# modelstreaming/ams

Hardware: AMD Instinct MI355X
Metric: frames/sec student infer (DeeplabV3+MobileNetV2, 512x1024) + distill-steps/sec (higher is better)
Workload: dtype f32 (2xfp16 split products)

## Files before the change

ams_amd/csrc/api.hip:

```cpp
#include "engine.hpp"
#include "head_common.hpp"

using namespace ams;

extern "C" {

const char* ams_last_error(void) { return ams::last_error(); }
int ams_abi_version(void) { return AMS_ABI_VERSION; }

int ams_device_info(char* name_out, size_t name_cap, int32_t* n_cu, int64_t* hbm_bytes) {
    int dev = 0;
    AMS_CHECK_HIP(hipGetDevice(&dev));
    hipDeviceProp_t p;
    AMS_CHECK_HIP(hipGetDeviceProperties(&p, dev));
    if (name_out && name_cap) { snprintf(name_out, name_cap, "%s (%s)", p.name, p.gcnArchName); }
    if (n_cu) *n_cu = p.multiProcessorCount;
    if (hbm_bytes) *hbm_bytes = (int64_t)p.totalGlobalMem;
    return AMS_OK;
}

int ams_student_arena_bytes(const ams_student_config* cfg, const ams_layer_desc* layers, size_t* bytes_out) {
    AMS_REQUIRE(bytes_out, "arena_bytes: null output");
    ams_student tmp;
    int rc = student_build(&tmp, cfg, layers);
// ... 639 lines not shown
                                int32_t* status_dev, int64_t* scratch_dev, size_t scratch_elems, void* stream) {
    AMS_REQUIRE(base_params_dev && payload_dev && payload_bytes_dev && status_dev && scratch_dev, "encode_delta_q8: null pointer");
    AMS_REQUIRE(advance_base == 0 || advance_base == 1, "encode_delta_q8: advance_base %d (0 or 1)", advance_base);
    bool has_stats = false;
    const int64_t shape = delta_table_shape(vars_host, n_vars, "encode_delta_q8", &has_stats);
    if (shape < 0) return AMS_E_INVALID;
    AMS_REQUIRE(base_stats_dev || !has_stats, "encode_delta_q8: null statistics base, and the table has variables in AMS_REGION_STATS");
    const size_t table = q8_encode_table_words(n_vars);
    const size_t need = table + 1 + (size_t)delta_segments(shape);
    AMS_REQUIRE(scratch_elems >= need, "encode_delta_q8: scratch too small (need %zu int64)", need);
    AMS_REQUIRE(payload_cap >= shape + 4 * (int64_t)n_vars, "encode_delta_q8: room for %lld bytes, the mask and scale sections alone have %lld",
                (long long)payload_cap, (long long)(shape + 4 * (int64_t)n_vars));
    AMS_REQUIRE(s, "encode_delta_q8: null handle");
    const int64_t mask_bytes = delta_mask_bytes(s, vars_host, n_vars, "encode_delta_q8");
    if (mask_bytes < 0) return AMS_E_INVALID;
    hipStream_t st = (hipStream_t)stream;
    if (s->ev_encode) AMS_CHECK_HIP(hipEventSynchronize(s->ev_encode));
    else RUN(create_sync_event(&s->ev_encode));
    s->encode_table.assign(table, 0);
    memcpy(s->encode_table.data(), vars_host, n_vars * sizeof(ams_delta_var));
    int64_t first = 0;
    for (int32_t i = 0; i < n_vars; ++i) { s->encode_table[4 * (size_t)n_vars + i] = first; first += vars_host[i].count; }
    s->encode_table[5 * (size_t)n_vars] = first;
    AMS_CHECK_HIP(hipMemcpyAsync(scratch_dev, s->encode_table.data(), table * sizeof(int64_t), hipMemcpyHostToDevice, st));
    AMS_CHECK_HIP(hipEventRecord(s->ev_encode, st));
    return launch_encode_delta_q8(mask_dev, scratch_dev, n_vars, mask_bytes, s->params, s->stats, base_params_dev, base_stats_dev, advance_base,
                                  scratch_dev + table, payload_dev, payload_cap, payload_bytes_dev, status_dev, st);
}

size_t ams_student_apply_delta_q8_scratch(const ams_delta_var* vars_host, int32_t n_vars) {
    return ams_student_apply_delta_scratch(vars_host, n_vars);
}

int ams_student_apply_delta_q8(ams_student* s, const uint8_t* payload_dev, int64_t payload_bytes, const ams_delta_var* vars_host, int32_t n_vars,
                               int64_t* n_applied_dev, int32_t* status_dev, int64_t* scratch_dev, size_t scratch_elems, void* stream) {
    AMS_REQUIRE(n_applied_dev && status_dev && scratch_dev, "apply_delta_q8: null pointer");
    AMS_REQUIRE(payload_bytes >= 0 && (payload_dev || payload_bytes == 0), "apply_delta_q8: %lld payload bytes at %p", (long long)payload_bytes,
                (const void*)payload_dev);
    bool has_stats = false;
    const int64_t shape = delta_table_shape(vars_host, n_vars, "apply_delta_q8", &has_stats);
    if (shape < 0) return AMS_E_INVALID;
    const size_t need = 4 * (size_t)n_vars + (size_t)delta_segments(shape);
    AMS_REQUIRE(scratch_elems >= need, "apply_delta_q8: scratch too small (need %zu int64)", need);
    AMS_REQUIRE(s, "apply_delta_q8: null handle");
    const int64_t mask_bytes = delta_mask_bytes(s, vars_host, n_vars, "apply_delta_q8");
    if (mask_bytes < 0) return AMS_E_INVALID;
    hipStream_t st = (hipStream_t)stream;
    if (s->ev_delta) AMS_CHECK_HIP(hipEventSynchronize(s->ev_delta));
    else RUN(create_sync_event(&s->ev_delta));
    s->delta_vars.assign(vars_host, vars_host + n_vars);
    ams_delta_var* vars_dev = reinterpret_cast<ams_delta_var*>(scratch_dev);
    AMS_CHECK_HIP(hipMemcpyAsync(vars_dev, s->delta_vars.data(), n_vars * sizeof(ams_delta_var), hipMemcpyHostToDevice, st));
    AMS_CHECK_HIP(hipEventRecord(s->ev_delta, st));
    return launch_apply_delta_q8(payload_dev, payload_bytes, vars_dev, n_vars, mask_bytes, s->params, (int64_t)s->cfg.n_trainable, s->stats,
                                 (int64_t)s->cfg.n_stats, scratch_dev + 4 * n_vars, n_applied_dev, status_dev, st);
}

int ams_k_stem_conv(const void* frames, int32_t frames_dtype, int32_t B, int32_t H, int32_t W, const float* w, int32_t cout,
                    const float* scale, const float* shift, int32_t act, float pixel_scale, float* y, void* stream) {
    return launch_stem(frames, frames_dtype, B, H, W, w, cout, scale, shift, act, pixel_scale, y, (hipStream_t)stream);
}

int ams_k_depthwise3x3(const float* x, int32_t B, int32_t H, int32_t W, int32_t C, const float* w, int32_t stride, int32_t rate,
                       const float* scale, const float* shift, int32_t act, float* y, void* stream) {
    return launch_depthwise(x, B, H, W, C, w, stride, rate, scale, shift, act, y, (hipStream_t)stream);
}

int ams_k_pointwise(const float* x, int64_t M, int32_t K, const float* w, int32_t N, int32_t trans_w, const float* img_bias,
                    int64_t rows_per_img, const float* scale, const float* shift, int32_t act, const float* res, float* y,
                    void* stream) {
    PwArgs a = pw_args(x, M, K, K, w, N, y, N);
    if (trans_w) { a.w_sk = 1; a.w_sn = K; }
    a.img_bias = img_bias; a.rows_per_img = rows_per_img > 0 ? rows_per_img : 1;
    a.scale = scale; a.shift = shift; a.act = act; a.res = res; a.ldr = N;
    if (scale && !shift) { set_error("pointwise: scale without shift"); return AMS_E_INVALID; }
    return launch_pointwise(a, (hipStream_t)stream);
}

int ams_k_pointwise_split(const float* x, int64_t M, int32_t K, const float* w, int32_t N, const float* scale, const float* shift,
                          int32_t act, const float* res, float* y, uint16_t* panels, size_t panel_elems, void* stream) {
    const int Kp = (K + 31) / 32 * 32;
    AMS_REQUIRE(panels && panel_elems >= (size_t)2 * N * Kp, "pointwise_split: panel scratch too small (need %zu)", (size_t)2 * N * Kp);
    hipStream_t st = (hipStream_t)stream;
    uint16_t* hi = panels;
    uint16_t* lo = panels + (size_t)N * Kp;
    RUN(launch_split_weights(w, N, 1, K, N, Kp, hi, lo, st));
    PwArgs a = pw_args(x, M, K, K, w, N, y, N);
    a.scale = scale; a.shift = shift; a.act = act; a.res = res; a.ldr = N;
    if (scale && !shift) { set_error("pointwise_split: scale without shift"); return AMS_E_INVALID; }
    return launch_pointwise_split(a, hi, lo, Kp, st);
}

int ams_k_pointwise_split3(const float* x, int64_t M, int32_t K, const float* w, int32_t N, const float* scale, const float* shift,
                           int32_t act, const float* res, float* y, uint16_t* panels, size_t panel_elems, void* stream) {
    const int Kp = (K + 31) / 32 * 32;
    const size_t plane = (size_t)N * Kp;
    AMS_REQUIRE(panels && panel_elems >= 3 * plane, "pointwise_split3: panel scratch too small (need %zu)", 3 * plane);
    hipStream_t st = (hipStream_t)stream;
    RUN(launch_split_weights3(w, N, 1, K, N, Kp, panels, panels + plane, panels + 2 * plane, st));
    PwArgs a = pw_args(x, M, K, K, w, N, y, N);
    a.scale = scale; a.shift = shift; a.act = act; a.res = res; a.ldr = N;
    if (scale && !shift) { set_error("pointwise_split3: scale without shift"); return AMS_E_INVALID; }
    return launch_pointwise_split3(a, panels, panels + plane, panels + 2 * plane, Kp, st);
}

int ams_k_pack_h2i(const float* x, int64_t M, int32_t Cn, float* out, void* stream) { return launch_pack_h2i(x, M, Cn, out, (hipStream_t)stream); }

int ams_k_pointwise_split_f16(const float* x, int64_t M, int32_t K, const float* w, int32_t N, const float* scale, const float* shift, int32_t act,
                              const float* res, float* y, uint16_t* panels, size_t panel_elems, float* x_h2i, uint16_t* y_parts, void* stream) {
    const int Kp = (K + 31) / 32 * 32;
    const size_t plane = (size_t)N * Kp;
    AMS_REQUIRE(panels && panel_elems >= 2 * plane, "pointwise_split_f16: panel scratch too small (need %zu)", 2 * plane);
    hipStream_t st = (hipStream_t)stream;
    RUN(launch_split_weights_f16(w, N, 1, K, N, Kp, panels, panels + plane, st));
    PwArgs a = pw_args(x, M, K, K, w, N, y, N);
    a.scale = scale; a.shift = shift; a.act = act; a.res = res; a.ldr = N;
    if (scale && !shift) { set_error("pointwise_split_f16: scale without shift"); return AMS_E_INVALID; }
    if (x_h2i) {
        if (x_h2i != x) RUN(launch_pack_h2i(x, M, K, x_h2i, st));
        a.x = x_h2i; a.x_fmt = 1;
    }
    if (y_parts) {
        AMS_REQUIRE(pointwise_split_writes_parts(a), "pointwise_split_f16: this shape has no vector epilogue to write parts from");
        a.ysplit = y_parts; a.ysplit_plane = M * (int64_t)N; a.ysplit_np = 2; a.ysplit_fmt = 1;
    }
    AMS_REQUIRE(pointwise_f16_applies(a), "pointwise_split_f16: unsupported shape M=%lld K=%d", (long long)M, K);
    return launch_pointwise_split_f16(a, panels, (int64_t)plane, Kp, st);
}

int ams_ingest_resize_u8(const uint8_t* src, int32_t Hs, int32_t Ws, int32_t Cn, int32_t mode, int32_t swap_rb, uint8_t* dst, int32_t H,
                         int32_t W, void* stream) {
    return launch_resize_u8(src, Hs, Ws, Cn, mode, swap_rb, dst, H, W, (hipStream_t)stream);
}

static void set_panels(ConvLayer* l, const uint16_t* panels, int64_t plane, int np, int Kp) { l->panels = panels; l->plane = plane; l->np = np; l->Kp = Kp; }

int ams_k_dw_project(const float* e, int32_t B, int32_t H, int32_t W, int32_t Cc, const float* w_dw, int32_t rate, const float* scale_d,
                     const float* shift_d, const float* w_proj, int32_t N, const float* scale_p, const float* shift_p,
                     const float* res, float* y, uint16_t* panels, size_t panel_elems, void* stream) {
    hipStream_t st = (hipStream_t)stream;
    const int64_t plane = (int64_t)N * Cc;
    BlockCall c;
    c.x = e; c.B = B; c.H = H; c.W = W; c.Cexp = Cc; c.rate = rate; c.Cout = N; c.residual = res != nullptr; c.res = res; c.y = y;
    c.dw = ConvLayer{w_dw, scale_d, shift_d, AMS_ACT_RELU6};
    c.project = ConvLayer{w_proj, scale_p, shift_p, AMS_ACT_NONE, panels, plane, 2, Cc};
    const EntryScratch sc{panels, panel_elems, (size_t)(2 * plane)};
    RUN(block_call_check("dw_project", BK_DW_PROJECT, c, &sc));
    RUN(launch_split_weights(w_proj, N, 1, Cc, N, Cc, panels, panels + plane, st));
    return launch_dw_project(c, st);
}

static int block_fused_entry(const char* who, bool f16, const float* x, int32_t B, int32_t H, int32_t W, int32_t Cin, const float* w_exp,
                             const float* scale_e, const float* shift_e, int32_t Cexp, const float* w_dw, int32_t stride, const float* scale_d,
                             const float* shift_d, const float* w_proj, int32_t Cout, const float* scale_p, const float* shift_p, int32_t residual,
                             float* y, uint16_t* panels, size_t panel_elems, void* stream) {
    hipStream_t st = (hipStream_t)stream;
    const int kp_p = (Cexp + 31) / 32 * 32;
    const int64_t pe = (int64_t)Cexp * 32, pp = (int64_t)Cout * kp_p;
    BlockCall c;
    c.x = x; c.B = B; c.H = H; c.W = W; c.Cin = Cin; c.Cexp = Cexp; c.stride = stride; c.Cout = Cout; c.residual = residual != 0; c.y = y;
    c.expand = ConvLayer{w_exp, scale_e, shift_e, AMS_ACT_RELU6};
    c.dw = ConvLayer{w_dw, scale_d, shift_d, AMS_ACT_RELU6};
    c.project = ConvLayer{w_proj, scale_p, shift_p, AMS_ACT_NONE};
    uint16_t* hp = panels ? panels + 2 * pe : nullptr;
    if (f16) { set_panels(&c.expand, panels, pe, AMS_NP_F16, 32); set_panels(&c.project, hp, pp, AMS_NP_F16, kp_p); }
    else if (panels) set_panels(&c.expand, panels, pe, 3, 32);
    const EntryScratch sc{panels, panel_elems, (size_t)(f16 ? 2 * pe + 2 * pp : panels ? 3 * pe : 0)};
    RUN(block_call_check(who, BK_WHOLE, c, &sc));
    if (f16) {
        RUN(launch_split_weights_f16(w_exp, Cexp, 1, Cin, Cexp, 32, panels, panels + pe, st));
        RUN(launch_split_weights_f16(w_proj, Cout, 1, Cexp, Cout, kp_p, hp, hp + pp, st));
    } else if (panels)
        RUN(launch_split_weights3(w_exp, Cexp, 1, Cin, Cexp, 32, panels, panels + pe, panels + 2 * pe, st));
    return launch_block_fused(c, st);
}

int ams_k_block_fused(const float* x, int32_t B, int32_t H, int32_t W, int32_t Cin, const float* w_exp, const float* scale_e, const float* shift_e,
                      int32_t Cexp, const float* w_dw, int32_t stride, const float* scale_d, const float* shift_d, const float* w_proj, int32_t Cout,
                      const float* scale_p, const float* shift_p, int32_t residual, float* y, uint16_t* panels, size_t panel_elems, void* stream) {
    return block_fused_entry("block_fused", false, x, B, H, W, Cin, w_exp, scale_e, shift_e, Cexp, w_dw, stride, scale_d, shift_d, w_proj, Cout, scale_p,
                             shift_p, residual, y, panels, panel_elems, stream);
}

int ams_k_block_fused_f16(const float* x, int32_t B, int32_t H, int32_t W, int32_t Cin, const float* w_exp, const float* scale_e, const float* shift_e,
                          int32_t Cexp, const float* w_dw, int32_t stride, const float* scale_d, const float* shift_d, const float* w_proj, int32_t Cout,
                          const float* scale_p, const float* shift_p, int32_t residual, float* y, uint16_t* panels, size_t panel_elems, void* stream) {
    return block_fused_entry("block_fused_f16", true, x, B, H, W, Cin, w_exp, scale_e, shift_e, Cexp, w_dw, stride, scale_d, shift_d, w_proj, Cout, scale_p,
                             shift_p, residual, y, panels, panel_elems, stream);
}

static_assert(sizeof(ams_first_block_plan) == sizeof(FirstBlockPlan) && sizeof(FirstBlockPlan) == 15 * sizeof(int32_t), "ams_first_block_plan is FirstBlockPlan, field by field");
static size_t first_block_scratch(int form) { return form == 1 ? 3 * 32 * 32 : (form == 2 ? 2 * 32 * 32 + 2 * 16 * 32 : 0); }
static BlockCall first_block_call(const void* frames, int dtype, int B, int H, int W, float pixel_scale, const float* w_stem, const float* scale_s,
                                  const float* shift_s, const float* w_dw, const float* scale_d, const float* shift_d, const float* w_proj,
                                  const float* scale_p, const float* shift_p, float* y) {
    BlockCall c;
    c.frames = frames; c.dtype = dtype; c.pixel_scale = pixel_scale; c.B = B; c.H = H; c.W = W; c.Cin = 3; c.Cexp = 32; c.Cout = 16; c.y = y;
    c.expand = ConvLayer{w_stem, scale_s, shift_s, AMS_ACT_RELU6};
    c.dw = ConvLayer{w_dw, scale_d, shift_d, AMS_ACT_RELU6};
    c.project = ConvLayer{w_proj, scale_p, shift_p, AMS_ACT_NONE};
    return c;
}

size_t ams_k_first_block_scratch(int32_t form) { return first_block_scratch(form); }

int ams_k_first_block_plan(int32_t frames_dtype, int32_t B, int32_t H, int32_t W, int32_t form, const int32_t* occupancy, ams_first_block_plan* plan_out) {
    BlockCall c;
    c.dtype = frames_dtype; c.B = B; c.H = H; c.W = W;
    const EntryScratch sc{nullptr, 0, 0, form, 3};
    RUN(block_call_check("first_block_plan", BK_FIRST_PLAN, c, &sc));
    AMS_REQUIRE(!occupancy || (occupancy[0] > 0 && occupancy[1] > 0 && occupancy[2] > 0), "first_block_plan: occupancy figures must be positive");
    AMS_REQUIRE(plan_out, "first_block_plan: null pointer");
    FirstBlockPlan p;
    RUN(first_block_plan(frames_dtype, B, H, W, form == 2, occupancy, &p));
    memcpy(plan_out, &p, sizeof(p));
    return AMS_OK;
}

int ams_k_first_block(const void* frames, int32_t frames_dtype, int32_t B, int32_t H, int32_t W, float pixel_scale, const float* w_stem,
                      const float* scale_s, const float* shift_s, const float* w_dw, const float* scale_d, const float* shift_d, const float* w_proj,
                      const float* scale_p, const float* shift_p, float* y, int32_t form, uint16_t* panels, size_t panel_elems,
                      ams_first_block_plan* plan_out, void* stream) {
    hipStream_t st = (hipStream_t)stream;
    const int64_t ps = 32 * 32, pj = 16 * 32;
    BlockCall c = first_block_call(frames, frames_dtype, B, H, W, pixel_scale, w_stem, scale_s, shift_s, w_dw, scale_d, shift_d, w_proj, scale_p, shift_p, y);
    uint16_t* hj = panels ? panels + 2 * ps : nullptr;
    if (form == 1) set_panels(&c.expand, panels, ps, 3, 32);
    else if (form == 2) { set_panels(&c.expand, panels, ps, AMS_NP_F16, 32); set_panels(&c.project, hj, pj, AMS_NP_F16, 32); }
    const EntryScratch sc{panels, panel_elems, first_block_scratch(form), form, 3};
    RUN(block_call_check("first_block", BK_FIRST, c, &sc));
    if (form == 1)
        RUN(launch_split_weights3(w_stem, 32, 1, 27, 32, 32, panels, panels + ps, panels + 2 * ps, st));
    else if (form == 2) {
        RUN(launch_split_weights_f16(w_stem, 32, 1, 27, 32, 32, panels, panels + ps, st));
        RUN(launch_split_weights_f16(w_proj, 16, 1, 32, 16, 32, hj, hj + pj, st));
    }
    FirstBlockPlan p;
    RUN(launch_first_block(c, st, &p));
    if (plan_out) memcpy(plan_out, &p, sizeof(p));
    return AMS_OK;
}

int ams_k_first_block_tiles(const void* frames, int32_t frames_dtype, int32_t B, int32_t H, int32_t W, float pixel_scale, const float* w_stem,
                            const float* scale_s, const float* shift_s, const float* w_dw, const float* scale_d, const float* shift_d,
                            const float* w_proj, const float* scale_p, const float* shift_p, float* y, void* stream) {
    return launch_first_block_tiles(first_block_call(frames, frames_dtype, B, H, W, pixel_scale, w_stem, scale_s, shift_s, w_dw, scale_d, shift_d, w_proj,
                                                     scale_p, shift_p, y), (hipStream_t)stream);
}

int ams_k_expand_dw(const float* x, int32_t B, int32_t H, int32_t W, int32_t Cin, const float* w_exp, const float* scale_e,
                    const float* shift_e, int32_t Cexp, const float* w_dw, int32_t stride, int32_t rate, const float* scale_d,
                    const float* shift_d, float* y, void* stream) {
    BlockCall c;
    c.x = x; c.B = B; c.H = H; c.W = W; c.Cin = Cin; c.Cexp = Cexp; c.stride = stride; c.rate = rate; c.y = y;
    c.expand = ConvLayer{w_exp, scale_e, shift_e, AMS_ACT_RELU6};
    c.dw = ConvLayer{w_dw, scale_d, shift_d, AMS_ACT_RELU6};
    return launch_expand_dw(c, (hipStream_t)stream);
}

static int expand_dw_stream_entry(const char* who, bool f16, const float* x, int32_t B, int32_t H, int32_t W, int32_t Cin, const float* w_exp,
                                  const float* scale_e, const float* shift_e, int32_t Cexp, const float* w_dw, int32_t rate, const float* scale_d,
                                  const float* shift_d, float* y, uint16_t* panels, size_t panel_elems, int32_t parts, int32_t presplit, int32_t y_h2i,
                                  void* stream) {
    hipStream_t st = (hipStream_t)stream;
    const bool f32 = !f16 && Cin <= 32;
    const int ns = f16 ? 2 : 3;
    const size_t plane = (size_t)Cexp * Cin, xplane = (size_t)B * H * W * Cin;
    BlockCall c;
    c.x = x; c.B = B; c.H = H; c.W = W; c.Cin = Cin; c.Cexp = Cexp; c.rate = rate; c.y = y; c.y_fmt = y_h2i ? 1 : 0;
    c.expand = ConvLayer{w_exp, scale_e, shift_e, AMS_ACT_RELU6};
    c.dw = ConvLayer{w_dw, scale_d, shift_d, AMS_ACT_RELU6};
    if (f32 && rate < 0) { c.stride = -rate; c.rate = 1; }
    const EntryScratch sc{panels, panel_elems, f32 ? 0 : ns * plane + (presplit ? ns * xplane : 0), 0, 1, f16 ? Cin >= 64 : (parts == 2 || parts == 3)};
    uint16_t* xq = panels && presplit ? panels + ns * plane : nullptr;
    if (!f32) {
        set_panels(&c.expand, panels, (int64_t)plane, f16 ? AMS_NP_F16 : parts, Cin);
        c.x_parts = xq; c.x_plane = (int64_t)xplane;
    }
    const bool wreg = !f32 && presplit == 2;
    RUN(block_call_check(who, wreg ? BK_WREG : BK_STREAM, c, &sc));
    AMS_REQUIRE(x, "%s: null pointer", who);
    if (!f32) {
        const int M = (int)((int64_t)B * H * W);
        if (f16) RUN(launch_split_weights_f16(w_exp, Cexp, 1, Cin, Cexp, Cin, panels, panels + plane, st));
        else RUN(launch_split_weights3(w_exp, Cexp, 1, Cin, Cexp, Cin, panels, panels + plane, panels + 2 * plane, st));
        if (xq && f16) RUN(launch_split_weights_f16(x, 1, Cin, Cin, M, Cin, xq, xq + xplane, st));
        else if (xq) RUN(launch_split_weights3(x, 1, Cin, Cin, M, Cin, xq, xq + xplane, xq + 2 * xplane, st));
    }
    return wreg ? launch_expand_dw_wreg(c, st) : launch_expand_dw_stream(c, st);
}

int ams_k_expand_dw_stream(const float* x, int32_t B, int32_t H, int32_t W, int32_t Cin, const float* w_exp, const float* scale_e,
                           const float* shift_e, int32_t Cexp, const float* w_dw, int32_t rate, const float* scale_d, const float* shift_d,
                           float* y, uint16_t* panels, size_t panel_elems, int32_t parts, int32_t presplit, void* stream) {
    return expand_dw_stream_entry("expand_dw_stream", false, x, B, H, W, Cin, w_exp, scale_e, shift_e, Cexp, w_dw, rate, scale_d, shift_d, y, panels, panel_elems,
                                  parts, presplit, 0, stream);
}

int ams_k_expand_dw_stream_f16(const float* x, int32_t B, int32_t H, int32_t W, int32_t Cin, const float* w_exp, const float* scale_e,
                               const float* shift_e, int32_t Cexp, const float* w_dw, int32_t rate, const float* scale_d, const float* shift_d,
                               float* y, uint16_t* panels, size_t panel_elems, int32_t presplit, int32_t y_h2i, void* stream) {
    return expand_dw_stream_entry("expand_dw_stream_f16", true, x, B, H, W, Cin, w_exp, scale_e, shift_e, Cexp, w_dw, rate, scale_d, shift_d, y, panels,
                                  panel_elems, 2, presplit, y_h2i, stream);
}

int ams_k_global_mean(const float* x, int32_t B, int64_t HW, int32_t C, float* y, float* scratch, size_t scratch_floats,
                      void* stream) {
    AMS_REQUIRE(scratch && scratch_floats >= image_colsum_scratch(B, C), "global_mean: scratch too small (need %zu floats)",
                image_colsum_scratch(B, C));
    return launch_global_mean(x, B, HW, C, y, scratch, (hipStream_t)stream);
}
size_t ams_k_global_mean_scratch(int32_t B, int32_t C) { return image_colsum_scratch(B, C); }

int ams_k_upsample_argmax(const float* logits, int32_t B, int32_t h, int32_t w, int32_t NC, const int32_t* class_idx_host, int32_t K,
                          int32_t H, int32_t W, const uint8_t* teacher, int32_t* labels_out, int64_t* conf_mat, double* loss,
                          void* stream) {
    const HeadCall c{logits, NC, B, h, w, class_idx_host, K, H, W, teacher, NC};
    return launch_upsample_argmax(c, labels_out, conf_mat, loss, (hipStream_t)stream);
}

int ams_k_upsample_confidence(const float* logits, int32_t B, int32_t h, int32_t w, int32_t NC, const int32_t* class_idx_host, int32_t K,
                              int32_t H, int32_t W, const uint8_t* teacher, uint8_t* conf_u8, float* conf_f32, int64_t* stats, void* stream) {
    const HeadCall c{logits, NC, B, h, w, class_idx_host, K, H, W, teacher, NC};
    return launch_upsample_confidence(c, conf_u8, conf_f32, stats, (hipStream_t)stream);
}
size_t ams_confidence_stats_len(void) { return (size_t)confidence_stats_len(); }

int ams_k_upsample_soft_metric_layout(const float* logits, int32_t B, int32_t h, int32_t w, int32_t ld, int32_t NC, const int32_t* class_idx_host,
                                      int32_t K, int32_t H, int32_t W, const uint8_t* teacher, const float* teacher_logits, int32_t th, int32_t tw,
                                      int32_t layout, int64_t* stats, float* p_f32, float* ce_f32, void* stream) {
    const HeadCall c{logits, ld, B, h, w, class_idx_host, K, H, W, teacher, NC};
    return launch_upsample_soft_metric(c, LossObjective{teacher_logits, th, tw, layout}, stats, p_f32, ce_f32, (hipStream_t)stream);
}

int ams_k_upsample_soft_metric(const float* logits, int32_t B, int32_t h, int32_t w, int32_t NC, const int32_t* class_idx_host, int32_t K,
                               int32_t H, int32_t W, const uint8_t* teacher, const float* teacher_logits, int32_t th, int32_t tw, int64_t* stats,
                               float* p_f32, float* ce_f32, void* stream) {
    return ams_k_upsample_soft_metric_layout(logits, B, h, w, NC, NC, class_idx_host, K, H, W, teacher, teacher_logits, th, tw, AMS_TLOGITS_FULL, stats, p_f32,
                                             ce_f32, stream);
}
size_t ams_soft_metric_stats_len(int32_t K) { return K >= 1 && K <= 32 ? (size_t)soft_metric_stats_len(K) : 0; }

int ams_k_ce_grad(const float* logits, int32_t B, int32_t h, int32_t w, int32_t NC, const int32_t* class_idx_host, int32_t K, int32_t H,
                  int32_t W, const uint8_t* teacher, const double* loss_and_count_dev, float* dlogits, void* stream) {
    const HeadCall c{logits, NC, B, h, w, class_idx_host, K, H, W, teacher, NC};
    return launch_ce_grad(c, loss_and_count_dev, dlogits, NC, (hipStream_t)stream);
}

size_t ams_k_ce_loss_grad_scratch(int32_t B, int32_t h, int32_t w, int32_t K) { return ce_loss_grad_scratch(B, h, w, K); }

static int ce_loss_grad_entry(const char* who, const HeadCall& c, const LossObjective& o, bool needs_teacher_logits, double* loss_dev, float* dlogits,
                              float* scratch, size_t scratch_floats, void* stream) {
    RUN(kd_params_check(who, o.temperature, o.alpha));
    RUN(loss_weights_check(who, o.class_weights, c.K, c.K, o.conf_gamma));
    AMS_REQUIRE(o.teacher_logits || !needs_teacher_logits, "%s: null teacher logits (alpha %g, conf_gamma %g)", who, (double)o.alpha, (double)o.conf_gamma);
    AMS_REQUIRE(c.cls, "%s: null class table", who);
    AMS_REQUIRE(c.K >= 1 && c.K <= 32, "%s: K=%d out of range (1..32)", who, c.K);
    AMS_REQUIRE(tlogits_layout_ok(o.layout), "%s: unknown teacher-logit layout %d", who, o.layout);
    AMS_REQUIRE(c.ld >= c.NC && c.ld <= 256, "%s: row stride %d must hold %d classes", who, c.ld, c.NC);
    AMS_REQUIRE(ce_loss_grad_supported(c.w, c.W), "%s: %d output columns on %d source columns is outside the one-pass kernel", who, c.W, c.w);
    AMS_REQUIRE(scratch && scratch_floats >= ce_loss_grad_scratch(c.B, c.h, c.w, c.K), "%s: scratch too small (need %zu floats)", who,
                ce_loss_grad_scratch(c.B, c.h, c.w, c.K));
    hipStream_t st = (hipStream_t)stream;
    RUN(launch_ce_loss_grad(c, o, loss_dev, scratch, st));
    return launch_ce_combine(c, loss_dev, scratch, dlogits, c.ld, st);
}

int ams_k_ce_loss_grad(const float* logits, int32_t B, int32_t h, int32_t w, int32_t NC, const int32_t* class_idx_host, int32_t K, int32_t H,
                       int32_t W, const uint8_t* teacher, double* loss_dev, float* dlogits, float* scratch, size_t scratch_floats, void* stream) {
    const HeadCall c{logits, NC, B, h, w, class_idx_host, K, H, W, teacher, NC};
    return ce_loss_grad_entry("ce_loss_grad", c, LossObjective{}, false, loss_dev, dlogits, scratch, scratch_floats, stream);
}

int ams_k_ce_loss_grad_soft(const float* logits, int32_t B, int32_t h, int32_t w, int32_t NC, const int32_t* class_idx_host, int32_t K, int32_t H,
                            int32_t W, const uint8_t* teacher, const float* teacher_logits, int32_t th, int32_t tw, double* loss_dev, float* dlogits,
                            float* scratch, size_t scratch_floats, void* stream) {
    const HeadCall c{logits, NC, B, h, w, class_idx_host, K, H, W, teacher, NC};
    const LossObjective o{teacher_logits, th, tw, AMS_TLOGITS_FULL};
    return ce_loss_grad_entry("ce_loss_grad_soft", c, o, true, loss_dev, dlogits, scratch, scratch_floats, stream);
}

int ams_k_ce_loss_grad_soft_layout(const float* logits, int32_t B, int32_t h, int32_t w, int32_t ld, int32_t NC, const int32_t* class_idx_host,
                                   int32_t K, int32_t H, int32_t W, const uint8_t* teacher, const float* teacher_logits, int32_t th, int32_t tw, int32_t layout,
                                   double* loss_dev, float* dlogits, float* scratch, size_t scratch_floats, void* stream) {
    const HeadCall c{logits, ld, B, h, w, class_idx_host, K, H, W, teacher, NC};
    const LossObjective o{teacher_logits, th, tw, layout};
    return ce_loss_grad_entry("ce_loss_grad_soft_layout", c, o, true, loss_dev, dlogits, scratch, scratch_floats, stream);
}

int ams_k_ce_loss_grad_kd(const float* logits, int32_t B, int32_t h, int32_t w, int32_t ld, int32_t NC, const int32_t* class_idx_host, int32_t K,
                          int32_t H, int32_t W, const uint8_t* teacher, const float* teacher_logits, int32_t th, int32_t tw, int32_t layout,
                          double* loss_dev, float* dlogits, float* scratch, size_t scratch_floats, void* stream, float temperature, float alpha) {
    const HeadCall c{logits, ld, B, h, w, class_idx_host, K, H, W, teacher, NC};
    const LossObjective o{teacher_logits, th, tw, layout, temperature, alpha};
    return ce_loss_grad_entry("ce_loss_grad_kd", c, o, true, loss_dev, dlogits, scratch, scratch_floats, stream);
}

int ams_k_ce_loss_grad_weighted(const float* logits, int32_t B, int32_t h, int32_t w, int32_t ld, int32_t NC, const int32_t* class_idx_host, int32_t K,
                                int32_t H, int32_t W, const uint8_t* teacher, const float* teacher_logits, int32_t th, int32_t tw, int32_t layout,
                                double* loss_dev, float* dlogits, float* scratch, size_t scratch_floats, void* stream, float temperature, float alpha,
                                const float* class_weights_host, float conf_gamma) {
    const HeadCall c{logits, ld, B, h, w, class_idx_host, K, H, W, teacher, NC};
    const LossObjective o{teacher_logits, th, tw, layout, temperature, alpha, class_weights_host, conf_gamma};
    return ce_loss_grad_entry("ce_loss_grad_weighted", c, o, conf_gamma != 0.f || alpha != 0.f, loss_dev, dlogits, scratch, scratch_floats, stream);
}

size_t ams_k_loss_mining_scratch(int32_t B, int32_t H, int32_t W) { return loss_mining_scratch(B, H, W); }

int ams_k_ce_loss_grad_mined(const float* logits, int32_t B, int32_t h, int32_t w, int32_t ld, int32_t NC, const int32_t* class_idx_host, int32_t K,
                             int32_t H, int32_t W, const uint8_t* teacher, const float* teacher_logits, int32_t th, int32_t tw, int32_t layout,
                             double* loss_dev, float* dlogits, float* scratch, size_t scratch_floats, void* stream, float temperature, float alpha,
                             const float* class_weights_host, float conf_gamma, float top_k, uint8_t* labels_out_dev, float* key_out_dev,
                             ams_mining_result* result_dev, void* mining_scratch_dev, size_t mining_scratch_bytes) {
    const char* who = "ce_loss_grad_mined";
    HeadCall c{logits, ld, B, h, w, class_idx_host, K, H, W, teacher, NC};
    const LossObjective o{teacher_logits, th, tw, layout, temperature, alpha, class_weights_host, conf_gamma};
    RUN(kd_params_check(who, o.temperature, o.alpha));
    RUN(loss_weights_check(who, o.class_weights, c.K, c.K, o.conf_gamma));
    AMS_REQUIRE(o.teacher_logits || (conf_gamma == 0.f && alpha == 0.f), "%s: null teacher logits (alpha %g, conf_gamma %g)", who, (double)o.alpha, (double)o.conf_gamma);
    AMS_REQUIRE(c.cls, "%s: null class table", who);
    AMS_REQUIRE(c.K >= 1 && c.K <= 32, "%s: K=%d out of range (1..32)", who, c.K);
    AMS_REQUIRE(tlogits_layout_ok(o.layout), "%s: unknown teacher-logit layout %d", who, o.layout);
    AMS_REQUIRE(c.ld >= c.NC && c.ld <= 256, "%s: row stride %d must hold %d classes", who, c.ld, c.NC);
    AMS_REQUIRE(ce_loss_grad_supported(c.w, c.W), "%s: %d output columns on %d source columns is outside the one-pass kernel", who, c.W, c.w);
    AMS_REQUIRE(scratch && scratch_floats >= ce_loss_grad_scratch(c.B, c.h, c.w, c.K), "%s: scratch too small (need %zu floats)", who,
                ce_loss_grad_scratch(c.B, c.h, c.w, c.K));
    RUN(mining_top_k_check(who, top_k));
    hipStream_t st = (hipStream_t)stream;
    if (top_k < 1.f) {
        AMS_REQUIRE(B >= 1 && H >= 1 && W >= 1, "%s: no pixels: B=%d, %d x %d", who, B, H, W);
        AMS_REQUIRE(mining_scratch_dev && ((uintptr_t)mining_scratch_dev & 15) == 0 && mining_scratch_bytes >= loss_mining_scratch(B, H, W),
                    "%s: mining scratch NULL, misaligned or too small (need %zu bytes, 16-byte aligned)", who, loss_mining_scratch(B, H, W));
        AMS_REQUIRE(labels_out_dev && result_dev, "%s: null output (mined labels, result)", who);
        AMS_REQUIRE(((uintptr_t)result_dev & 7) == 0 && ((uintptr_t)key_out_dev & 3) == 0, "%s: misaligned output", who);
        MiningBuffers m = loss_mining_buffers(mining_scratch_dev, B, H, W);
        m.labels = labels_out_dev;
        m.result = result_dev;
        if (key_out_dev) m.keys = key_out_dev;
        AMS_REQUIRE(loss_dev && dlogits, "%s: null pointer", who);
        RUN(launch_loss_mining(c, o, top_k, m, st));
        c.teacher = labels_out_dev;
    } else {
        AMS_REQUIRE(labels_out_dev, "%s: null output (mined labels)", who);
        AMS_REQUIRE(c.logits && c.teacher && loss_dev && dlogits && B >= 1 && H >= 1 && W >= 1, "%s: null pointer", who);
        AMS_CHECK_HIP(hipMemcpyAsync(labels_out_dev, teacher, (size_t)B * H * W, hipMemcpyDeviceToDevice, st));
    }
    RUN(launch_ce_loss_grad(c, o, loss_dev, scratch, st));
    return launch_ce_combine(c, loss_dev, scratch, dlogits, c.ld, st);
}

size_t ams_k_pointwise_wgrad_scratch(int64_t M, int32_t K, int32_t N) { return pointwise_wgrad_scratch(M, K, N); }

int ams_k_pointwise_wgrad_split(const float* x, const float* dy, int64_t M, int32_t K, int32_t N, float* dw, float* scratch,
                                size_t scratch_floats, void* stream) {
    if (!pointwise_wgrad_x6_applies(M, K, N, K, N)) { set_error("pointwise_wgrad_split: shape M=%lld K=%d N=%d not supported", (long long)M, K, N); return AMS_E_INVALID; }
    WgArgs a;
    a.x = x; a.ldx = K; a.K = K; a.dy = dy; a.ldy = N; a.N = N; a.M = M; a.dw = dw; a.scratch = scratch; a.scratch_floats = scratch_floats; a.allow_split = 1;
    return launch_pointwise_wgrad(a, (hipStream_t)stream);
}

int ams_k_pointwise_wgrad(const float* x, const float* dy, int64_t M, int32_t K, int32_t N, float* dw, float* scratch,
                          size_t scratch_floats, void* stream) {
    WgArgs a;
    a.x = x; a.ldx = K; a.K = K; a.dy = dy; a.ldy = N; a.N = N; a.M = M; a.dw = dw; a.scratch = scratch; a.scratch_floats = scratch_floats; a.allow_split = 0;
    return launch_pointwise_wgrad(a, (hipStream_t)stream);
}

int ams_k_depthwise3x3_dgrad(const float* dy, int32_t B, int32_t H, int32_t W, int32_t C, const float* w, int32_t stride, int32_t rate,
                             float* dx, void* stream) {
    return launch_depthwise_dgrad(dy, B, H, W, C, w, stride, rate, dx, (hipStream_t)stream);
}

int ams_k_depthwise3x3_wgrad(const float* x, const float* dy, int32_t B, int32_t H, int32_t W, int32_t C, int32_t stride, int32_t rate,
                             float* dw, float* scratch, size_t scratch_floats, void* stream) {
    return launch_depthwise_wgrad(x, dy, B, H, W, C, stride, rate, dw, scratch, scratch_floats, (hipStream_t)stream);
}

int ams_k_pointwise_red(const float* x, int64_t M, int32_t K, const float* w, int32_t N, int32_t trans_w, int32_t split, int32_t mode,
                        const float* center, const float* z, const float* scale, const float* shift, const float* mean, const float* rstd,
                        int32_t act, const float* res, float* y, float* part, size_t part_floats, int32_t* rows_out, uint16_t* panels,
                        size_t panel_elems, void* stream) {
    AMS_REQUIRE(x && w && y && part && rows_out && (mode == 1 || mode == 2), "pointwise_red: bad arguments");
    AMS_REQUIRE(mode == 1 || (z && scale && shift && mean && rstd), "pointwise_red: mode 2 needs z, scale, shift, mean, rstd");
    hipStream_t st = (hipStream_t)stream;
    PwArgs a = pw_args(x, M, K, K, w, N, y, N);
    if (trans_w) { a.w_sk = 1; a.w_sn = K; }
    a.res = res; a.ldr = N;
    a.red_mode = mode; a.red_center = center; a.red_z = z; a.red_scale = scale; a.red_shift = shift; a.red_mean = mean; a.red_rstd = rstd;
    a.red_act = act; a.red_part = part; a.red_part_floats = part_floats;
    int rows = 0;
    a.red_rows_out = &rows;
    int rc;
    if (split == 2) {
        const int Kp = (K + 31) / 32 * 32;
        const size_t plane = (size_t)N * Kp;
        AMS_REQUIRE(panels && panel_elems >= 2 * plane && pointwise_f16_applies(a), "pointwise_red: fp16 form needs mode 1, K %% 8 == 0 and %zu panel elements", 2 * plane);
        RUN(launch_split_weights_f16(w, a.w_sk, a.w_sn, K, N, Kp, panels, panels + plane, st));
        rc = launch_pointwise_split_f16(a, panels, (int64_t)plane, Kp, st);
    } else if (split) {
        const int Kp = (K + 31) / 32 * 32;
        const size_t plane = (size_t)N * Kp;
        AMS_REQUIRE(panels && panel_elems >= 3 * plane && K % 8 == 0, "pointwise_red: panel scratch too small (need %zu) or K %% 8", 3 * plane);
        RUN(launch_split_weights3(w, a.w_sk, a.w_sn, K, N, Kp, panels, panels + plane, panels + 2 * plane, st));
        rc = launch_pointwise_split3(a, panels, panels + plane, panels + 2 * plane, Kp, st);
    } else {
        rc = launch_pointwise(a, st);
    }
    *rows_out = rows;
    return rc;
}

int ams_k_pointwise_xform(const float* x, int64_t M, int32_t K, const float* w, int32_t N, int32_t trans_w, int32_t split, int32_t x_mode,
                          int32_t x_act, const float* v0, const float* v1, const float* v2, const float* x2, float* y, float* x_tmp,
                          uint16_t* panels, size_t panel_elems, void* stream) {
    AMS_REQUIRE(x && w && y && v0 && v1 && (x_mode == 1 || (x_mode == 2 && v2 && x2)), "pointwise_xform: bad arguments");
    hipStream_t st = (hipStream_t)stream;
    PwArgs a = pw_args(x, M, K, K, w, N, y, N);
    if (trans_w) { a.w_sk = 1; a.w_sn = K; }
    a.x_mode = x_mode; a.x_act = x_act; a.x_v0 = v0; a.x_v1 = v1; a.x_v2 = v2; a.x2 = x2; a.x_tmp = x_tmp;
    if (split == 2) {
        const int Kp = (K + 31) / 32 * 32;
        const size_t plane = (size_t)N * Kp;
        AMS_REQUIRE(panels && panel_elems >= 2 * plane && pointwise_f16_applies(a), "pointwise_xform: fp16 form needs x_mode 1, K %% 8 == 0, K <= 1024 and %zu panel elements", 2 * plane);
        RUN(launch_split_weights_f16(w, a.w_sk, a.w_sn, K, N, Kp, panels, panels + plane, st));
        return launch_pointwise_split_f16(a, panels, (int64_t)plane, Kp, st);
    }
    if (split) {
        const int Kp = (K + 31) / 32 * 32;
        const size_t plane = (size_t)N * Kp;
        AMS_REQUIRE(panels && panel_elems >= 3 * plane && K % 8 == 0, "pointwise_xform: panel scratch too small (need %zu) or K %% 8", 3 * plane);
        RUN(launch_split_weights3(w, a.w_sk, a.w_sn, K, N, Kp, panels, panels + plane, panels + 2 * plane, st));
        return launch_pointwise_split3(a, panels, panels + plane, panels + 2 * plane, Kp, st);
    }
    return launch_pointwise(a, st);
}

int ams_k_pointwise_wgrad_xform(const float* x, const float* dy, int64_t M, int32_t K, int32_t N, int32_t split, int32_t x_mode, int32_t x_act,
                                const float* v0, const float* v1, int32_t dy_mode, const float* d0, const float* d1, const float* d2,
                                const float* dy2, float* dw, float* scratch, size_t scratch_floats, void* stream) {
    AMS_REQUIRE(x && dy && dw && scratch, "pointwise_wgrad_xform: null pointer");
    if (split && !pointwise_wgrad_x6_applies(M, K, N, K, N)) { set_error("pointwise_wgrad_xform: shape M=%lld K=%d N=%d outside the split kernel", (long long)M, K, N); return AMS_E_INVALID; }
    WgArgs a;
    a.x = x; a.ldx = K; a.K = K; a.dy = dy; a.ldy = N; a.N = N; a.M = M; a.dw = dw; a.scratch = scratch; a.scratch_floats = scratch_floats;
    a.allow_split = split != 0;
    a.x_mode = x_mode; a.x_act = x_act; a.x_v0 = v0; a.x_v1 = v1;
    a.dy_mode = dy_mode; a.dy_v0 = d0; a.dy_v1 = d1; a.dy_v2 = d2; a.dy2 = dy2;
    return launch_pointwise_wgrad(a, (hipStream_t)stream);
}

size_t ams_k_depthwise3x3_fwd_bn_scratch(int32_t B, int32_t H, int32_t W, int32_t C, int32_t rate) { return depthwise_fwd_bn_scratch(B, H, W, C, rate); }
int ams_k_depthwise3x3_fwd_bn(const float* ze, int32_t B, int32_t H, int32_t W, int32_t C, const float* w, int32_t rate, const float* scale,
                              const float* shift, int32_t act, const float* center, float* zd, float* scratch, size_t scratch_floats,
                              int32_t* rows_out, void* stream) {
    AMS_REQUIRE(ze && w && scale && shift && zd && scratch && rows_out, "depthwise3x3_fwd_bn: null pointer");
    AMS_REQUIRE(scratch_floats >= depthwise_fwd_bn_scratch(B, H, W, C, rate), "depthwise3x3_fwd_bn: scratch too small");
    int rows = 0;
    int rc = launch_depthwise_fwd_bn(ze, B, H, W, C, w, rate, scale, shift, act, center, zd, scratch, &rows, (hipStream_t)stream);
    *rows_out = rows;
    return rc;
}
size_t ams_k_depthwise3x3_dgrad_bn_scratch(int32_t B, int32_t H, int32_t W, int32_t C) { return depthwise_dgrad_bn_scratch(B, H, W, C); }
int ams_k_depthwise3x3_dgrad_bn(const float* dz, int32_t B, int32_t H, int32_t W, int32_t C, const float* w, int32_t rate, const float* z_prev,
                                const float* scale, const float* shift, int32_t act, const float* mean, const float* rstd, float* out,
                                float* scratch, size_t scratch_floats, int32_t* rows_out, void* stream) {
    AMS_REQUIRE(dz && w && z_prev && scale && shift && mean && rstd && out && scratch && rows_out, "depthwise3x3_dgrad_bn: null pointer");
    AMS_REQUIRE(rate == 1 || rate == 2, "depthwise3x3_dgrad_bn: rate %d", rate);
    AMS_REQUIRE(scratch_floats >= depthwise_dgrad_bn_scratch(B, H, W, C), "depthwise3x3_dgrad_bn: scratch too small");
    int rows = 0;
    int rc = launch_depthwise_dgrad_bn(dz, B, H, W, C, w, rate, z_prev, scale, shift, act, mean, rstd, out, scratch, &rows, (hipStream_t)stream);
    *rows_out = rows;
    return rc;
}

size_t ams_k_depthwise3x3_fwd_bn_tiles_scratch(int32_t B, int32_t H, int32_t W, int32_t C, int32_t rate) { return depthwise_fwd_bn2_scratch(B, H, W, C, rate); }
int ams_k_depthwise3x3_fwd_bn_tiles(const float* ze, int32_t B, int32_t H, int32_t W, int32_t C, const float* w, int32_t rate, const float* scale,
                                    const float* shift, int32_t act, const float* center, float* zd, float* scratch, size_t scratch_floats,
                                    int32_t* rows_out, void* stream) {
    AMS_REQUIRE(ze && w && scale && shift && zd && scratch && rows_out, "depthwise3x3_fwd_bn_tiles: null pointer");
    AMS_REQUIRE(scratch_floats >= depthwise_fwd_bn2_scratch(B, H, W, C, rate), "depthwise3x3_fwd_bn_tiles: scratch too small");
    int rows = 0;
    int rc = launch_depthwise_fwd_bn2(ze, B, H, W, C, w, rate, scale, shift, act, center, zd, scratch, &rows, (hipStream_t)stream);
    *rows_out = rows;
    return rc;
}

size_t ams_k_depthwise3x3_dgrad_bn_apply_scratch(int32_t B, int32_t H, int32_t W, int32_t C, int32_t rate) { return depthwise_dgrad_bn2_scratch(B, H, W, C, rate); }
int ams_k_depthwise3x3_dgrad_bn_apply(const float* dy, const float* zd, const float* cA, const float* cB, const float* cC, int32_t B, int32_t H, int32_t W,
                                      int32_t C, const float* w, int32_t rate, const float* z_prev, const float* scale, const float* shift, int32_t act,
                                      const float* mean, const float* rstd, float* out, float* scratch, size_t scratch_floats, int32_t* rows_out,
                                      void* stream) {
    AMS_REQUIRE(dy && zd && cA && cB && cC && w && z_prev && scale && shift && mean && rstd && out && scratch && rows_out, "depthwise3x3_dgrad_bn_apply: null pointer");
    AMS_REQUIRE(rate == 1 || rate == 2, "depthwise3x3_dgrad_bn_apply: rate %d", rate);
    AMS_REQUIRE(scratch_floats >= depthwise_dgrad_bn2_scratch(B, H, W, C, rate), "depthwise3x3_dgrad_bn_apply: scratch too small");
    int rows = 0;
    int rc = launch_depthwise_dgrad_bn2(dy, zd, cA, cB, cC, B, H, W, C, w, rate, z_prev, scale, shift, act, mean, rstd, out, scratch, &rows, (hipStream_t)stream);
    *rows_out = rows;
    return rc;
}

size_t ams_k_xx_gram_scratch(int64_t M, int32_t Cin) { return xx_stats_scratch_doubles(M, Cin); }
int ams_k_xx_gram(const float* x, int64_t M, int32_t Cin, double* scratch, size_t scratch_doubles, double* xx64, float* xx32, void* stream) {
    AMS_REQUIRE(scratch_doubles >= xx_stats_scratch_doubles(M, Cin), "xx_gram: scratch too small");
    return launch_xx_gram(x, M, Cin, scratch, xx64, xx32, (hipStream_t)stream);
}
int ams_k_expand_stats(const double* xx64, int32_t Cin, const float* w_exp, int32_t Cexp, double n, const float* center, const float* gamma,
                       const float* beta, float eps, float one_minus_decay, float* moving_mean, float* moving_var, float* scale, float* shift,
// ... 58 lines not shown
```

ams_amd/csrc/k_xdw_stream.hip:

```cpp
#include "pw_common.hpp"
#include "split_bf16.hpp"
#include "block_call.hpp"

namespace ams {

#ifdef AMS_XDW_PK
#define AMS_DW_FMA4(A_, V_, W_) fma4_pk(A_, V_, W_)
#else
#define AMS_DW_FMA4(A_, V_, W_) do { A_.x = fmaf(V_.x, W_.x, A_.x); A_.y = fmaf(V_.y, W_.y, A_.y); A_.z = fmaf(V_.z, W_.z, A_.z); A_.w = fmaf(V_.w, W_.w, A_.w); } while (0)
#endif

constexpr int xds_pitch(int nc) { return nc == 32 ? 48 : nc == 64 ? 80 : nc == 96 ? 112 : nc + 4; }

struct XdsArgs {
    const float* x;
    const unsigned short* xs;
    int64_t xs_plane;
    int B, H, W, Cin;
    const unsigned short* wp;
    int64_t plane;
    const float* wf;
    const float* sc_e; const float* sh_e;
    int act_e;
    int Cexp;
    const float* w_dw;
    const float* sc_d; const float* sh_d;
    int act_d;
    float* y;
    int rate;
    int stride;
    int Ho, Wo, cy0, cx0;
    int SH, SW;
    int Wp;
    int T;
    int ring;
    int nsy, nsx;
    int chunks;
    int items;
    int groups;
    int y_fmt;
    int timed;
};

__device__ unsigned long long g_xds_cycles[1024][8];

template <int KS, int NT, int NP, int NWE, int NWD, bool PRE, bool F32, int S = 1, bool H16 = false>
__global__ __launch_bounds__(64 * (NWE + NWD)) void xdw_stream_kernel(XdsArgs a, unsigned nblocks) {
    static_assert(!H16 || (NP == 2 && !F32 && S == 1), "the fp16 form: two parts, stride 1");
    constexpr int NC = 16 * NT;
    constexpr int CG = NC / 4;
    constexpr int STEP = 16 * NWE;
    constexpr int PX = STEP * CG / (64 * NWD);
    static_assert(PX * 64 * NWD == STEP * CG && PX >= 1, "D-step mapping");
    static_assert(!(F32 && PRE), "the exact-f32 form splits nothing");
    constexpr int PITCH = xds_pitch(NC);
    constexpr int MIRROR = 4;
    constexpr int Kp = F32 ? KS * 16 : KS * 32;
    constexpr int WPF = NC + 4;
    constexpr int W_BYTES = F32 ? Kp * WPF * 4 : NP * Kp * NC * 2;
    extern __shared__ __attribute__((aligned(16))) unsigned char smem[];
    u32x4* sW = reinterpret_cast<u32x4*>(smem);
    float* sWf = reinterpret_cast<float*>(smem);
    float* sAff = reinterpret_cast<float*>(smem + W_BYTES);
    float* ring = sAff + 2 * NC;

    const unsigned lb = xcd_remap(blockIdx.x, nblocks);
    const int chunk = lb % a.chunks;
    const int group = lb / a.chunks;
    const int n0 = chunk * NC;
    const int tid = threadIdx.x, lane = tid & 63;
    const int wave = __builtin_amdgcn_readfirstlane(tid >> 6);
    const int Wp = a.Wp, rate = a.rate, R = a.ring;

    if constexpr (F32) {
        for (int e = tid; e < Kp * NC; e += 64 * (NWE + NWD)) {
            const int k = e / NC, n = e - k * NC;
            const int nn = n0 + n < a.Cexp ? n0 + n : a.Cexp - 1;
            sWf[k * WPF + n] = k < a.Cin ? a.wf[(int64_t)k * a.Cexp + nn] : 0.f;
        }
    } else {
        constexpr int UPR = Kp / 8;
        constexpr int NPIECE = NP * NC * UPR;
        for (int e = tid; e < NPIECE; e += 64 * (NWE + NWD)) {
            const int part = e / (NC * UPR), r = e - part * (NC * UPR), n = r / UPR, u = r - n * UPR;
            const int nn = n0 + n < a.Cexp ? n0 + n : a.Cexp - 1;
            const u32x4 v = *reinterpret_cast<const u32x4*>(a.wp + part * a.plane + (int64_t)nn * Kp + u * 8);
            sW[((part * KS + (u >> 2)) * 4 + (u & 3)) * NC + n] = v;
        }
    }
    if (tid < NC) {
        const int nn = n0 + tid < a.Cexp ? n0 + tid : a.Cexp - 1;
        sAff[tid] = a.sc_e[nn]; sAff[NC + tid] = a.sh_e[nn];
    }
    __syncthreads();
    const int qS = STEP / Wp, rS = STEP - qS * Wp;
    unsigned long long tc[2] = {0, 0}, tl_ = a.timed ? __builtin_amdgcn_s_memtime() : 0, nstep = 0;
    auto lap = [&](int slot) {
        if (a.timed) {
            const unsigned long long now = __builtin_amdgcn_s_memtime();
            tc[slot] += now - tl_;
            tl_ = now;
        }
    };
    auto flush = [&](int base) {
        if (a.timed && lane == 0) {
            unsigned long long* row = g_xds_cycles[(blockIdx.x * 8 + wave) & 1023];
            atomicAdd(&row[base], tc[0]);
            atomicAdd(&row[base + 1], tc[1]);
            atomicAdd(&row[base ? 7 : 6], nstep);
        }
    };

    if (wave < NWE) {
        const int l15 = lane & 15, q = lane >> 4;
        const int ring_lane = (16 * wave + l15) * PITCH + 4 * q;
        int sbase = 0;
        for (int item = group; item < a.items; item += a.groups) {
            int u1 = item;
            const int segx = u1 % a.nsx; u1 /= a.nsx;
            const int segy = u1 % a.nsy; u1 /= a.nsy;
            const int sub = u1 % (rate * rate);
            const int b = u1 / (rate * rate);
            const int sy = sub / rate, sx = sub - sy * rate;
            const int Hs = (a.H - sy + rate - 1) / rate, Ws = (a.W - sx + rate - 1) / rate;
            const int i0 = segy * a.SH, j0 = segx * a.SW;
            const bool live = i0 < Hs && j0 < Ws;
            const int64_t frame0 = (int64_t)b * a.H * a.W * a.Cin + (F32 ? 0 : 8 * q);
            int e_row, e_col;
            { const int e0 = 16 * wave + l15; e_row = e0 / Wp; e_col = e0 - e_row * Wp; }
            float4 raw[(PRE || F32) ? 1 : KS][2];
            u32x4 rawp[PRE ? KS : 1][NP];
            float4 rawf[F32 ? KS : 1];
            bool in_next = false;
            auto next_pixel = [&]() -> int64_t {
                const int i = i0 - 1 + e_row, j = j0 - 1 + e_col;
                in_next = (i >= 0) & (i < Hs) & (j >= 0) & (j < Ws) & (e_row < a.SH + 2) & live;
                const int ic = i < 0 ? 0 : (i > Hs - 1 ? Hs - 1 : i), jc = j < 0 ? 0 : (j > Ws - 1 ? Ws - 1 : j);
                return frame0 + ((int64_t)(sy + rate * ic) * a.W + (sx + rate * jc)) * a.Cin;
            };
            auto load_stage = [&](int64_t off, int s) {
                if constexpr (F32) {
                    int ko = 16 * s + 4 * q;
                    if (ko > a.Cin - 4) ko = a.Cin - 4;
                    rawf[s] = ld4(a.x + off + ko);
                } else if constexpr (PRE) {
#pragma unroll
                    for (int pp = 0; pp < NP; ++pp) rawp[s][pp] = *reinterpret_cast<const u32x4*>(a.xs + pp * a.xs_plane + off + 32 * s);
                } else {
                    raw[s][0] = ld4(a.x + off + 32 * s);
                    raw[s][1] = ld4(a.x + off + 32 * s + 4);
                }
            };
            {
                const int64_t p = next_pixel();
#pragma unroll
                for (int s = 0; s < KS; ++s) load_stage(p, s);
            }
            for (int t = 0; t < a.T; ++t) {
                const bool inside = in_next;
                f32x4 acc[NT], accx[H16 ? NT : 1];
#pragma unroll
                for (int tt = 0; tt < NT; ++tt) acc[tt] = (f32x4){0.f, 0.f, 0.f, 0.f};
#pragma unroll
                for (int tt = 0; tt < (H16 ? NT : 1); ++tt) accx[tt] = (f32x4){0.f, 0.f, 0.f, 0.f};
                e_row += qS; e_col += rS;
                if (e_col >= Wp) { e_col -= Wp; ++e_row; }
                const int64_t pn = next_pixel();
                if constexpr (F32) {
#pragma unroll
                    for (int s = 0; s < KS; ++s) {
                        const float4 av[1] = {rawf[s]};
                        load_stage(pn, s);
                        f32x4(&acc2)[1][NT] = *reinterpret_cast<f32x4(*)[1][NT]>(&acc);
                        pw_chunk<1, NT, WPF>(acc2, av, sWf + (16 * s + 4 * q) * WPF + l15);
                    }
                } else {
                bf16x8 x0, x1, x2;
    #pragma unroll
                    for (int s = 0; s < KS; ++s) {
                        if constexpr (PRE) {
                            x0 = __builtin_bit_cast(bf16x8, rawp[s][0]);
                            if (NP >= 2) x1 = __builtin_bit_cast(bf16x8, rawp[s][NP >= 2 ? 1 : 0]);
                            if (NP == 3) x2 = __builtin_bit_cast(bf16x8, rawp[s][NP - 1]);
                        } else if constexpr (H16) {
                            f16x8 h, l;
                            split8_f16(raw[s][0], raw[s][1], h, l);
                            x0 = __builtin_bit_cast(bf16x8, h); x1 = __builtin_bit_cast(bf16x8, l);
                        } else {
                            if (NP == 3) split8(raw[s][0], raw[s][1], x0, x1, x2);
                            else if (NP == 2) split8(raw[s][0], raw[s][1], x0, x1);
                            else split8(raw[s][0], raw[s][1], x0);
                        }
                        load_stage(pn, s);
                        const u32x4* bw = sW + (s * 4 + q) * NC + l15;
                        bf16x8 q0[NT], q1[NT], q2[NT];
    #pragma unroll
                        for (int tt = 0; tt < NT; ++tt) {
                            q0[tt] = *reinterpret_cast<const bf16x8*>(bw + 16 * tt);
                            if (NP >= 2) q1[tt] = *reinterpret_cast<const bf16x8*>(bw + KS * 4 * NC + 16 * tt);
                            if (NP == 3) q2[tt] = *reinterpret_cast<const bf16x8*>(bw + 2 * KS * 4 * NC + 16 * tt);
                        }
                        if constexpr (H16) {
    #pragma unroll
                            for (int tt = 0; tt < NT; ++tt) accx[tt] = __builtin_amdgcn_mfma_f32_16x16x32_f16(__builtin_bit_cast(f16x8, q1[tt]), __builtin_bit_cast(f16x8, x0), accx[tt], 0, 0, 0);
    #pragma unroll
                            for (int tt = 0; tt < NT; ++tt) accx[tt] = __builtin_amdgcn_mfma_f32_16x16x32_f16(__builtin_bit_cast(f16x8, q0[tt]), __builtin_bit_cast(f16x8, x1), accx[tt], 0, 0, 0);
    #pragma unroll
                            for (int tt = 0; tt < NT; ++tt) acc[tt] = __builtin_amdgcn_mfma_f32_16x16x32_f16(__builtin_bit_cast(f16x8, q0[tt]), __builtin_bit_cast(f16x8, x0), acc[tt], 0, 0, 0);
                        } else {
                        if (NP == 3) {
    #pragma unroll
                            for (int tt = 0; tt < NT; ++tt) acc[tt] = __builtin_amdgcn_mfma_f32_16x16x32_bf16(q2[tt], x0, acc[tt], 0, 0, 0);
    #pragma unroll
                            for (int tt = 0; tt < NT; ++tt) acc[tt] = __builtin_amdgcn_mfma_f32_16x16x32_bf16(q0[tt], x2, acc[tt], 0, 0, 0);
    #pragma unroll
                            for (int tt = 0; tt < NT; ++tt) acc[tt] = __builtin_amdgcn_mfma_f32_16x16x32_bf16(q1[tt], x1, acc[tt], 0, 0, 0);
                        }
                        if (NP >= 2) {
    #pragma unroll
                            for (int tt = 0; tt < NT; ++tt) acc[tt] = __builtin_amdgcn_mfma_f32_16x16x32_bf16(q1[tt], x0, acc[tt], 0, 0, 0);
    #pragma unroll
                            for (int tt = 0; tt < NT; ++tt) acc[tt] = __builtin_amdgcn_mfma_f32_16x16x32_bf16(q0[tt], x1, acc[tt], 0, 0, 0);
                        }
    #pragma unroll
                        for (int tt = 0; tt < NT; ++tt) acc[tt] = __builtin_amdgcn_mfma_f32_16x16x32_bf16(q0[tt], x0, acc[tt], 0, 0, 0);
                        }
                    }
                }
                {
                    float* dst = ring + sbase * PITCH + ring_lane;
                    const bool mirror = sbase == 0 && 16 * wave + l15 < MIRROR;
#pragma unroll
                    for (int tt = 0; tt < NT; ++tt) {
                        const float4 sc = ld4(sAff + 16 * tt + 4 * q), sh = ld4(sAff + NC + 16 * tt + 4 * q);
                        float4 v;
                        const float lo = inside ? (a.act_e == AMS_ACT_NONE ? -__builtin_huge_valf() : 0.f) : 0.f;
                        const float hi = inside ? (a.act_e == AMS_ACT_RELU6 ? 6.f : __builtin_huge_valf()) : 0.f;
                        if constexpr (H16) acc[tt] = combine_f16(acc[tt], accx[H16 ? tt : 0]);
                        const float4 bn = muladd4_pk(make_float4(acc[tt][0], acc[tt][1], acc[tt][2], acc[tt][3]), sc, sh);
                        v.x = __builtin_amdgcn_fmed3f(bn.x, lo, hi); v.y = __builtin_amdgcn_fmed3f(bn.y, lo, hi);
                        v.z = __builtin_amdgcn_fmed3f(bn.z, lo, hi); v.w = __builtin_amdgcn_fmed3f(bn.w, lo, hi);
                        st4(dst + 16 * tt, v);
                        if (mirror) st4(dst + R * PITCH + 16 * tt, v);
                    }
                }
                sbase += STEP;
                if (sbase == R) sbase = 0;
                lap(0);
                __syncthreads();
                lap(1);
                ++nstep;
            }
            __syncthreads();
        }
        flush(0);
    } else {
        const int dt = tid - 64 * NWE;
        const int cg = dt % CG, pt = dt / CG;
        const bool chan_ok = n0 + 4 * cg < a.Cexp;
        const int nch = chan_ok ? n0 + 4 * cg : 0;
        float4 wv[9];
#pragma unroll
        for (int k = 0; k < 9; ++k) wv[k] = ld4(a.w_dw + (int64_t)k * a.Cexp + nch);
        const float4 dsc = ld4(a.sc_d + nch), dsh = ld4(a.sh_d + nch);
        const bool odd_cg = (cg & 1) != 0;
        const unsigned ych = a.y_fmt ? (unsigned)(nch >> 3) * 32u + (odd_cg ? 16u : 0u) : (unsigned)nch * 4u;
        int cb = (2 * R - 2 * Wp - 2 + pt * PX) % R;
        for (int item = group; item < a.items; item += a.groups) {
            int u1 = item;
            const int segx = u1 % a.nsx; u1 /= a.nsx;
            const int segy = u1 % a.nsy; u1 /= a.nsy;
            const int sub = u1 % (rate * rate);
            const int b = u1 / (rate * rate);
            const int sy = sub / rate, sx = sub - sy * rate;
            const int Hs = (a.H - sy + rate - 1) / rate, Ws = (a.W - sx + rate - 1) / rate;
            const int i0 = segy * a.SH, j0 = segx * a.SW;
            const bool live = i0 < Hs && j0 < Ws && chan_ok;
            const int64_t oframe = S == 2 ? (int64_t)a.Ho * a.Wo * a.Cexp : (int64_t)a.H * a.W * a.Cexp;
            const __amdgpu_buffer_rsrc_t yrsrc = __builtin_amdgcn_make_buffer_rsrc(a.y + b * oframe, 0, (int)(oframe * 4), 0x00020000);
            const int rmax = live ? (a.SH < Hs - i0 ? a.SH : Hs - i0) : 0, cmax = a.SW < Ws - j0 ? a.SW : Ws - j0;
            const int colpitch = rate * a.Cexp * 4, rowpitch = rate * a.W * a.Cexp * 4;
            const int off0 = ((sy + rate * (i0 - 1)) * a.W + sx + rate * (j0 - 1)) * a.Cexp * 4 + (int)ych;
            int d_row, d_col;
            { const int c0 = Wp - 1 + pt * PX; d_row = c0 / Wp; d_col = c0 - d_row * Wp; d_row -= 2; }
            __syncthreads();
            for (int t = 0; t < a.T; ++t) {
                if constexpr (S == 2) {
#pragma unroll
                    for (int h = 0; h < PX; h += 2) {
                        int row = d_row, col = d_col + h;
#pragma unroll
                        for (int w = 0; w < (PX + 1) / 2; ++w)
                            if (col >= Wp) { col -= Wp; ++row; }
                        const int u = (j0 + col - 1 - a.cx0) & 1;
                        col += u;
                        if (col >= Wp) { col -= Wp; ++row; }
                        const int i = i0 + row - 1, j = j0 + col - 1;
                        const bool ok = ((unsigned)(row - 1) < (unsigned)rmax) & ((unsigned)(col - 1) < (unsigned)cmax) &
                                        ((((i - a.cy0) | (j - a.cx0)) & 1) == 0);
                        if (__builtin_amdgcn_ballot_w64(ok) != 0) {
                            float4 v[3][3];
#pragma unroll
                            for (int di = 0; di < 3; ++di) {
                                unsigned slot = (unsigned)(cb + di * Wp + h + u);
                                slot = slot < (unsigned)R ? slot : slot - (unsigned)R;
                                const float* rp = ring + __umul24(slot, PITCH) + 4 * cg;
#pragma unroll
                                for (int jj = 0; jj < 3; ++jj) v[di][jj] = ld4(rp + jj * PITCH);
                            }
                            float4 acc4 = make_float4(0.f, 0.f, 0.f, 0.f);
#pragma unroll
                            for (int ii = 0; ii < 3; ++ii)
#pragma unroll
                                for (int jj = 0; jj < 3; ++jj) {
                                    const float4 vv = v[ii][jj];
                                    const float4 w4 = wv[ii * 3 + jj];
                                    AMS_DW_FMA4(acc4, vv, w4);
                                }
                            float4 o;
                            o.x = apply_act(acc4.x * dsc.x + dsh.x, a.act_d); o.y = apply_act(acc4.y * dsc.y + dsh.y, a.act_d);
                            o.z = apply_act(acc4.z * dsc.z + dsh.z, a.act_d); o.w = apply_act(acc4.w * dsc.w + dsh.w, a.act_d);
                            const int oy = (i - a.cy0) >> 1, ox = (j - a.cx0) >> 1;
                            const unsigned off = ok ? (unsigned)((oy * a.Wo + ox) * a.Cexp * 4) + ych : 0xfffffff0u;
                            const u32x4 d = {__float_as_uint(o.x), __float_as_uint(o.y), __float_as_uint(o.z), __float_as_uint(o.w)};
                            __builtin_amdgcn_raw_buffer_store_b128(d, yrsrc, off, 0, 0);
                        }
                    }
                } else
#pragma unroll
                for (int h = 0; h < PX; h += 2) {
                    constexpr int PH = PX >= 2 ? 2 : 1;
                    float4 v[3][PH + 2];
#pragma unroll
                    for (int di = 0; di < 3; ++di) {
                        unsigned slot = (unsigned)(cb + di * Wp + h);
                        slot = slot < (unsigned)R ? slot : slot - (unsigned)R;
                        const float* rp = ring + __umul24(slot, PITCH) + 4 * cg;
#pragma unroll
                        for (int jj = 0; jj < PH + 2; ++jj) v[di][jj] = ld4(rp + jj * PITCH);
                    }
#pragma unroll
                    for (int u = 0; u < PH; ++u) {
                        float4 acc4 = make_float4(0.f, 0.f, 0.f, 0.f);
#pragma unroll
                        for (int i = 0; i < 3; ++i)
#pragma unroll
                            for (int j = 0; j < 3; ++j) {
                                const float4 vv = v[i][u + j];
                                const float4 w4 = wv[i * 3 + j];
                                AMS_DW_FMA4(acc4, vv, w4);
                            }
                        float4 o;
                        o.x = apply_act(acc4.x * dsc.x + dsh.x, a.act_d); o.y = apply_act(acc4.y * dsc.y + dsh.y, a.act_d);
                        o.z = apply_act(acc4.z * dsc.z + dsh.z, a.act_d); o.w = apply_act(acc4.w * dsc.w + dsh.w, a.act_d);
                        int row = d_row, col = d_col + h + u;
#pragma unroll
                        for (int w = 0; w < (PX + 1) / 2; ++w)
                            if (col >= Wp) { col -= Wp; ++row; }
                        const bool ok = ((unsigned)(row - 1) < (unsigned)rmax) & ((unsigned)(col - 1) < (unsigned)cmax);
                        const unsigned off = ok ? (unsigned)(row * rowpitch + col * colpitch + off0) : 0xfffffff0u;
                        if (H16 && a.y_fmt) {
                            unsigned h[2], l[2];
                            split4_f16(o, h, l);
                            const unsigned r0 = (unsigned)__builtin_amdgcn_update_dpp(0, (int)(odd_cg ? h[0] : l[0]), 0xB1, 0xF, 0xF, false);
                            const unsigned r1 = (unsigned)__builtin_amdgcn_update_dpp(0, (int)(odd_cg ? h[1] : l[1]), 0xB1, 0xF, 0xF, false);
                            const u32x4 d = {odd_cg ? r0 : h[0], odd_cg ? r1 : h[1], odd_cg ? l[0] : r0, odd_cg ? l[1] : r1};
                            __builtin_amdgcn_raw_buffer_store_b128(d, yrsrc, off, 0, 0);
                        } else {
                        const u32x4 d = {__float_as_uint(o.x), __float_as_uint(o.y), __float_as_uint(o.z), __float_as_uint(o.w)};
                        __builtin_amdgcn_raw_buffer_store_b128(d, yrsrc, off, 0, 0);
                        }
                    }
                }
                d_row += qS; d_col += rS;
                if (d_col >= Wp) { d_col -= Wp; ++d_row; }
                cb += STEP;
                if (cb >= R) cb -= R;
                lap(0);
                __syncthreads();
                lap(1);
                ++nstep;
            }
        }
        flush(2);
    }
}

int xds_phase_cycles(unsigned long long* h) {
    static unsigned long long rows[1024][8], z[1024][8];
    if (hipMemcpyFromSymbol(rows, HIP_SYMBOL(g_xds_cycles), sizeof(rows)) != hipSuccess) return AMS_E_HIP;
    if (hipMemcpyToSymbol(HIP_SYMBOL(g_xds_cycles), z, sizeof(z)) != hipSuccess) return AMS_E_HIP;
    for (int i = 0; i < 8; ++i) h[i] = 0;
    for (int r = 0; r < 1024; ++r)
        for (int i = 0; i < 8; ++i) h[i] += rows[r][i];
    return AMS_OK;
}

struct XdsPlan { int nt, nwe, nwd, SH, SW, nsy, nsx, ring, groups; size_t lds; };

static size_t xds_lds(int Kp, int nt, int np, int ring) {
    const int NC = 16 * nt;
    const size_t w = np == 0 ? (size_t)Kp * (NC + 4) * 4 : (size_t)np * Kp * NC * 2;
    return w + 2 * NC * 4 + (size_t)(ring + 4) * xds_pitch(NC) * 4;
}
static int xds_ring(int SW, int step) { return (2 * (SW + 2) + 2 + 2 * step + step - 1) / step * step; }

static bool xds_plan_try(int B, int H, int W, int Cin, int Cexp, int rate, int np, int nt, int nwe, int nwd, int nsy_force, int nsx_force,
                         int groups_force, XdsPlan* p) {
    const int Kp = np == 0 ? (Cin + 15) / 16 * 16 : Cin;
    const int Hs = (H + rate - 1) / rate, Ws = (W + rate - 1) / rate;
    const int step = 16 * nwe;
    const size_t budget = 160 * 1024 - 512;
    int nsx = nsx_force > 0 ? nsx_force : 1;
    int SW, ring;
    for (;; ++nsx) {
        SW = (Ws + nsx - 1) / nsx;
        ring = xds_ring(SW, step);
        if (xds_lds(Kp, nt, np, ring) <= budget / 2 || SW <= 24 || nsx_force > 0) break;
    }
    for (; xds_lds(Kp, nt, np, ring) > budget && SW > 1; ++nsx) {
        SW = (Ws + nsx) / (nsx + 1);
        ring = xds_ring(SW, step);
    }
    if (xds_lds(Kp, nt, np, ring) > budget || SW < 1) return false;
    nsx = (Ws + SW - 1) / SW;
    const int chunks = (Cexp + 16 * nt - 1) / (16 * nt);
    int nsy = 1;
    if (nsy_force > 0) nsy = nsy_force;
    else
        while ((int64_t)B * rate * rate * chunks * nsx * nsy < 768 && (Hs + nsy - 1) / nsy > 8) ++nsy;
    p->nt = nt; p->nwe = nwe; p->nwd = nwd; p->nsx = nsx; p->SW = SW; p->nsy = nsy; p->SH = (Hs + nsy - 1) / nsy; p->ring = ring;
    p->lds = xds_lds(Kp, nt, np, ring);
    const int64_t items = (int64_t)B * rate * rate * nsx * nsy;
    int64_t groups = groups_force > 0 ? groups_force : (2048 + chunks - 1) / chunks;
    if (groups > items) groups = items;
    if (groups < 1) groups = 1;
    p->groups = (int)groups;
    return true;
}

static bool xds_plan(int B, int H, int W, int Cin, int Cexp, int rate, int np, XdsPlan* p) {
    int nt = Cin >= 128 ? 4 : 2, nsy_force = 0, nsx_force = 0, nwe = 4, nwd = 4, groups_force = 0;
    if (knobs().xds_set) { const int* f = knobs().xds; nt = f[0]; nsy_force = f[1]; nsx_force = f[2]; nwe = f[3]; nwd = f[4]; groups_force = f[5]; }
    if (nt != 2 && nt != 4) nt = Cin >= 128 ? 4 : 2;
    if (np == 0) { nwe = 4; nwd = 4; }
    if (!((nwe == 4 && (nwd == 2 || nwd == 4)) || (nwe == 8 && nwd == 4))) { nwe = 4; nwd = 4; }
    if (xds_plan_try(B, H, W, Cin, Cexp, rate, np, nt, nwe, nwd, nsy_force, nsx_force, groups_force, p)) return true;
    if (xds_plan_try(B, H, W, Cin, Cexp, rate, np, 2, nwe, nwd, nsy_force, nsx_force, groups_force, p)) return true;
    return xds_plan_try(B, H, W, Cin, Cexp, rate, np, 2, 4, 4, nsy_force, 0, groups_force, p);
}

bool expand_dw_stream_supported(int Cin, int Cexp, int stride, int rate) {
    if (rate != 1 && rate != 2) return false;
    if (stride == 2) { if (rate != 1 || Cin > 32) return false; }
    else if (stride != 1) return false;
    if (Cin != 16 && Cin != 24 && Cin != 32 && Cin != 64 && Cin != 96 && Cin != 160) return false;
    return Cexp % 16 == 0 && Cexp >= 32;
}

template <int KS, int NT, int NP, int NWE, int NWD, bool PRE, bool F32 = false, int S = 1, bool H16 = false>
static int launch_xds_p(XdsArgs a, const XdsPlan& p, hipStream_t st) {
    RUN_RC(func_allow_lds((const void*)xdw_stream_kernel<KS, NT, NP, NWE, NWD, PRE, F32, S, H16>, p.lds));
    const int64_t nblocks = (int64_t)a.groups * a.chunks;
    AMS_REQUIRE(nblocks > 0 && nblocks < 0x7fffffffLL, "expand_dw_stream: bad grid");
    static const std::string nm = "xdw_stream_kernel<" + std::to_string(KS) + ", " + std::to_string(NT) + ", " + std::to_string(NP) + ", " +
                                  std::to_string(NWE) + ", " + std::to_string(NWD) + (PRE ? ", true" : ", false") + (F32 ? ", true, " : ", false, ") + std::to_string(S) +
                                  (H16 ? ", true>" : ", false>");
    note_kernel(nm.c_str());
    hipLaunchKernelGGL((xdw_stream_kernel<KS, NT, NP, NWE, NWD, PRE, F32, S, H16>), dim3((unsigned)nblocks), dim3(64 * (NWE + NWD)), p.lds, st, a, (unsigned)nblocks);
    AMS_CHECK_LAUNCH();
    return AMS_OK;
}

template <int KS, int NT, int NP, int NWE, int NWD>
static int launch_xds_k(const XdsArgs& a, const XdsPlan& p, hipStream_t st) {
    return a.xs ? launch_xds_p<KS, NT, NP, NWE, NWD, true>(a, p, st) : launch_xds_p<KS, NT, NP, NWE, NWD, false>(a, p, st);
}

template <int KS, int NT, int NP>
static int launch_xds_w(const XdsArgs& a, const XdsPlan& p, hipStream_t st) {
    if (p.nwe == 8) return launch_xds_k<KS, NT, NP, 8, 4>(a, p, st);
    if (p.nwd == 4) return launch_xds_k<KS, NT, NP, 4, 4>(a, p, st);
    return launch_xds_k<KS, NT, NP, 4, 2>(a, p, st);
}

template <int KC>
static int launch_xds_f32(const XdsArgs& a, const XdsPlan& p, hipStream_t st) {
    if (a.stride == 2) return p.nt == 4 ? launch_xds_p<KC, 4, 3, 4, 4, false, true, 2>(a, p, st) : launch_xds_p<KC, 2, 3, 4, 4, false, true, 2>(a, p, st);
    if (p.nt == 4) return launch_xds_p<KC, 4, 3, 4, 4, false, true>(a, p, st);
    return launch_xds_p<KC, 2, 3, 4, 4, false, true>(a, p, st);
}

template <int KS>
static int launch_xds_h16(const XdsArgs& a, const XdsPlan& p, hipStream_t st) {
    if (p.nt == 4) return a.xs ? launch_xds_p<KS, 4, 2, 4, 4, true, false, 1, true>(a, p, st) : launch_xds_p<KS, 4, 2, 4, 4, false, false, 1, true>(a, p, st);
    return a.xs ? launch_xds_p<KS, 2, 2, 4, 4, true, false, 1, true>(a, p, st) : launch_xds_p<KS, 2, 2, 4, 4, false, false, 1, true>(a, p, st);
}

template <int KS>
static int launch_xds_ks(const XdsArgs& a, const XdsPlan& p, int np, hipStream_t st) {
    if (p.nt == 4) return np == 3 ? launch_xds_w<KS, 4, 3>(a, p, st) : np == 1 ? launch_xds_w<KS, 4, 1>(a, p, st) : launch_xds_w<KS, 4, 2>(a, p, st);
    return np == 3 ? launch_xds_w<KS, 2, 3>(a, p, st) : np == 1 ? launch_xds_w<KS, 2, 1>(a, p, st) : launch_xds_w<KS, 2, 2>(a, p, st);
}

int launch_expand_dw_stream(const BlockCall& c, hipStream_t st) {
    RUN_RC(block_call_check("expand_dw_stream", BK_STREAM, c));
    const int B = c.B, H = c.H, W = c.W, Cin = c.Cin, Cexp = c.Cexp, stride = c.stride, rate = c.rate;
    const bool f32 = Cin <= 32;
    const bool h16 = !f32 && c.expand.np == AMS_NP_F16;
    const int np = f32 ? 0 : h16 ? 2 : c.expand.np;
    AMS_REQUIRE((int64_t)H * W * Cexp * 4 < 0x7fffffffLL, "expand_dw_stream: a frame of the output exceeds 2 GiB");
    XdsPlan p;
    AMS_REQUIRE(xds_plan(B, H, W, Cin, Cexp, rate, np, &p), "expand_dw_stream: no segment geometry fits LDS (W=%d rate=%d)", W, rate);
    XdsArgs a;
    memset(&a, 0, sizeof(a));
    a.x = c.x; a.xs = f32 ? nullptr : c.x_parts; a.xs_plane = c.x_plane; a.wf = c.expand.w; a.B = B; a.H = H; a.W = W; a.Cin = Cin; a.wp = c.expand.panels; a.plane = c.expand.plane;
    a.sc_e = c.expand.scale; a.sh_e = c.expand.shift; a.act_e = c.expand.act;
    a.Cexp = Cexp; a.w_dw = c.dw.w; a.sc_d = c.dw.scale; a.sh_d = c.dw.shift; a.act_d = c.dw.act; a.y = c.y; a.rate = rate;
    a.stride = stride;
    if (stride == 2) {
        int pt, pl;
        same_pad(H, 3, 2, 1, &a.Ho, &pt);
        same_pad(W, 3, 2, 1, &a.Wo, &pl);
        a.cy0 = 1 - pt; a.cx0 = 1 - pl;
    }
    const int step = 16 * p.nwe;
    a.SH = p.SH; a.SW = p.SW; a.Wp = p.SW + 2; a.T = ((p.SH + 2) * a.Wp + step - 1) / step; a.ring = p.ring;
    a.nsy = p.nsy; a.nsx = p.nsx; a.chunks = (Cexp + 16 * p.nt - 1) / (16 * p.nt);
    a.items = B * rate * rate * p.nsy * p.nsx; a.groups = p.groups;
    a.y_fmt = c.y_fmt;
    a.timed = knobs().xwr_timed;
    if (h16) {
        AMS_REQUIRE(p.nwe == 4 && p.nwd == 4, "expand_dw_stream: the fp16 form runs with 4 + 4 waves");
        switch (Cin / 32) {
            case 2: return launch_xds_h16<2>(a, p, st);
            case 3: return launch_xds_h16<3>(a, p, st);
            default: return launch_xds_h16<5>(a, p, st);
        }
    }
    if (f32) return Cin <= 16 ? launch_xds_f32<1>(a, p, st) : launch_xds_f32<2>(a, p, st);
    switch (Cin / 32) {
        case 2: return launch_xds_ks<2>(a, p, np, st);
        case 3: return launch_xds_ks<3>(a, p, np, st);
        default: return launch_xds_ks<5>(a, p, np, st);
    }
}

}
```

ams_amd/csrc/k_xdw_wreg.hip:

```cpp
#include "pw_common.hpp"
#include "split_bf16.hpp"
#include "block_call.hpp"

namespace ams {

#ifdef AMS_XDW_PK
#define AMS_DW_FMA4(A_, V_, W_) fma4_pk(A_, V_, W_)
#else
#define AMS_DW_FMA4(A_, V_, W_) do { A_.x = fmaf(V_.x, W_.x, A_.x); A_.y = fmaf(V_.y, W_.y, A_.y); A_.z = fmaf(V_.z, W_.z, A_.z); A_.w = fmaf(V_.w, W_.w, A_.w); } while (0)
#endif

struct XwrArgs {
    const unsigned short* xs;
    int64_t xs_plane;
    int B, H, W, Cin;
    const unsigned short* wp;
    int64_t plane;
    const float* sc_e; const float* sh_e;
    int act_e;
    int Cexp;
    const float* w_dw;
    const float* sc_d; const float* sh_d;
    int act_d;
    float* y;
    int rate;
    int SH, SW, Wp, T, ring;
    int nsy, nsx;
    int cgroups;
    int items, groups;
    int y_fmt;
};

__device__ unsigned long long g_xwr_cycles[1024][8];

template <int KS, int NP, int NWE, int NWD, int NRG, bool H16 = false, int ABL = 0>
__global__ __launch_bounds__(64 * (NWE + NWD)) void xdw_wreg_kernel(XwrArgs a, unsigned nblocks) {
    static_assert(!H16 || NP == 2, "the fp16 form has two parts");
    constexpr int STEP = 16 * NRG;
    constexpr int NCB = 32 * NWE;
    constexpr int CG = NCB / 4;
    constexpr int NDT = 64 * NWD;
    constexpr int PX = STEP * CG / NDT;
    static_assert(PX * NDT == STEP * CG && NDT % CG == 0 && (PX == 1 || PX % 2 == 0), "D-step mapping");
    constexpr int PH = PX >= 2 ? 2 : 1;
    constexpr int PITCH = NCB + 4;
    constexpr int MIRROR = 4;
    constexpr int Kp = KS * 32;
    constexpr int PPP = NP * KS * 4;
    constexpr int AUNITS = NRG * PPP * 16;
    constexpr int TPP = 4 * NWE / NRG;
    constexpr int LPT = (PPP + TPP - 1) / TPP;
    extern __shared__ __attribute__((aligned(16))) unsigned char smem[];
    u32x4* sA = reinterpret_cast<u32x4*>(smem);
    float* ring = reinterpret_cast<float*>(smem + 2 * AUNITS * 16);

    const unsigned lb = xcd_remap(blockIdx.x, nblocks);
    const int cgi = lb % a.cgroups;
    const int group = lb / a.cgroups;
    const int tid = threadIdx.x, lane = tid & 63;
    const int wave = __builtin_amdgcn_readfirstlane(tid >> 6);
    const int Wp = a.Wp, rate = a.rate, R = a.ring;
    const int qS = STEP / Wp, rS = STEP - qS * Wp;
    constexpr bool TIMED = (ABL & 32) != 0;
    unsigned long long tc[4] = {0, 0, 0, 0}, tl_ = TIMED ? __builtin_amdgcn_s_memtime() : 0, nstep = 0;
    auto lap = [&](int slot) {
        if constexpr (TIMED) {
            const unsigned long long now = __builtin_amdgcn_s_memtime();
            tc[slot] += now - tl_;
            tl_ = now;
        }
    };
    auto flush = [&](int base) {
        if (TIMED && lane == 0) {
            unsigned long long* row = g_xwr_cycles[(blockIdx.x * 8 + wave) & 1023];
            atomicAdd(&row[base], tc[0]);
            atomicAdd(&row[base + 1], tc[1]);
            atomicAdd(&row[base ? 7 : 6], nstep);
            if (base) { atomicAdd(&row[4], tc[2]); atomicAdd(&row[5], tc[3]); }
        }
    };

    if (wave < NWE) {
        const int l15 = lane & 15, q = lane >> 4;
        const int n0 = cgi * NCB + 32 * wave;
        const bool active = n0 < a.Cexp;
        const int n0c = active ? n0 : 0;
        bf16x8 wq[NP][KS][2];
#pragma unroll
        for (int pp = 0; pp < NP; ++pp)
#pragma unroll
            for (int s = 0; s < KS; ++s)
#pragma unroll
                for (int tt = 0; tt < 2; ++tt)
                    wq[pp][s][tt] = *reinterpret_cast<const bf16x8*>(a.wp + pp * a.plane + (int64_t)(n0c + 16 * tt + l15) * Kp + 32 * s + 8 * q);
        float4 esc[2], esh[2];
#pragma unroll
        for (int tt = 0; tt < 2; ++tt) { esc[tt] = ld4(a.sc_e + n0c + 16 * tt + 4 * q); esh[tt] = ld4(a.sh_e + n0c + 16 * tt + 4 * q); }
        const int ring_lane = l15 * PITCH + 32 * wave + 4 * q;
        const float lo_e = a.act_e == AMS_ACT_NONE ? -__builtin_huge_valf() : 0.f, hi_e = a.act_e == AMS_ACT_RELU6 ? 6.f : __builtin_huge_valf();
        const int lrg = NRG == 2 ? (q & 1) : 0;
        const int lj = NRG == 2 ? wave * 2 + (q >> 1) : wave * 4 + q;
        int64_t psrc[LPT];
        int pdst[LPT];
#pragma unroll
        for (int k = 0; k < LPT; ++k) {
            int j = lj + k * TPP;
            if (j > PPP - 1) j = PPP - 1;
            const int part = j / (KS * 4), u = j - part * (KS * 4);
            psrc[k] = part * a.xs_plane + 8 * u;
            pdst[k] = (lrg * PPP + j) * 16 + l15;
        }
        int sbase = 0;
        int par = 0;
        for (int item = group; item < a.items; item += a.groups) {
            int u1 = item;
            const int segx = u1 % a.nsx; u1 /= a.nsx;
            const int segy = u1 % a.nsy; u1 /= a.nsy;
            const int sub = u1 % (rate * rate);
            const int b = u1 / (rate * rate);
            const int sy = sub / rate, sx = sub - sy * rate;
            const int Hs = (a.H - sy + rate - 1) / rate, Ws = (a.W - sx + rate - 1) / rate;
            const int i0 = segy * a.SH, j0 = segx * a.SW;
            const bool live = i0 < Hs && j0 < Ws;
            const unsigned short* xf = a.xs + (int64_t)b * a.H * a.W * a.Cin;
            int e_row[NRG], e_col[NRG];
#pragma unroll
            for (int rg = 0; rg < NRG; ++rg) { const int e0 = l15 + 16 * rg; e_row[rg] = e0 / Wp; e_col[rg] = e0 - e_row[rg] * Wp; }
            bool in_cur[NRG];
            auto inside_of = [&](int rg) {
                const int i = i0 - 1 + e_row[rg], j = j0 - 1 + e_col[rg];
                return (bool)((i >= 0) & (i < Hs) & (j >= 0) & (j < Ws) & (e_row[rg] < a.SH + 2) & live);
            };
            auto loader_pixel = [&]() -> const unsigned short* {
                const int er = NRG == 2 ? (lrg ? e_row[NRG - 1] : e_row[0]) : e_row[0], ec = NRG == 2 ? (lrg ? e_col[NRG - 1] : e_col[0]) : e_col[0];
                const int i = i0 - 1 + er, j = j0 - 1 + ec;
                const int ic = i < 0 ? 0 : (i > Hs - 1 ? Hs - 1 : i), jc = j < 0 ? 0 : (j > Ws - 1 ? Ws - 1 : j);
                return xf + ((int64_t)(sy + rate * ic) * a.W + (sx + rate * jc)) * a.Cin;
            };
            u32x4 piece[LPT];
            auto load_pieces = [&](const unsigned short* px) {
#pragma unroll
                for (int k = 0; k < LPT; ++k) piece[k] = *reinterpret_cast<const u32x4*>(px + psrc[k]);
            };
            auto store_pieces = [&](int buf) {
#pragma unroll
                for (int k = 0; k < LPT; ++k) sA[buf * AUNITS + pdst[k]] = piece[k];
            };
            load_pieces(loader_pixel());
            store_pieces(par);
            __syncthreads();
            for (int t = 0; t < a.T; ++t) {
#pragma unroll
                for (int rg = 0; rg < NRG; ++rg) {
                    in_cur[rg] = inside_of(rg);
                    e_row[rg] += qS; e_col[rg] += rS;
                    if (e_col[rg] >= Wp) { e_col[rg] -= Wp; ++e_row[rg]; }
                }
                if constexpr (!(ABL & 1)) load_pieces(loader_pixel());
                f32x4 acc[NRG][2], accx[H16 ? NRG : 1][2];
                auto zero_acc = [&]() {
#pragma unroll
                    for (int rg = 0; rg < NRG; ++rg) { acc[rg][0] = (f32x4){0.f, 0.f, 0.f, 0.f}; acc[rg][1] = (f32x4){0.f, 0.f, 0.f, 0.f}; }
#pragma unroll
                    for (int rg = 0; rg < (H16 ? NRG : 1); ++rg) { accx[rg][0] = (f32x4){0.f, 0.f, 0.f, 0.f}; accx[rg][1] = (f32x4){0.f, 0.f, 0.f, 0.f}; }
                };
                if constexpr ((ABL & 2) != 0) zero_acc();
                else if (active) {
                    zero_acc();
                    const u32x4* ap = sA + par * AUNITS + q * 16 + l15;
                    constexpr bool XA2 = NWD <= 4;
                    bf16x8 xa[XA2 ? 2 : 1][NP][NRG];
                    auto load_x = [&](int s, bf16x8 (&dst)[NP][NRG]) {
#pragma unroll
                        for (int rg = 0; rg < NRG; ++rg)
#pragma unroll
                            for (int pp = 0; pp < NP; ++pp) dst[pp][rg] = __builtin_bit_cast(bf16x8, ap[((rg * NP + pp) * KS + s) * 64]);
                    };
                    if constexpr (XA2) load_x(0, xa[0]);
#pragma unroll
                    for (int s = 0; s < KS; ++s) {
                        if constexpr (XA2) { if (s + 1 < KS) load_x(s + 1, xa[(s + 1) & 1]); }
                        else load_x(s, xa[0]);
                        constexpr int XS = XA2 ? 1 : 0;
                        bf16x8 x0[NRG], x1[NRG], x2[NRG];
#pragma unroll
                        for (int rg = 0; rg < NRG; ++rg) {
                            x0[rg] = xa[s & XS][0][rg];
                            if (NP >= 2) x1[rg] = xa[s & XS][NP >= 2 ? 1 : 0][rg];
                            if (NP == 3) x2[rg] = xa[s & XS][NP - 1][rg];
                        }
#define AMS_XWR_TERM(WP, XB)                                                                                         \
    _Pragma("unroll") for (int rg = 0; rg < NRG; ++rg)                                                               \
        _Pragma("unroll") for (int tt = 0; tt < 2; ++tt)                                                             \
            acc[rg][tt] = __builtin_amdgcn_mfma_f32_16x16x32_bf16(wq[WP][s][tt], XB[rg], acc[rg][tt], 0, 0, 0);
#define AMS_XWR_TERM_H(ACC, WP, XB)                                                                                   \
    _Pragma("unroll") for (int rg = 0; rg < NRG; ++rg)                                                               \
        _Pragma("unroll") for (int tt = 0; tt < 2; ++tt)                                                             \
            ACC[H16 ? rg : 0][tt] = __builtin_amdgcn_mfma_f32_16x16x32_f16(__builtin_bit_cast(f16x8, wq[WP][s][tt]), __builtin_bit_cast(f16x8, XB[rg]), ACC[H16 ? rg : 0][tt], 0, 0, 0);
                        if constexpr (H16) {
                            AMS_XWR_TERM_H(accx, 1, x0)
                            AMS_XWR_TERM_H(accx, 0, x1)
                            AMS_XWR_TERM_H(acc, 0, x0)
                        } else {
                        if (NP == 3) {
                            AMS_XWR_TERM(NP - 1, x0)
                            AMS_XWR_TERM(0, x2)
                            AMS_XWR_TERM(1, x1)
                        }
                        if (NP >= 2) {
                            AMS_XWR_TERM(NP >= 2 ? 1 : 0, x0)
                            AMS_XWR_TERM(0, x1)
                        }
                        AMS_XWR_TERM(0, x0)
                        }
#undef AMS_XWR_TERM
#undef AMS_XWR_TERM_H
                    }
                }
                if (active || (ABL & 2) != 0)
#pragma unroll
                for (int rg = 0; rg < NRG; ++rg) {
                    const float lo = in_cur[rg] ? lo_e : 0.f, hi = in_cur[rg] ? hi_e : 0.f;
                    float* dst = ring + (sbase + 16 * rg) * PITCH + ring_lane;
                    const bool mirror = sbase == 0 && rg == 0 && l15 < MIRROR;
#pragma unroll
                    for (int tt = 0; tt < 2; ++tt) {
                        float4 v;
                        if constexpr (H16) acc[rg][tt] = combine_f16(acc[rg][tt], accx[H16 ? rg : 0][tt]);
                        const float4 bn = muladd4_pk(make_float4(acc[rg][tt][0], acc[rg][tt][1], acc[rg][tt][2], acc[rg][tt][3]), esc[tt], esh[tt]);
                        v.x = __builtin_amdgcn_fmed3f(bn.x, lo, hi);
                        v.y = __builtin_amdgcn_fmed3f(bn.y, lo, hi);
                        v.z = __builtin_amdgcn_fmed3f(bn.z, lo, hi);
                        v.w = __builtin_amdgcn_fmed3f(bn.w, lo, hi);
                        if constexpr (!(ABL & 16)) {
                        st4(dst + 16 * tt, v);
                        if (mirror) st4(dst + R * PITCH + 16 * tt, v);
                        }
                    }
                }
                store_pieces(par ^ 1);
                par ^= 1;
                sbase += STEP;
                if (sbase == R) sbase = 0;
                lap(0);
                __syncthreads();
                lap(1);
                if constexpr (TIMED) ++nstep;
            }
            __syncthreads();
            par = 0;
        }
        flush(0);
    } else {
        const int dt = tid - 64 * NWE;
        const int cg = dt % CG, pt = dt / CG;
        const int nch = cgi * NCB + 4 * cg;
        const bool chan_ok = nch < a.Cexp;
        const int nchc = chan_ok ? nch : 0;
        float4 wv[9];
#pragma unroll
        for (int k = 0; k < 9; ++k) wv[k] = ld4(a.w_dw + (int64_t)k * a.Cexp + nchc);
        const float4 dsc = ld4(a.sc_d + nchc), dsh = ld4(a.sh_d + nchc);
        const bool odd_cg = (cg & 1) != 0;
        const unsigned ych = a.y_fmt ? (unsigned)(nchc >> 3) * 32u + (odd_cg ? 16u : 0u) : (unsigned)nchc * 4u;
        int cb = (2 * R - 2 * Wp - 2 + pt * PX) % R;
        for (int item = group; item < a.items; item += a.groups) {
            int u1 = item;
            const int segx = u1 % a.nsx; u1 /= a.nsx;
            const int segy = u1 % a.nsy; u1 /= a.nsy;
            const int sub = u1 % (rate * rate);
            const int b = u1 / (rate * rate);
            const int sy = sub / rate, sx = sub - sy * rate;
            const int Hs = (a.H - sy + rate - 1) / rate, Ws = (a.W - sx + rate - 1) / rate;
            const int i0 = segy * a.SH, j0 = segx * a.SW;
            const bool live = i0 < Hs && j0 < Ws && chan_ok;
            const __amdgpu_buffer_rsrc_t yrsrc = __builtin_amdgcn_make_buffer_rsrc(a.y + (int64_t)b * a.H * a.W * a.Cexp, 0,
                                                                                   (int)((int64_t)a.H * a.W * a.Cexp * 4), 0x00020000);
            const int rmax = live ? (a.SH < Hs - i0 ? a.SH : Hs - i0) : 0, cmax = a.SW < Ws - j0 ? a.SW : Ws - j0;
            const int colpitch = rate * a.Cexp * 4, rowpitch = rate * a.W * a.Cexp * 4;
            const int off0 = ((sy + rate * (i0 - 1)) * a.W + sx + rate * (j0 - 1)) * a.Cexp * 4 + (int)ych;
            int d_row, d_col;
            { const int c0 = Wp - 1 + pt * PX; d_row = c0 / Wp; d_col = c0 - d_row * Wp; d_row -= 2; }
            const int wrapdelta = rowpitch - Wp * colpitch;
            const int stepdelta = qS * rowpitch + rS * colpitch;
            int d_off = d_row * rowpitch + d_col * colpitch + off0;
            __syncthreads();
            __syncthreads();
            constexpr int NH = (PX + 1) / 2;
            float4 vt[NH][3][PH + 2];
            auto load_row = [&](int di) {
#pragma unroll
                for (int hh = 0; hh < NH; ++hh) {
                    unsigned slot = (unsigned)(cb + di * Wp + 2 * hh);
                    slot = slot < (unsigned)R ? slot : slot - (unsigned)R;
                    slot = slot < (unsigned)R ? slot : slot - (unsigned)R;
                    const float* rp = ring + __umul24(slot, PITCH) + 4 * cg;
#pragma unroll
                    for (int jj = 0; jj < PH + 2; ++jj) vt[hh][di][jj] = (ABL & 4) ? wv[di] : ld4(rp + jj * PITCH);
                }
            };
            auto epilogue = [&](const float4 (&accs)[NH][PH], int row, int col, int off_c) {
#pragma unroll
                for (int hh = 0; hh < NH; ++hh) {
#pragma unroll
                    for (int u = 0; u < PH; ++u) {
                        const float4 a4 = accs[hh][u];
                        float4 o;
                        o.x = apply_act(a4.x * dsc.x + dsh.x, a.act_d); o.y = apply_act(a4.y * dsc.y + dsh.y, a.act_d);
                        o.z = apply_act(a4.z * dsc.z + dsh.z, a.act_d); o.w = apply_act(a4.w * dsc.w + dsh.w, a.act_d);
                        const bool ok = ((unsigned)(row - 1) < (unsigned)rmax) & ((unsigned)(col - 1) < (unsigned)cmax);
                        const unsigned off = (ok && !(ABL & 8)) ? (unsigned)off_c : 0xfffffff0u;
                        ++col; off_c += colpitch;
                        if (col >= Wp) { col -= Wp; ++row; off_c += wrapdelta; }
                        if (H16 && a.y_fmt) {
                            unsigned h2[2], l2[2];
                            split4_f16_mix(o, h2, l2);
                            const unsigned r0 = (unsigned)__builtin_amdgcn_update_dpp(0, (int)(odd_cg ? h2[0] : l2[0]), 0xB1, 0xF, 0xF, false);
                            const unsigned r1 = (unsigned)__builtin_amdgcn_update_dpp(0, (int)(odd_cg ? h2[1] : l2[1]), 0xB1, 0xF, 0xF, false);
                            const u32x4 d = {odd_cg ? r0 : h2[0], odd_cg ? r1 : h2[1], odd_cg ? l2[0] : r0, odd_cg ? l2[1] : r1};
                            __builtin_amdgcn_raw_buffer_store_b128(d, yrsrc, off, 0, 2);
                        } else {
                        const u32x4 d = {__float_as_uint(o.x), __float_as_uint(o.y), __float_as_uint(o.z), __float_as_uint(o.w)};
                        __builtin_amdgcn_raw_buffer_store_b128(d, yrsrc, off, 0, 0);
                        }
                    }
                }
            };
            for (int t = 0; t < a.T; ++t) {
                load_row(0);
                load_row(1);
                load_row(2);
                if constexpr (TIMED) { asm volatile("s_waitcnt lgkmcnt(0)" ::: "memory"); lap(2); }
                float4 acc4[NH][PH];
#pragma unroll
                for (int hh = 0; hh < NH; ++hh)
#pragma unroll
                    for (int u = 0; u < PH; ++u) acc4[hh][u] = make_float4(0.f, 0.f, 0.f, 0.f);
#pragma unroll
                for (int i = 0; i < ((ABL & 4) ? 1 : 3); ++i) {
#pragma unroll
                    for (int hh = 0; hh < NH; ++hh)
#pragma unroll
                        for (int u = 0; u < PH; ++u)
#pragma unroll
                            for (int j = 0; j < ((ABL & 4) ? 1 : 3); ++j) {
                                const float4 vv = vt[hh][i][u + j];
                                const float4 w4 = wv[i * 3 + j];
                                AMS_DW_FMA4(acc4[hh][u], vv, w4);
                            }
                }
                const int row0 = d_row, col0 = d_col, off0c = d_off;
                d_row += qS; d_col += rS; d_off += stepdelta;
                if (d_col >= Wp) { d_col -= Wp; ++d_row; d_off += wrapdelta; }
                cb += STEP;
                if (cb >= R) cb -= R;
                if constexpr (TIMED) {
#pragma unroll
                    for (int hh = 0; hh < NH; ++hh)
#pragma unroll
                        for (int u = 0; u < PH; ++u) asm volatile("" : "+v"(acc4[hh][u].x), "+v"(acc4[hh][u].y), "+v"(acc4[hh][u].z), "+v"(acc4[hh][u].w));
                    lap(3);
                }
                epilogue(acc4, row0, col0, off0c);
                lap(0);
                __syncthreads();
                lap(1);
                if constexpr (TIMED) ++nstep;
            }
        }
        flush(2);
    }
}

int xwr_phase_cycles(unsigned long long* h) {
    static unsigned long long rows[1024][8], z[1024][8];
    if (hipMemcpyFromSymbol(rows, HIP_SYMBOL(g_xwr_cycles), sizeof(rows)) != hipSuccess) return AMS_E_HIP;
    if (hipMemcpyToSymbol(HIP_SYMBOL(g_xwr_cycles), z, sizeof(z)) != hipSuccess) return AMS_E_HIP;
    for (int i = 0; i < 8; ++i) h[i] = 0;
    for (int r = 0; r < 1024; ++r)
        for (int i = 0; i < 8; ++i) h[i] += rows[r][i];
    return AMS_OK;
}

static size_t xwr_lds(int Kp, int np, int nwe, int nrg, int ring) {
    return (size_t)2 * nrg * np * (Kp / 8) * 16 * 16 + (size_t)(ring + 4) * (32 * nwe + 4) * 4;
}

template <int KS, int NP, int NWE, int NWD, int NRG, bool H16 = false, int ABL = 0>
static int launch_xwr_k(const XwrArgs& a, size_t lds, hipStream_t st) {
#ifdef AMS_MEASURE
    if constexpr (ABL == 0 && KS == 5 && NP == 2 && NWE == 4 && NWD == 4 && NRG == 2 && H16) {
        switch (knobs().xwr_abl) {
            case 1: return launch_xwr_k<KS, NP, NWE, NWD, NRG, H16, 1>(a, lds, st);
            case 2: return launch_xwr_k<KS, NP, NWE, NWD, NRG, H16, 2>(a, lds, st);
            case 3: return launch_xwr_k<KS, NP, NWE, NWD, NRG, H16, 3>(a, lds, st);
            case 4: return launch_xwr_k<KS, NP, NWE, NWD, NRG, H16, 4>(a, lds, st);
            case 8: return launch_xwr_k<KS, NP, NWE, NWD, NRG, H16, 8>(a, lds, st);
            case 12: return launch_xwr_k<KS, NP, NWE, NWD, NRG, H16, 12>(a, lds, st);
            case 16: return launch_xwr_k<KS, NP, NWE, NWD, NRG, H16, 16>(a, lds, st);
            case 19: return launch_xwr_k<KS, NP, NWE, NWD, NRG, H16, 19>(a, lds, st);
            case 28: return launch_xwr_k<KS, NP, NWE, NWD, NRG, H16, 28>(a, lds, st);
            case 31: return launch_xwr_k<KS, NP, NWE, NWD, NRG, H16, 31>(a, lds, st);
            default: break;
        }
        if (knobs().xwr_timed) return launch_xwr_k<KS, NP, NWE, NWD, NRG, H16, 32>(a, lds, st);
    }
#endif
    RUN_RC(func_allow_lds((const void*)xdw_wreg_kernel<KS, NP, NWE, NWD, NRG, H16, ABL>, lds));
    const int64_t nblocks = (int64_t)a.groups * a.cgroups;
    AMS_REQUIRE(nblocks > 0 && nblocks < 0x7fffffffLL, "expand_dw_wreg: bad grid");
    static const std::string nm = "xdw_wreg_kernel<" + std::to_string(KS) + ", " + std::to_string(NP) + ", " + std::to_string(NWE) + ", " +
                                  std::to_string(NWD) + ", " + std::to_string(NRG) + (H16 ? ", true, " : ", false, ") + std::to_string(ABL) + ">";
    note_kernel(nm.c_str());
    hipLaunchKernelGGL((xdw_wreg_kernel<KS, NP, NWE, NWD, NRG, H16, ABL>), dim3((unsigned)nblocks), dim3(64 * (NWE + NWD)), lds, st, a, (unsigned)nblocks);
    AMS_CHECK_LAUNCH();
    return AMS_OK;
}

template <int KS, int NP, bool H16 = false>
static int launch_xwr_w(const XwrArgs& a, int nwe, int nrg, size_t lds, hipStream_t st) {
    if (nwe == 8) return launch_xwr_k<KS, NP, 8, 4, 1, H16>(a, lds, st);
    if (nrg == 2) return launch_xwr_k<KS, NP, 4, 4, 2, H16>(a, lds, st);
    return launch_xwr_k<KS, NP, 4, 4, 1, H16>(a, lds, st);
}

int launch_expand_dw_wreg(const BlockCall& c, hipStream_t st) {
    RUN_RC(block_call_check("expand_dw_wreg", BK_WREG, c));
    const int B = c.B, H = c.H, W = c.W, Cin = c.Cin, Cexp = c.Cexp, rate = c.rate;
    const bool h16 = c.expand.np == AMS_NP_F16;
    const int np = h16 ? 2 : c.expand.np;
    AMS_REQUIRE((int64_t)H * W * Cexp * 4 < 0x7fffffffLL, "expand_dw_wreg: a frame of the output exceeds 2 GiB");
    int nwe = 4, nsy_force = 0, nsx_force = 0, groups_force = 0, nrg = 2;
    if (knobs().xwr_set) { const int* f = knobs().xwr; nwe = f[0]; nsy_force = f[1]; nsx_force = f[2]; groups_force = f[3]; nrg = f[4]; }
    if (nwe != 4 && nwe != 8) nwe = 4;
    if (nrg != 1 && nrg != 2) nrg = 2;
    if (nwe == 8) nrg = 1;
    const int step = 16 * nrg;
    const int Hs = (H + rate - 1) / rate, Ws = (W + rate - 1) / rate;
    const size_t budget = 160 * 1024 - 512;
    int nsx = nsx_force > 0 ? nsx_force : 1, SW, ring;
    for (;; ++nsx) {
        SW = (Ws + nsx - 1) / nsx;
        ring = (2 * (SW + 2) + 2 + 2 * step + step - 1) / step * step;
        if (xwr_lds(Cin, np, nwe, nrg, ring) <= budget || SW <= 1) break;
    }
    AMS_REQUIRE(xwr_lds(Cin, np, nwe, nrg, ring) <= budget, "expand_dw_wreg: no segment geometry fits LDS (W=%d rate=%d)", W, rate);
    nsx = (Ws + SW - 1) / SW;
    const int cgroups = (Cexp + 32 * nwe - 1) / (32 * nwe);
    int nsy = 1;
    if (nsy_force > 0) nsy = nsy_force;
    else
        while ((int64_t)B * rate * rate * cgroups * nsx * nsy < 512 && (Hs + nsy - 1) / nsy > 8) ++nsy;
    XwrArgs a;
    memset(&a, 0, sizeof(a));
    a.xs = c.x_parts; a.xs_plane = c.x_plane; a.B = B; a.H = H; a.W = W; a.Cin = Cin; a.wp = c.expand.panels; a.plane = c.expand.plane; a.sc_e = c.expand.scale;
    a.sh_e = c.expand.shift; a.act_e = c.expand.act; a.Cexp = Cexp; a.w_dw = c.dw.w; a.sc_d = c.dw.scale; a.sh_d = c.dw.shift; a.act_d = c.dw.act; a.y = c.y; a.rate = rate;
    a.SH = (Hs + nsy - 1) / nsy; a.SW = SW; a.Wp = SW + 2; a.T = ((a.SH + 2) * a.Wp + step - 1) / step; a.ring = ring;
    a.nsy = nsy; a.nsx = nsx; a.cgroups = cgroups;
    a.items = B * rate * rate * nsy * nsx;
    a.y_fmt = c.y_fmt;
    int64_t groups = groups_force > 0 ? groups_force : (512 + cgroups - 1) / cgroups;
    if (groups > a.items) groups = a.items;
    a.groups = (int)groups;
    const size_t lds = xwr_lds(Cin, np, nwe, nrg, ring);
    if (h16) {
        switch (Cin / 32) {
            case 2: return launch_xwr_w<2, 2, true>(a, nwe, nrg, lds, st);
            case 3: return launch_xwr_w<3, 2, true>(a, nwe, nrg, lds, st);
            default: return launch_xwr_w<5, 2, true>(a, nwe, nrg, lds, st);
        }
    }
    switch (Cin / 32) {
        case 2: return np == 3 ? launch_xwr_w<2, 3>(a, nwe, nrg, lds, st) : np == 1 ? launch_xwr_w<2, 1>(a, nwe, nrg, lds, st) : launch_xwr_w<2, 2>(a, nwe, nrg, lds, st);
        case 3: return np == 3 ? launch_xwr_w<3, 3>(a, nwe, nrg, lds, st) : np == 1 ? launch_xwr_w<3, 1>(a, nwe, nrg, lds, st) : launch_xwr_w<3, 2>(a, nwe, nrg, lds, st);
        default: return np == 3 ? launch_xwr_w<5, 3>(a, nwe, nrg, lds, st) : np == 1 ? launch_xwr_w<5, 1>(a, nwe, nrg, lds, st) : launch_xwr_w<5, 2>(a, nwe, nrg, lds, st);
    }
}

}
```

ams_amd/csrc/kernels.hpp:

```cpp
#pragma once
#include <vector>

#include "common.hpp"

struct ams_comm;

namespace ams {

struct ConvLayer;
struct BlockCall;

int func_allow_lds(const void* fn, size_t lds);
int func_blocks_per_cu(const void* fn, int threads, size_t lds, int* per_cu);
int device_cus(int* cus);
bool launch_table_needs_attr(int device, const void* fn, size_t lds);
struct Knobs {
    int blk_th = 0, blk_tw = 0;
    int fb_walk = -1;
    int fb_abl = 0;
    int xwr_timed = 0;
    int blk_timed = 0;
    int blk_hp = -1;
    char pw_force = 0; int pw_rm = 0, pw_nt = 0;
    int pw_percu = 0;
    bool pwx_no_tail = false;
    int pwx_rm = 0, pwx_nt = 0;
    int xwr_abl = 0;
    int pwh_abl = 0;
    bool pwh_set = false; int pwh_nw = 4, pwh_d = 2;
    bool xds_set = false; int xds[6] = {0, 0, 0, 0, 0, 0};
    bool xwr_set = false; int xwr[5] = {0, 0, 0, 0, 0};
    bool wg6_eight_waves = false;
    int wg6_split_cap = 0;
    int event_flags = -1;
    unsigned side_cu_mask = 0;
};
const Knobs& knobs();
int blk_phase_cycles(unsigned long long* h);
int xwr_phase_cycles(unsigned long long* h);
int xds_phase_cycles(unsigned long long* h);
int create_side_stream(hipStream_t* out);
int create_sync_event(hipEvent_t* out);

int comm_allreduce(ams_comm* c, void* p, size_t n, int dtype, hipStream_t st);

struct PwArgs {
    const float* x;
    int64_t M;
    int K;
    int Kw;
    int ldx;
    const float* w;
    int64_t w_sk, w_sn;
    int N;
    const float* img_bias;
    int64_t rows_per_img;
    const float* scale;
    const float* shift;
    int act;
    const float* res;
    int ldr;
    float* y;
    int ldy;
    uint16_t* ysplit;
    int64_t ysplit_plane;
    int ysplit_np;
    int ysplit_fmt;
    int y_skip_f32;
    int x_fmt;
    int red_mode;
    const float* red_center;
    const float* red_z; const float* red_scale; const float* red_shift; const float* red_mean; const float* red_rstd;
    int red_act;
    float* red_part;
    size_t red_part_floats;
    int* red_rows_out;
    const float* red_res; int red_ldr;
    int x_mode; int x_act;
    const float* x_v0; const float* x_v1; const float* x_v2; const float* x2;
    float* x_tmp;
};
static inline PwArgs pw_args(const float* x, int64_t M, int K, int ldx, const float* w, int N, float* y, int ldy) {
    PwArgs a;
    memset(&a, 0, sizeof(a));
    a.x = x; a.M = M; a.K = K; a.Kw = K; a.ldx = ldx; a.w = w; a.w_sk = N; a.w_sn = 1; a.N = N;
    a.rows_per_img = 1; a.act = AMS_ACT_NONE; a.y = y; a.ldy = ldy;
    return a;
}
int launch_pointwise(const PwArgs& a, hipStream_t st);
int pointwise_materialize_x(const PwArgs& a, PwArgs* b, hipStream_t st);
bool pointwise_stream_applies(const PwArgs& a);
bool pointwise_transforms_on_load(const PwArgs& a);
bool pointwise_split3_transforms_on_load(const PwArgs& a);

int launch_split_weights(const float* w, int64_t sk, int64_t sn, int K, int N, int Kp, uint16_t* hi, uint16_t* lo, hipStream_t st);
int launch_pointwise_split(const PwArgs& a, const uint16_t* whi, const uint16_t* wlo, int Kp, hipStream_t st);
int launch_split_weights3(const float* w, int64_t sk, int64_t sn, int K, int N, int Kp, uint16_t* hi, uint16_t* mid, uint16_t* lo,
                          hipStream_t st);
int launch_pointwise_split3(const PwArgs& a, const uint16_t* whi, const uint16_t* wmid, const uint16_t* wlo, int Kp, hipStream_t st);
struct SplitJob { const float* w; int64_t sk, sn; int K, N, Kp; uint16_t* p0; int64_t plane; int64_t first_block; int f16; };
int launch_split_batch(const SplitJob* jobs_dev, int njobs, int64_t total_blocks, hipStream_t st, int write_f16);
int launch_pointwise_split1(const PwArgs& a, const uint16_t* whi, int Kp, hipStream_t st);
int launch_split_weights_f16(const float* w, int64_t sk, int64_t sn, int K, int N, int Kp, uint16_t* hi, uint16_t* lo, hipStream_t st);
bool pointwise_f16_applies(const PwArgs& a);
int launch_pointwise_split_f16(const PwArgs& a, const uint16_t* whi, int64_t plane, int Kp, hipStream_t st);
int launch_pack_h2i(const float* x, int64_t M, int C, float* out, hipStream_t st);
bool pointwise_split_writes_parts(const PwArgs& a);
bool head_chain_supported(int KA, int NA, int KB, int NB, int KC, int NC);
int launch_head_chain(const float* x, int64_t M, int KA, const ConvLayer& A, const ConvLayer& B, const ConvLayer& C, const float* img_bias,
                      int64_t rows_per_img, int NC, float* y, hipStream_t st);

struct WgArgs {
    const float* x;  int ldx;  int K;
    const float* dy; int ldy;  int N;
    int64_t M;
    float* dw;
    float* scratch; size_t scratch_floats;
    int allow_split;
    int x_mode = 0, x_act = 0; const float* x_v0 = nullptr; const float* x_v1 = nullptr;
    int dy_mode = 0; const float* dy_v0 = nullptr; const float* dy_v1 = nullptr; const float* dy_v2 = nullptr; const float* dy2 = nullptr;
};
bool dw_project_supported(int C, int N, int stride, int rate);
int launch_dw_project(const BlockCall& c, hipStream_t st);
bool pointwise_wgrad_x6_applies(int64_t M, int K, int N, int ldx, int ldy);
int wgrad_x6_splits(int64_t M, int K, int N);
int launch_pointwise_wgrad_x6(const WgArgs& a, int splits, hipStream_t st);
size_t pointwise_wgrad_scratch(int64_t M, int K, int N);
int launch_pointwise_wgrad(const WgArgs& a, hipStream_t st);

struct FirstBlockPlan {
    int Ho, Wo, pt, pl;
    int tiles_y, tiles_x;
    int ity0, itx0, niy, nix;
    int interior_tiles, interior_grid;
    int border_tiles, border_grid;
    int border_walks;
};
int first_block_plan(int dtype, int B, int H, int W, bool h16, const int* occupancy, FirstBlockPlan* plan);
int launch_first_block(const BlockCall& c, hipStream_t st, FirstBlockPlan* plan_out = nullptr);

int launch_resize_u8(const uint8_t* src, int Hs, int Ws, int C, int mode, int swap_rb, uint8_t* dst, int H, int W, hipStream_t st);

int launch_stem(const void* frames, int dtype, int B, int H, int W, const float* w, int cout, const float* scale,
                const float* shift, int act, float pixel_scale, float* y, hipStream_t st);
int launch_stem_im2col(const void* frames, int dtype, int B, int H, int W, float pixel_scale, float* out, hipStream_t st);
int launch_depthwise(const float* x, int B, int H, int W, int C, const float* w, int stride, int rate,
                     const float* scale, const float* shift, int act, float* y, hipStream_t st);
int launch_depthwise_dgrad(const float* dy, int B, int H, int W, int C, const float* w, int stride, int rate,
                           float* dx, hipStream_t st);
size_t depthwise_fwd_bn_scratch(int B, int H, int W, int C, int rate);
int launch_depthwise_fwd_bn(const float* ze, int B, int H, int W, int C, const float* w, int rate, const float* scale, const float* shift, int act,
                            const float* center, float* zd, float* scratch, int* rows_out, hipStream_t st);
size_t depthwise_dgrad_bn_scratch(int B, int H, int W, int C);
int launch_depthwise_dgrad_bn(const float* dy, int B, int H, int W, int C, const float* w, int rate, const float* z, const float* scale,
                              const float* shift, int act, const float* mean, const float* rstd, float* out, float* scratch, int* rows_out,
                              hipStream_t st);
size_t depthwise_dgrad_bn2_scratch(int B, int H, int W, int C, int rate);
int launch_depthwise_dgrad_bn2(const float* dy, const float* zd, const float* cA, const float* cB, const float* cC, int B, int H, int W, int C,
                               const float* w, int rate, const float* ze, const float* scale, const float* shift, int act, const float* mean,
                               const float* rstd, float* out, float* scratch, int* rows_out, hipStream_t st);
size_t depthwise_fwd_bn2_scratch(int B, int H, int W, int C, int rate);
int launch_depthwise_fwd_bn2(const float* ze, int B, int H, int W, int C, const float* w, int rate, const float* scale, const float* shift, int act,
                             const float* center, float* zd, float* scratch, int* rows_out, hipStream_t st);
size_t depthwise_wgrad_scratch(int B, int H, int W, int C, int stride, int rate);
int launch_depthwise_wgrad(const float* x, const float* dy, int B, int H, int W, int C, int stride, int rate,
                           float* dw, float* scratch, size_t scratch_floats, hipStream_t st);

bool expand_dw_supported(int Cin, int Cexp, int stride, int rate);
size_t expand_dw_stats_scratch(int B, int H, int W, int Cexp, int stride);
int launch_expand_dw(const BlockCall& c, hipStream_t st, const float* stats_center = nullptr, float* stats_part = nullptr, int* stats_rows = nullptr);

bool xdw_train_supported(int Cin, int Cexp, int stride, int rate);
size_t xdw_train_scratch(int B, int H, int W, int Cin, int Cexp);
int xdw_train_blocks(int B, int H, int W, int Cexp);
int launch_xdw_fwd_stats(const float* x, int B, int H, int W, int Cin, const float* w_exp, int Cexp, const float* center, float* scratch,
                         int* rows_out, int64_t* stride_out, hipStream_t st);
int launch_xdw_bwd_reduce(const float* x, int B, int H, int W, int Cin, const float* w_exp, int Cexp, const float* sc_e, const float* sh_e,
                          const float* mean_e, const float* rstd_e, int act_e, const float* w_dw, int stride, const float* dz_d, float* scratch,
                          int* rows_out, int64_t* stride_out, hipStream_t st);
size_t xdw_stem_scratch(int B, int fH, int fW);
int launch_xdw_bwd_reduce_stem(const void* frames, int dtype, int B, int fH, int fW, float pixel_scale, const float* w_stem, const float* sc_e,
                               const float* sh_e, const float* mean_e, const float* rstd_e, int act_e, const float* w_dw, const float* dz_d,
                               float* scratch, int* rows_out, int64_t* stride_out, hipStream_t st);
int launch_xdw_bwd_dx(const float* x, int B, int H, int W, int Cin, const float* w_exp, int Cexp, const float* sc_e, const float* sh_e,
                      int act_e, const float* w_dw, int stride, const float* dz_d, const float* cA, const float* cB, const float* cC,
                      const float* res, float* dx, hipStream_t st, const float* red_z = nullptr, const float* red_mean = nullptr,
                      const float* red_rstd = nullptr, float* red_part = nullptr, int* red_rows_out = nullptr);
int launch_xdw_dwe(const float* G1, const float* xx_g0, int Cin, int Cexp, const float* w_exp, const float* cA, const float* cB, const float* cC,
                   float* dw, hipStream_t st);

int xx_stats_blocks(int64_t M);
size_t xx_stats_scratch_doubles(int64_t M, int Cin);
int launch_xx_gram(const float* x, int64_t M, int Cin, double* scratch, double* xx64, float* xx32, hipStream_t st);
int launch_expand_stats(const double* xx64, int Cin, const float* w_exp, int Cexp, double n, const float* center, const float* gamma,
                        const float* beta, float eps, float one_minus_decay, float* moving_mean, float* moving_var, float* scale, float* shift,
                        float* save_mean, float* save_rstd, double* sums, hipStream_t st);

bool block_fused_supported(int Cin, int Cexp, int Cout, int stride, int rate, bool residual);
int launch_block_fused(const BlockCall& c, hipStream_t st);
int launch_first_block_tiles(const BlockCall& c, hipStream_t st);
int launch_block_pack(const float* sc_e, const float* sh_e, const float* sc_d, const float* sh_d, const float* w_dw, int Cexp, float* out, hipStream_t st);

constexpr int AMS_NP_F16 = 4;
bool expand_dw_stream_supported(int Cin, int Cexp, int stride, int rate);
int launch_expand_dw_stream(const BlockCall& c, hipStream_t st);

int launch_expand_dw_wreg(const BlockCall& c, hipStream_t st);


size_t image_colsum_scratch(int B, int C);
int launch_global_mean(const float* x, int B, int64_t HW, int C, float* y, float* scratch, hipStream_t st);
int launch_image_colsum(const float* x, int B, int64_t HW, int C, int ldx, float* out, float* scratch, hipStream_t st);

size_t colstats_scratch(int64_t M, int C);
int launch_colstats(const float* z, int64_t M, int C, const float* center, double* sums , float* scratch,
                    hipStream_t st);
int launch_colstats_f64(const float* z, int64_t M, int C, const float* center, double* sums , hipStream_t st);
int launch_bn_finalize(const double* sums, double n, int C, const float* center, const float* gamma, const float* beta,
                       float eps, float one_minus_decay, float* moving_mean, float* moving_var, float* scale,
                       float* shift, float* save_mean, float* save_rstd, hipStream_t st);
int launch_bn_fold(const float* gamma, const float* beta, const float* mean, const float* var, float eps, int C,
                   float* scale, float* shift, hipStream_t st);
int launch_bn_act(const float* z, int64_t M, int C, const float* scale, const float* shift, int act, const float* res,
                  float* a, hipStream_t st);
int launch_bn_bwd_reduce(const float* da, const float* z, int64_t M, int C, const float* scale, const float* shift,
                         int act, const float* mean, const float* rstd, double* sums, float* scratch, hipStream_t st);
int launch_bn_bwd_coef(const double* sums, double n, int C, const float* gamma, const float* mean, const float* rstd,
                       float* coefA, float* coefB, float* coefC, float* dgamma, float* dbeta, hipStream_t st);
int launch_bn_param_grads(const double* sums, int C, float* dgamma, float* dbeta, hipStream_t st);
int launch_colstats_bn(const float* z, int64_t M, int C, const float* center, double* sums, float* scratch, double n,
                       const float* gamma, const float* beta, float eps, float one_minus_decay, float* moving_mean,
                       float* moving_var, float* scale, float* shift, float* save_mean, float* save_rstd, hipStream_t st);
int launch_bn_bwd_reduce_coef(const float* da, const float* z, int64_t M, int C, const float* scale, const float* shift, int act,
                              const float* mean, const float* rstd, double* sums, float* scratch, double n, const float* gamma,
                              float* coefA, float* coefB, float* coefC, float* dgamma, float* dbeta, hipStream_t st);
int launch_bn_bwd_apply(const float* da, const float* z, int64_t M, int C, const float* scale, const float* shift, int act,
                        const float* coefA, const float* coefB, const float* coefC, float* dz, hipStream_t st);
int launch_colsum(const float* x, int64_t M, int C, int ldx, float* out, float* scratch, hipStream_t st);
int launch_adam(float* p, const float* g, float* m, float* v, const uint8_t* mask, int64_t n, float lr_t, float b1,
                float b2, float eps, hipStream_t st);
struct ReduceJobs {
    static constexpr int kMax = 32;
    int n = 0;
    const float* part[kMax]; float* out[kMax]; int splits[kMax]; int64_t count[kMax]; int64_t stride[kMax]; int first_block[kMax];
    bool add(const float* p, int splits_, int64_t count_, float* o, int64_t stride_) {
        if (n >= kMax) return false;
        part[n] = p; splits[n] = splits_; count[n] = count_; out[n] = o; stride[n] = stride_ > 0 ? stride_ : count_; ++n;
        return true;
    }
};
int launch_reduce_batch(ReduceJobs& jobs, hipStream_t st);
int launch_reduce_splits(const float* part, int splits, int64_t n, float* out, hipStream_t st, int64_t stride = 0);
int launch_bn_fwd_finalize_partials(const float* part, int rows, int64_t row_stride, int C, double* sums, double n, const float* center,
                                    const float* gamma, const float* beta, float eps, float one_minus_decay, float* moving_mean,
                                    float* moving_var, float* scale, float* shift, float* save_mean, float* save_rstd, hipStream_t st);
int launch_bn_bwd_finalize_partials(const float* part, int rows, int64_t row_stride, int C, double* sums, double n, const float* gamma,
                                    const float* mean, const float* rstd, float* coefA, float* coefB, float* coefC, float* dgamma,
                                    float* dbeta, hipStream_t st);
int launch_partials_to_sums(const float* part, int rows, int64_t row_stride, int C, double* sums, hipStream_t st);
int launch_fill(float* p, int64_t n, float v, hipStream_t st);
int launch_round_bf16(float* p, int64_t n, hipStream_t st);
int launch_copy(float* dst, const float* src, int64_t n, hipStream_t st);
size_t pack_fp16_scratch(int64_t n);
int launch_pack_fp16(const float* p, const uint8_t* mask, int64_t n, uint16_t* out, int64_t* n_out, int64_t* counts, hipStream_t st);
int64_t delta_segments(int64_t mask_bytes);
int launch_apply_delta(const uint8_t* payload, int64_t payload_bytes, const ams_delta_var* vars_dev, int n_vars, int64_t mask_bytes,
                       float* params, int64_t n_params, float* stats, int64_t n_stats, int64_t* counts, int64_t* n_applied, int32_t* status,
                       hipStream_t st);
int launch_delta_count(const uint8_t* payload, int64_t readable, int nseg, int64_t* counts, hipStream_t st);
size_t q8_encode_table_words(int n_vars);
int launch_encode_delta_q8(const uint8_t* mask, int64_t* table_dev, int n_vars, int64_t mask_bytes, const float* params, const float* stats,
                           float* base_params, float* base_stats, int advance_base, int64_t* work, uint8_t* payload, int64_t cap,
                           int64_t* payload_bytes, int32_t* status, hipStream_t st);
int launch_apply_delta_q8(const uint8_t* payload, int64_t payload_bytes, const ams_delta_var* vars_dev, int n_vars, int64_t mask_bytes,
                          float* params, int64_t n_params, float* stats, int64_t n_stats, int64_t* counts, int64_t* n_applied, int32_t* status,
                          hipStream_t st);
size_t select_scratch();
int launch_select_changed(const float* after, const float* before, int64_t n, int64_t k, ams_select_result* result, int64_t* scratch,
                          hipStream_t st);
int launch_select_apply(float* params, const float* before, int64_t n, float cut, uint8_t* mask, int64_t* n_kept, hipStream_t st);
int64_t encode_segments(int64_t mask_bytes);
int launch_encode_delta(const uint8_t* mask, const int64_t* table_dev, int n_vars, int64_t mask_bytes, const float* params, const float* stats,
                        int64_t* work, uint8_t* payload, int64_t cap, int64_t* payload_bytes, hipStream_t st);

struct HeadCall;
struct LossObjective;
int launch_upsample_argmax(const HeadCall& c, int32_t* labels, int64_t* conf, double* loss, hipStream_t st, int per_frame = 0,
                           int labels_u8 = 0 );
int launch_ce_grad(const HeadCall& c, const double* loss_and_count, float* dlogits, int ldd, hipStream_t st, float empty_val = 0.f);
bool ce_loss_grad_supported(int w, int W);
size_t ce_loss_grad_scratch(int B, int h, int w, int K);
int launch_ce_loss_grad(const HeadCall& c, const LossObjective& o, double* loss, float* scratch, hipStream_t st);
int launch_ce_combine(const HeadCall& c, const double* loss_and_count, const float* scratch, float* dlogits, int ldd, hipStream_t st,
                      float empty_val = 0.f);
struct WeightRange { const float* w; int64_t n; };
int weights_beyond(const std::vector<WeightRange>& jobs, float limit, float low, int* flags_dev , int* over_host,
                   hipStream_t st);
int launch_l2_regularizer(const float* p, float* g, const uint8_t* mask, int64_t n, int n_vars, float coef, double* part_scratch ,
                          double* loss, hipStream_t st);
int launch_cross_confusion(const uint8_t* a, const uint8_t* b, int64_t n, const int32_t* lut ,
                           int K, int64_t* conf, hipStream_t st);

int confidence_stats_len();
int launch_upsample_confidence(const HeadCall& c, uint8_t* conf_u8, float* conf_f32, int64_t* stats, hipStream_t st);

int soft_metric_stats_len(int K);
int launch_upsample_soft_metric(const HeadCall& c, const LossObjective& o, int64_t* stats, float* p_f32, float* ce_f32, hipStream_t st);

struct MiningBuffers { float* keys = nullptr; uint8_t* labels = nullptr; uint32_t* hist = nullptr; ams_mining_result* result = nullptr; };
size_t loss_mining_scratch(int B, int H, int W);
MiningBuffers loss_mining_buffers(void* scratch, int B, int H, int W);
int mining_top_k_check(const char* who, float top_k);
int launch_mining_keys(const HeadCall& c, const LossObjective& o, float top_k, const MiningBuffers& m, hipStream_t st);
int launch_mining_select(int64_t n, float top_k, const MiningBuffers& m, hipStream_t st);
int launch_mining_relabel(const uint8_t* labels, int64_t n, const MiningBuffers& m, hipStream_t st);
int launch_loss_mining(const HeadCall& c, const LossObjective& o, float top_k, const MiningBuffers& m, hipStream_t st);

int launch_replay_gather(const uint8_t* frame_slots, int64_t frame_stride, const uint8_t* label_slots, int64_t label_stride, int capacity, int Hs,
                         int Ws, const ams_replay_sample* samples_dev, const ams_replay_sample* samples_host, int B, int H, int W,
                         uint8_t* frames_out, uint8_t* labels_out, hipStream_t st);
int launch_replay_gather_rows(const float* slots, int64_t slot_stride, int capacity, int th, int tw, int C, const ams_replay_sample* samples_dev,
                              const ams_replay_sample* samples_host, int B, float* out, hipStream_t st);
int launch_replay_gather_logits(const float* slots, int64_t slot_stride, int capacity, int Hs, int Ws, int C, const ams_replay_sample* samples_dev,
                                const ams_replay_sample* samples_host, int B, int H, int W, float* out, hipStream_t st);
int launch_replay_gather_logits_lowres(const float* slots, int64_t slot_stride, int capacity, int lh, int lw, int C, int Hs, int Ws,
                                       const ams_replay_sample* samples_dev, const ams_replay_sample* samples_host, int B, int H, int W, float* out,
                                       hipStream_t st);
int launch_replay_pack_logits(const float* in, int th, int tw, int NC, const int32_t* idx_host, int K, float* out, hipStream_t st);
int launch_teacher_labels_from_logits(const float* logits, int64_t slot_stride, int n, int lh, int lw, int NC, int Hs, int Ws, uint8_t* out,
                                      int64_t out_stride, hipStream_t st);
int launch_cross_confusion_pairs(const uint8_t* label_slots, int64_t label_stride, int capacity, int64_t n, const int32_t* pairs_dev,
                                 const int32_t* pairs_host, int n_pairs, const int32_t* lut , int K, int64_t* conf,
                                 hipStream_t st);

int launch_render_views(const uint8_t* frames, const void* student, int student_dtype, const uint8_t* teacher, int B, int H, int W, int K,
                        const uint8_t* tables, const ams_render_out* out, hipStream_t st);

}
```

ams_amd/hip.py:

```python
from __future__ import annotations

import ctypes as C
import os
from pathlib import Path

_HERE = Path(__file__).resolve().parent
LIB_PATH = _HERE / "libams_hip.so"

ABI_VERSION = 6

ROLE_STEM, ROLE_EXPAND, ROLE_DEPTHWISE, ROLE_PROJECT, ROLE_POOL_CONV, ROLE_ASPP, ROLE_CONCAT_PROJ, ROLE_LOGITS = range(8)
ACT_NONE, ACT_RELU, ACT_RELU6 = 0, 1, 2
DT_F32, DT_U8, DT_I32, DT_F64 = 0, 1, 3, 4
MODE_FROZEN, MODE_LIVE = 0, 1
OPT_MATMUL = 1
RESIZE_NEAREST, RESIZE_LINEAR = 0, 1
OPT_FUSE_EXPAND_DW = 2
OPT_FUSE_DW_PROJECT = 3
OPT_FUSE_FIRST_BLOCK = 4
OPT_FUSE_EXPAND_DW_STREAM = 5
OPT_FUSE_BLOCK = 6
OPT_LATE_SUBBATCH = 7
OPT_BLOCK_X6 = 8
OPT_DUAL_STREAM = 10
OPT_TRAIN_RECOMPUTE = 11
OPT_FUSE_DGRAD_BN = 16
OPT_FUSE_GEMM_RED = 17
OPT_EMULATE_BF16_STORAGE = 15
OPT_DUAL_AUTOTUNE = 12
OPT_DUAL_PARTS = 13
OPT_NAN_GRADS = 18
OPT_TRAIN_FWD_F16 = 24
OPT_SOFT_TEACHER = 25
OPT_FUSE_HEAD = 26
TLOGITS_FULL, TLOGITS_SELECTED = 0, 1
TLOGITS_LAYOUTS = {"full": TLOGITS_FULL, "selected": TLOGITS_SELECTED}
OPT_OVERLAP_WGRAD = 19
OPT_OVERLAP_HEAD = 20
OPT_STREAM_MIN_ROWS = 21
OPT_FUSE_OPERAND_BN = 22
OPT_WGRAD_FORK_EVERY = 23
MATMUL_F32, MATMUL_SPLIT_BF16, MATMUL_SPLIT_BF16_X6, MATMUL_BF16, MATMUL_SPLIT_F16 = 0, 1, 2, 3, 4
MATMUL_DEFAULT = MATMUL_SPLIT_F16
(REGION_PARAMS, REGION_STATS, REGION_GRADS, REGION_ADAM_M, REGION_ADAM_V, REGION_FROZEN, REGION_BN_SYNC,
 REGION_LOGITS) = range(8)


class LayerDesc(C.Structure):
    _fields_ = [("role", C.c_int32), ("cin", C.c_int32), ("cout", C.c_int32), ("stride", C.c_int32),
                ("rate", C.c_int32), ("act", C.c_int32), ("residual_from", C.c_int32), ("bn_eps", C.c_float),
                ("w_off", C.c_int64), ("gamma_off", C.c_int64), ("beta_off", C.c_int64), ("mean_off", C.c_int64),
                ("var_off", C.c_int64)]


class StudentConfig(C.Structure):
    _fields_ = [("abi_version", C.c_int32), ("height", C.c_int32), ("width", C.c_int32), ("max_batch", C.c_int32),
                ("num_classes", C.c_int32), ("n_selected", C.c_int32), ("class_indices", C.c_int32 * 32),
                ("n_layers", C.c_int32), ("trainable", C.c_int32), ("act_dtype", C.c_int32),
                ("n_trainable", C.c_int64), ("n_stats", C.c_int64), ("bn_decay", C.c_float),
                ("bn_eps_frozen", C.c_float), ("pixel_scale", C.c_float)]


class DeltaVar(C.Structure):
    _fields_ = [("region", C.c_int32), ("reserved", C.c_int32), ("offset", C.c_int64), ("count", C.c_int64), ("mask_offset", C.c_int64)]


class RenderOut(C.Structure):
    _fields_ = [("colour_student", C.c_void_p), ("overlay_student", C.c_void_p), ("colour_teacher", C.c_void_p), ("overlay_teacher", C.c_void_p),
                ("ignore_mask", C.c_void_p), ("cross_mask", C.c_void_p)]


class FirstBlockPlan(C.Structure):
    _fields_ = [(n, C.c_int32) for n in ("out_h", "out_w", "pad_top", "pad_left", "tiles_y", "tiles_x", "ity0", "itx0", "niy", "nix",
                                         "interior_tiles", "interior_grid", "border_tiles", "border_grid", "border_walks")]


class MiningResult(C.Structure):
    _fields_ = [("threshold", C.c_float), ("valid", C.c_int64), ("rank", C.c_int64), ("kept", C.c_int64)]


MINING_KEYS_OFFSET = 24832

RENDER_VIEWS = tuple(f[0] for f in RenderOut._fields_)
RENDER_TABLE_BYTES = 1120
CONFIDENCE_BINS = 32

DELTA_OK, DELTA_BAD_SIZE, DELTA_BAD_PADDING, DELTA_BAD_SCALE, DELTA_Q8_NONFINITE = 0, 1, 2, 3, 4
DELTA_MAX_VARS = 1024

ALLREDUCE_CB = C.CFUNCTYPE(C.c_int, C.c_void_p, C.c_size_t, C.c_size_t, C.c_int32)

_vp, _i32, _i64, _f32, _sz = C.c_void_p, C.c_int32, C.c_int64, C.c_float, C.c_size_t

SIGNATURES = {
    "ams_last_error": (C.c_char_p, []),
    "ams_abi_version": (C.c_int, []),
    "ams_device_info": (C.c_int, [C.c_char_p, _sz, C.POINTER(_i32), C.POINTER(_i64)]),
    "ams_student_arena_bytes": (C.c_int, [C.POINTER(StudentConfig), C.POINTER(LayerDesc), C.POINTER(_sz)]),
    "ams_student_create": (C.c_int, [C.POINTER(StudentConfig), C.POINTER(LayerDesc), _vp, _sz, C.POINTER(_vp)]),
    "ams_student_destroy": (None, [_vp]),
    "ams_student_region": (C.c_int, [_vp, _i32, C.POINTER(_sz), C.POINTER(_sz)]),
    "ams_student_lowres_size": (C.c_int, [_vp, C.POINTER(_i32), C.POINTER(_i32)]),
    "ams_student_layer_tensor": (C.c_int, [_vp, _i32, _i32, C.POINTER(C.c_size_t), C.POINTER(C.c_size_t)]),
    "ams_student_freeze": (C.c_int, [_vp, _vp]),
    "ams_student_predict": (C.c_int, [_vp, _vp, _i32, _i32, _i32, _vp, _vp]),
    "ams_student_predict_with_metric": (C.c_int, [_vp, _vp, _i32, _i32, _i32, _vp, _vp, _vp, _vp, _vp]),
    "ams_student_predict_frames": (C.c_int, [_vp, _vp, _i32, _i32, _i32, _vp, _vp, _vp, _vp, _vp]),
    "ams_student_predict_frames_u8": (C.c_int, [_vp, _vp, _i32, _i32, _i32, _vp, _vp, _vp, _vp, _vp]),
    "ams_student_confidence": (C.c_int, [_vp, _i32, _vp, _vp, _vp, _vp, _vp]),
    "ams_student_soft_metric": (C.c_int, [_vp, _i32, _vp, _vp, _i32, _i32, _vp, _vp, _vp, _vp]),
    "ams_cross_confusion": (C.c_int, [_vp, _vp, _i64, _vp, _vp]),
    "ams_cross_confusion_pairs": (C.c_int, [_vp, _vp, _i64, _i32, _i64, _vp, _vp, _i32, _vp, _vp]),
    "ams_student_soft_metric_layout": (C.c_int, [_vp, _i32, _vp, _vp, _i32, _i32, _vp, _vp, _vp, _vp, _i32]),
    "ams_replay_pack_logits": (C.c_int, [_vp, _i32, _i32, _i32, C.POINTER(_i32), _i32, _i32, _vp, _vp]),
    "ams_replay_gather": (C.c_int, [_vp, _i64, _vp, _i64, _i32, _i32, _i32, _vp, _vp, _i32, _i32, _i32, _vp, _vp, _vp]),
    "ams_replay_gather_f32": (C.c_int, [_vp, _i64, _i32, _i32, _i32, _i32, _vp, _vp, _i32, _vp, _vp]),
    "ams_replay_gather_logits": (C.c_int, [_vp, _i64, _i32, _i32, _i32, _i32, _vp, _vp, _i32, _i32, _i32, _vp, _vp]),
    "ams_replay_gather_logits_lowres": (C.c_int, [_vp, _i64, _i32, _i32, _i32, _i32, _i32, _i32, _vp, _vp, _i32, _i32, _i32, _vp, _vp]),
    "ams_teacher_labels_from_logits": (C.c_int, [_vp, _i64, _i32, _i32, _i32, _i32, _i32, _i32, _vp, _i64, _vp]),
    "ams_render_table_bytes": (_sz, []),
    "ams_render_views": (C.c_int, [_vp, _vp, _i32, _vp, _i32, _i32, _i32, _i32, _vp, C.POINTER(RenderOut), _vp]),
    "ams_student_train_step": (C.c_int, [_vp, _vp, _i32, _vp, _i32, _f32, _vp, _vp, _vp]),
    "ams_student_train_step_dp": (C.c_int, [_vp, _vp, _i32, _vp, _i32, _i32, _f32, _vp, _vp, ALLREDUCE_CB, _vp, _vp]),
    "ams_comm_unique_id": (C.c_int, [_vp, _sz]),
    "ams_comm_create": (C.c_int, [_vp, _sz, _i32, _i32, C.POINTER(_vp)]),
    "ams_comm_destroy": (None, [_vp]),
    "ams_comm_stats": (C.c_int, [_vp, C.POINTER(_i32), C.POINTER(_i32), C.POINTER(_i64), C.POINTER(_i64)]),
    "ams_comm_set_timing": (C.c_int, [_vp, _i32]),
    "ams_comm_timing_read": (C.c_int, [_vp, C.POINTER(C.c_double), C.POINTER(C.c_double), C.POINTER(_i64)]),
    "ams_comm_allreduce": (C.c_int, [_vp, _vp, _sz, _i32, _vp]),
    "ams_student_train_step_rccl": (C.c_int, [_vp, _vp, _i32, _vp, _i32, _i32, _f32, _vp, _vp, _vp, _vp]),
    "ams_student_set_option": (C.c_int, [_vp, _i32, _i32]),
    "ams_student_feed_teacher_logits": (C.c_int, [_vp, _vp, _i32, _i32]),
    "ams_student_feed_teacher_logits_layout": (C.c_int, [_vp, _vp, _i32, _i32, _i32]),
    "ams_student_f16_fallback_layers": (C.c_int, [_vp, C.POINTER(_i32)]),
    "ams_student_set_regularizer": (C.c_int, [_vp, _vp, _i32, _f32]),
    "ams_student_set_kd": (C.c_int, [_vp, _f32, _f32]),
    "ams_student_set_loss_weights": (C.c_int, [_vp, C.POINTER(_f32), _i32, _f32]),
    "ams_student_profile": (C.c_int, [_vp, _i32]),
    "ams_student_profile_read": (C.c_int, [_vp, C.c_char_p, _sz, C.POINTER(_sz)]),
    "ams_student_get_adam_step": (C.c_int, [_vp, C.POINTER(_i64)]),
    "ams_student_set_adam_step": (C.c_int, [_vp, _i64]),
    "ams_pack_masked_fp16": (C.c_int, [_vp, _vp, _i64, _vp, _vp, _vp, _sz, _vp]),
    "ams_pack_masked_fp16_scratch": (_sz, [_i64]),
    "ams_student_apply_delta": (C.c_int, [_vp, _vp, _i64, C.POINTER(DeltaVar), _i32, _vp, _vp, _vp, _sz, _vp]),
    "ams_student_apply_delta_scratch": (_sz, [C.POINTER(DeltaVar), _i32]),
    "ams_select_changed": (C.c_int, [_vp, _vp, _i64, _i64, _vp, _vp, _sz, _vp]),
    "ams_select_changed_scratch": (_sz, [_i64]),
    "ams_select_apply": (C.c_int, [_vp, _vp, _i64, _f32, _vp, _vp, _vp]),
    "ams_student_encode_delta": (C.c_int, [_vp, _vp, C.POINTER(DeltaVar), _i32, _vp, _i64, _vp, _vp, _sz, _vp]),
    "ams_student_encode_delta_scratch": (_sz, [C.POINTER(DeltaVar), _i32]),
    "ams_student_encode_delta_q8": (C.c_int, [_vp, _vp, C.POINTER(DeltaVar), _i32, _vp, _vp, _i32, _vp, _i64, _vp, _vp, _vp, _sz, _vp]),
    "ams_student_encode_delta_q8_scratch": (_sz, [C.POINTER(DeltaVar), _i32]),
    "ams_student_apply_delta_q8": (C.c_int, [_vp, _vp, _i64, C.POINTER(DeltaVar), _i32, _vp, _vp, _vp, _sz, _vp]),
    "ams_student_apply_delta_q8_scratch": (_sz, [C.POINTER(DeltaVar), _i32]),
    "ams_k_stem_conv": (C.c_int, [_vp, _i32, _i32, _i32, _i32, _vp, _i32, _vp, _vp, _i32, _f32, _vp, _vp]),
    "ams_k_depthwise3x3": (C.c_int, [_vp, _i32, _i32, _i32, _i32, _vp, _i32, _i32, _vp, _vp, _i32, _vp, _vp]),
    "ams_k_pointwise": (C.c_int, [_vp, _i64, _i32, _vp, _i32, _i32, _vp, _i64, _vp, _vp, _i32, _vp, _vp, _vp]),
    "ams_k_pointwise_split": (C.c_int, [_vp, _i64, _i32, _vp, _i32, _vp, _vp, _i32, _vp, _vp, _vp, _sz, _vp]),
    "ams_k_pointwise_split3": (C.c_int, [_vp, _i64, _i32, _vp, _i32, _vp, _vp, _i32, _vp, _vp, _vp, _sz, _vp]),
    "ams_k_pack_h2i": (C.c_int, [_vp, _i64, _i32, _vp, _vp]),
    "ams_k_pointwise_split_f16": (C.c_int, [_vp, _i64, _i32, _vp, _i32, _vp, _vp, _i32, _vp, _vp, _vp, _sz, _vp, _vp, _vp]),
    "ams_k_expand_dw_stream_f16": (C.c_int, [_vp, _i32, _i32, _i32, _i32, _vp, _vp, _vp, _i32, _vp, _i32, _vp, _vp, _vp, _vp, _sz, _i32, _i32, _vp]),
    "ams_ingest_resize_u8": (C.c_int, [_vp, _i32, _i32, _i32, _i32, _i32, _vp, _i32, _i32, _vp]),
    "ams_k_dw_project": (C.c_int, [_vp, _i32, _i32, _i32, _i32, _vp, _i32, _vp, _vp, _vp, _i32, _vp, _vp, _vp, _vp, _vp, _sz, _vp]),
    "ams_k_block_fused": (C.c_int, [_vp, _i32, _i32, _i32, _i32, _vp, _vp, _vp, _i32, _vp, _i32, _vp, _vp, _vp, _i32, _vp, _vp, _i32, _vp, _vp, _sz, _vp]),
    "ams_k_block_fused_f16": (C.c_int, [_vp, _i32, _i32, _i32, _i32, _vp, _vp, _vp, _i32, _vp, _i32, _vp, _vp, _vp, _i32, _vp, _vp, _i32, _vp, _vp, _sz, _vp]),
    "ams_k_first_block_scratch": (_sz, [_i32]),
    "ams_k_first_block": (C.c_int, [_vp, _i32, _i32, _i32, _i32, _f32, _vp, _vp, _vp, _vp, _vp, _vp, _vp, _vp, _vp, _vp, _i32, _vp, _sz,
                                    C.POINTER(FirstBlockPlan), _vp]),
    "ams_k_first_block_tiles": (C.c_int, [_vp, _i32, _i32, _i32, _i32, _f32, _vp, _vp, _vp, _vp, _vp, _vp, _vp, _vp, _vp, _vp, _vp]),
    "ams_k_first_block_plan": (C.c_int, [_i32, _i32, _i32, _i32, _i32, C.POINTER(_i32), C.POINTER(FirstBlockPlan)]),
    "ams_k_expand_dw": (C.c_int, [_vp, _i32, _i32, _i32, _i32, _vp, _vp, _vp, _i32, _vp, _i32, _i32, _vp, _vp, _vp, _vp]),
    "ams_k_expand_dw_stream": (C.c_int, [_vp, _i32, _i32, _i32, _i32, _vp, _vp, _vp, _i32, _vp, _i32, _vp, _vp, _vp, _vp, _sz, _i32, _i32, _vp]),
    "ams_k_global_mean": (C.c_int, [_vp, _i32, _i64, _i32, _vp, _vp, _sz, _vp]),
    "ams_k_global_mean_scratch": (_sz, [_i32, _i32]),
    "ams_k_upsample_argmax": (C.c_int, [_vp, _i32, _i32, _i32, _i32, C.POINTER(_i32), _i32, _i32, _i32, _vp, _vp, _vp,
                                        _vp, _vp]),
    "ams_k_upsample_confidence": (C.c_int, [_vp, _i32, _i32, _i32, _i32, C.POINTER(_i32), _i32, _i32, _i32, _vp, _vp, _vp, _vp, _vp]),
    "ams_confidence_stats_len": (_sz, []),
    "ams_k_upsample_soft_metric": (C.c_int, [_vp, _i32, _i32, _i32, _i32, C.POINTER(_i32), _i32, _i32, _i32, _vp, _vp, _i32, _i32, _vp, _vp, _vp, _vp]),
    "ams_k_upsample_soft_metric_layout": (C.c_int, [_vp, _i32, _i32, _i32, _i32, _i32, C.POINTER(_i32), _i32, _i32, _i32, _vp, _vp, _i32, _i32, _i32, _vp, _vp, _vp, _vp]),
    "ams_soft_metric_stats_len": (_sz, [_i32]),
    "ams_k_ce_grad": (C.c_int, [_vp, _i32, _i32, _i32, _i32, C.POINTER(_i32), _i32, _i32, _i32, _vp, _vp, _vp, _vp]),
    "ams_k_ce_loss_grad": (C.c_int, [_vp, _i32, _i32, _i32, _i32, C.POINTER(_i32), _i32, _i32, _i32, _vp, _vp, _vp, _vp, _sz, _vp]),
    "ams_k_ce_loss_grad_scratch": (_sz, [_i32, _i32, _i32, _i32]),
    "ams_k_ce_loss_grad_soft": (C.c_int, [_vp, _i32, _i32, _i32, _i32, C.POINTER(_i32), _i32, _i32, _i32, _vp, _vp, _i32, _i32, _vp, _vp, _vp, _sz, _vp]),
    "ams_k_ce_loss_grad_soft_layout": (C.c_int, [_vp, _i32, _i32, _i32, _i32, _i32, C.POINTER(_i32), _i32, _i32, _i32, _vp, _vp, _i32, _i32, _i32, _vp, _vp, _vp, _sz, _vp]),
    "ams_k_ce_loss_grad_kd": (C.c_int, [_vp, _i32, _i32, _i32, _i32, _i32, C.POINTER(_i32), _i32, _i32, _i32, _vp, _vp, _i32, _i32, _i32, _vp, _vp, _vp, _sz, _vp,
                                        _f32, _f32]),
    "ams_k_ce_loss_grad_weighted": (C.c_int, [_vp, _i32, _i32, _i32, _i32, _i32, C.POINTER(_i32), _i32, _i32, _i32, _vp, _vp, _i32, _i32, _i32, _vp, _vp, _vp, _sz,
                                              _vp, _f32, _f32, C.POINTER(_f32), _f32]),
    "ams_k_ce_loss_grad_mined": (C.c_int, [_vp, _i32, _i32, _i32, _i32, _i32, C.POINTER(_i32), _i32, _i32, _i32, _vp, _vp, _i32, _i32, _i32, _vp, _vp, _vp, _sz,
                                           _vp, _f32, _f32, C.POINTER(_f32), _f32, _f32, _vp, _vp, _vp, _vp, _sz]),
    "ams_k_loss_mining_scratch": (_sz, [_i32, _i32, _i32]),
    "ams_student_set_loss_mining": (C.c_int, [_vp, _f32, _vp, _sz]),
    "ams_student_mining_result": (C.c_int, [_vp, _vp, _vp]),
    "ams_debug_launch_table_needs_attr": (C.c_int, [_i32, C.c_uint64, _sz]),
    "ams_debug_reload_knobs": (C.c_int, []),
    "ams_debug_phase_cycles": (C.c_int, [C.c_int32, C.POINTER(C.c_uint64), C.c_int32]),
    "ams_k_pointwise_wgrad": (C.c_int, [_vp, _vp, _i64, _i32, _i32, _vp, _vp, _sz, _vp]),
    "ams_k_pointwise_wgrad_scratch": (_sz, [_i64, _i32, _i32]),
    "ams_k_pointwise_wgrad_split": (C.c_int, [_vp, _vp, _i64, _i32, _i32, _vp, _vp, _sz, _vp]),
    "ams_k_depthwise3x3_dgrad": (C.c_int, [_vp, _i32, _i32, _i32, _i32, _vp, _i32, _i32, _vp, _vp]),
    "ams_k_depthwise3x3_wgrad": (C.c_int, [_vp, _vp, _i32, _i32, _i32, _i32, _i32, _i32, _vp, _vp, _sz, _vp]),
    "ams_k_pointwise_xform": (C.c_int, [_vp, _i64, _i32, _vp, _i32, _i32, _i32, _i32, _i32, _vp, _vp, _vp, _vp, _vp, _vp, _vp, _sz, _vp]),
    "ams_k_pointwise_wgrad_xform": (C.c_int, [_vp, _vp, _i64, _i32, _i32, _i32, _i32, _i32, _vp, _vp, _i32, _vp, _vp, _vp, _vp, _vp, _vp, _sz, _vp]),
    "ams_k_pointwise_red": (C.c_int, [_vp, _i64, _i32, _vp, _i32, _i32, _i32, _i32, _vp, _vp, _vp, _vp, _vp, _vp, _i32, _vp, _vp, _vp, _sz,
                                     C.POINTER(_i32), _vp, _sz, _vp]),
    "ams_k_depthwise3x3_fwd_bn_scratch": (_sz, [_i32, _i32, _i32, _i32, _i32]),
    "ams_k_depthwise3x3_fwd_bn": (C.c_int, [_vp, _i32, _i32, _i32, _i32, _vp, _i32, _vp, _vp, _i32, _vp, _vp, _vp, _sz, C.POINTER(_i32), _vp]),
    "ams_k_depthwise3x3_dgrad_bn_scratch": (_sz, [_i32, _i32, _i32, _i32]),
    "ams_k_depthwise3x3_dgrad_bn": (C.c_int, [_vp, _i32, _i32, _i32, _i32, _vp, _i32, _vp, _vp, _vp, _i32, _vp, _vp, _vp, _vp, _sz,
                                             C.POINTER(_i32), _vp]),
    "ams_k_depthwise3x3_fwd_bn_tiles_scratch": (_sz, [_i32, _i32, _i32, _i32, _i32]),
    "ams_k_depthwise3x3_fwd_bn_tiles": (C.c_int, [_vp, _i32, _i32, _i32, _i32, _vp, _i32, _vp, _vp, _i32, _vp, _vp, _vp, _sz, C.POINTER(_i32), _vp]),
    "ams_k_depthwise3x3_dgrad_bn_apply_scratch": (_sz, [_i32, _i32, _i32, _i32, _i32]),
    "ams_k_depthwise3x3_dgrad_bn_apply": (C.c_int, [_vp, _vp, _vp, _vp, _vp, _i32, _i32, _i32, _i32, _vp, _i32, _vp, _vp, _vp, _i32, _vp, _vp, _vp, _vp, _sz,
                                                    C.POINTER(_i32), _vp]),
    "ams_k_xx_gram_scratch": (_sz, [_i64, _i32]),
    "ams_k_xx_gram": (C.c_int, [_vp, _i64, _i32, _vp, _sz, _vp, _vp, _vp]),
    "ams_k_expand_stats": (C.c_int, [_vp, _i32, _vp, _i32, C.c_double, _vp, _vp, _vp, _f32, _f32, _vp, _vp, _vp, _vp, _vp, _vp, _vp, _vp]),
    "ams_k_xdw_train_scratch": (_sz, [_i32, _i32, _i32, _i32, _i32]),
    "ams_k_xdw_fwd_stats": (C.c_int, [_vp, _i32, _i32, _i32, _i32, _vp, _i32, _vp, _vp, _sz, C.POINTER(_i32), C.POINTER(_i64), _vp]),
    "ams_k_xdw_bwd_reduce": (C.c_int, [_vp, _i32, _i32, _i32, _i32, _vp, _i32, _vp, _vp, _vp, _vp, _i32, _vp, _i32, _vp, _vp, _sz,
                                      C.POINTER(_i32), C.POINTER(_i64), _vp]),
    "ams_k_xdw_bwd_dx": (C.c_int, [_vp, _i32, _i32, _i32, _i32, _vp, _i32, _vp, _vp, _i32, _vp, _i32, _vp, _vp, _vp, _vp, _vp, _vp, _vp]),
    "ams_k_xdw_stem_scratch": (_sz, [_i32, _i32, _i32]),
    "ams_k_xdw_bwd_reduce_stem": (C.c_int, [_vp, _i32, _i32, _i32, _i32, _f32, _vp, _vp, _vp, _vp, _vp, _i32, _vp, _vp, _vp, _sz,
                                           C.POINTER(_i32), C.POINTER(_i64), _vp]),
    "ams_k_xdw_dwe": (C.c_int, [_vp, _vp, _i32, _i32, _vp, _vp, _vp, _vp, _vp, _vp]),
    "ams_k_adam": (C.c_int, [_vp, _vp, _vp, _vp, _vp, _i64, _f32, _f32, _f32, _f32, _vp]),
}

_lib = None


class AmsHipError(RuntimeError):
    pass


def lib() -> C.CDLL:
    global _lib
    if _lib is not None:
        return _lib
    path = Path(os.environ.get("AMS_HIP_LIB", str(LIB_PATH)))
    if not path.exists():
        raise AmsHipError(
            "HIP library %s not found: the AMS student has no CPU fallback. Build it with "
            "`make -C ams_amd/csrc` (hipcc --offload-arch=gfx950)." % path)
    import torch
    handle = C.CDLL(str(path))
    for name, (res, args) in SIGNATURES.items():
        fn = getattr(handle, name)
        fn.restype = res
        fn.argtypes = args
    if handle.ams_abi_version() != ABI_VERSION:
        raise AmsHipError("libams_hip.so ABI %d, binding expects %d" % (handle.ams_abi_version(), ABI_VERSION))
    _lib = handle
    return handle


def check(rc: int, what: str = "") -> None:
    if rc != 0:
        msg = lib().ams_last_error()
        raise AmsHipError("%s failed (%d): %s" % (what or "libams_hip call", rc, msg.decode() if msg else "?"))
```

include/ams_hip.h:

```cpp
#ifndef AMS_HIP_H
#define AMS_HIP_H

#include <stddef.h>
#include <stdint.h>

#ifdef __cplusplus
extern "C" {
#endif

#define AMS_ABI_VERSION 6

enum {
    AMS_OK = 0,
    AMS_E_INVALID = -1,
    AMS_E_HIP = -2,
    AMS_E_STATE = -3,
    AMS_E_NOMEM = -4
};

enum {
    AMS_ROLE_STEM = 0,
    AMS_ROLE_EXPAND = 1,
    AMS_ROLE_DEPTHWISE = 2,
    AMS_ROLE_PROJECT = 3,
// ... 39 lines not shown
    float bn_decay;
    float bn_eps_frozen;
    float pixel_scale;
} ams_student_config;

typedef struct ams_student ams_student;

enum {
    AMS_REGION_PARAMS = 0,
    AMS_REGION_STATS = 1,
    AMS_REGION_GRADS = 2,
    AMS_REGION_ADAM_M = 3,
    AMS_REGION_ADAM_V = 4,
    AMS_REGION_FROZEN = 5,
    AMS_REGION_BN_SYNC = 6,
    AMS_REGION_LOGITS = 7
};

const char* ams_last_error(void);
int ams_abi_version(void);
int ams_device_info(char* name_out, size_t name_cap, int32_t* n_cu, int64_t* hbm_bytes);

int ams_student_arena_bytes(const ams_student_config* cfg, const ams_layer_desc* layers, size_t* bytes_out);
int ams_student_create(const ams_student_config* cfg, const ams_layer_desc* layers, void* arena_dev,
                       size_t arena_bytes, ams_student** out);
void ams_student_destroy(ams_student* s);
int ams_student_region(const ams_student* s, int32_t region, size_t* offset_bytes, size_t* n_elems);
int ams_student_lowres_size(const ams_student* s, int32_t* h, int32_t* w);
int ams_student_layer_tensor(const ams_student* s, int32_t layer, int32_t which, size_t* offset_bytes, size_t* n_elems);

int ams_student_freeze(ams_student* s, void* stream);

int ams_student_predict(ams_student* s, const void* frames_dev, int32_t frames_dtype, int32_t batch,
                        int32_t mode, int32_t* labels_out_dev, void* stream);

int ams_student_predict_with_metric(ams_student* s, const void* frames_dev, int32_t frames_dtype, int32_t batch,
                                    int32_t mode, const uint8_t* teacher_dev, int32_t* labels_out_dev,
                                    int64_t* conf_mat_dev, double* loss_dev, void* stream);

int ams_student_predict_frames(ams_student* s, const void* frames_dev, int32_t frames_dtype, int32_t batch, int32_t mode,
                               const uint8_t* teacher_dev, int32_t* labels_out_dev, int64_t* conf_mats_dev, double* losses_dev, void* stream);

int ams_student_predict_frames_u8(ams_student* s, const void* frames_dev, int32_t frames_dtype, int32_t batch, int32_t mode,
                                  const uint8_t* teacher_dev, uint8_t* labels_out_dev, int64_t* conf_mats_dev, double* losses_dev, void* stream);

int ams_student_confidence(ams_student* s, int32_t batch, const uint8_t* teacher_dev, uint8_t* conf_u8, float* conf_f32, int64_t* stats,
                           void* stream);

int ams_student_soft_metric(ams_student* s, int32_t batch, const uint8_t* teacher_dev, const float* teacher_logits_dev, int32_t th, int32_t tw,
                            int64_t* stats, float* p_f32, float* ce_f32, void* stream);
int ams_student_soft_metric_layout(ams_student* s, int32_t batch, const uint8_t* teacher_dev, const float* teacher_logits_dev, int32_t th, int32_t tw,
                                   int64_t* stats, float* p_f32, float* ce_f32, void* stream, int32_t layout);

int ams_cross_confusion(const ams_student* s, const uint8_t* labels_dev, int64_t n_pixels, int64_t* conf_mat_dev,
                        void* stream);

int ams_student_train_step(ams_student* s, const void* frames_dev, int32_t frames_dtype, const uint8_t* teacher_dev,
                           int32_t batch, float lr, const uint8_t* mask_dev, double* loss_dev, void* stream);

int ams_student_f16_fallback_layers(const ams_student* s, int32_t* n_layers);

int ams_student_feed_teacher_logits(ams_student* s, const float* teacher_logits_dev, int32_t th, int32_t tw);

enum { AMS_TLOGITS_FULL = 0, AMS_TLOGITS_SELECTED = 1 };

int ams_student_feed_teacher_logits_layout(ams_student* s, const float* teacher_logits_dev, int32_t th, int32_t tw, int32_t layout);
int ams_student_set_regularizer(ams_student* s, const uint8_t* reg_mask_dev, int32_t n_vars, float coef);

int ams_student_set_kd(ams_student* s, float temperature, float alpha);

int ams_student_set_loss_weights(ams_student* s, const float* class_weights_host , int32_t n, float conf_gamma);

typedef struct ams_mining_result {
    float threshold;
    int64_t valid;
    int64_t rank;
    int64_t kept;
} ams_mining_result;
#define AMS_MINING_KEYS_OFFSET 24832
size_t ams_k_loss_mining_scratch(int32_t B, int32_t H, int32_t W);
int ams_student_set_loss_mining(ams_student* s, float top_k, void* scratch_dev, size_t scratch_bytes);
int ams_student_mining_result(ams_student* s, ams_mining_result* out_host, void* stream);

typedef int (*ams_allreduce_cb)(void* user, size_t offset_bytes, size_t count, int32_t dtype);
int ams_student_train_step_dp(ams_student* s, const void* frames_dev, int32_t frames_dtype,
                              const uint8_t* teacher_dev, int32_t batch, int32_t global_batch, float lr,
                              const uint8_t* mask_dev, double* loss_dev, ams_allreduce_cb cb, void* user,
                              void* stream);

typedef struct ams_comm ams_comm;
int ams_comm_unique_id(uint8_t* id_out, size_t cap);
int ams_comm_create(const uint8_t* id, size_t id_len, int32_t rank, int32_t world, ams_comm** out);
void ams_comm_destroy(ams_comm* c);
int ams_comm_stats(const ams_comm* c, int32_t* rank, int32_t* world, int64_t* calls, int64_t* bytes);
int ams_comm_set_timing(ams_comm* c, int32_t enable);
int ams_comm_timing_read(ams_comm* c, double* total_ms, double* max_ms, int64_t* spans);
int ams_comm_allreduce(ams_comm* c, void* buf_dev, size_t count, int32_t dtype, void* stream);
int ams_student_train_step_rccl(ams_student* s, const void* frames_dev, int32_t frames_dtype, const uint8_t* teacher_dev,
                                int32_t batch, int32_t global_batch, float lr, const uint8_t* mask_dev, double* loss_dev,
                                ams_comm* comm, void* stream);

enum { AMS_OPT_FUSE_HEAD = 26 ,
       AMS_OPT_SOFT_TEACHER = 25 ,
       AMS_OPT_TRAIN_FWD_F16 = 24 ,
       AMS_OPT_WGRAD_FORK_EVERY = 23 ,
       AMS_OPT_FUSE_OPERAND_BN = 22 ,
       AMS_OPT_NAN_GRADS = 18 ,
       AMS_OPT_OVERLAP_WGRAD = 19 ,
       AMS_OPT_OVERLAP_HEAD = 20 ,
       AMS_OPT_STREAM_MIN_ROWS = 21 ,
       AMS_OPT_DUAL_AUTOTUNE = 12 ,
       AMS_OPT_DUAL_PARTS = 13 ,
       AMS_OPT_EMULATE_BF16_STORAGE = 15 ,
       AMS_OPT_FUSE_DGRAD_BN = 16 ,
       AMS_OPT_FUSE_GEMM_RED = 17 ,
       AMS_OPT_TRAIN_RECOMPUTE = 11 ,
       AMS_OPT_DUAL_STREAM = 10 ,
       AMS_OPT_BLOCK_X6 = 8 ,
       AMS_OPT_LATE_SUBBATCH = 7 ,
       AMS_OPT_FUSE_BLOCK = 6 ,
       AMS_OPT_FUSE_FIRST_BLOCK = 4 ,
       AMS_OPT_FUSE_DW_PROJECT = 3 ,
       AMS_OPT_FUSE_EXPAND_DW_STREAM = 5 ,
       AMS_OPT_MATMUL = 1, AMS_OPT_FUSE_EXPAND_DW = 2  };
enum { AMS_MATMUL_F32 = 0, AMS_MATMUL_SPLIT_BF16 = 1, AMS_MATMUL_SPLIT_BF16_X6 = 2,
       AMS_MATMUL_SPLIT_F16 = 4 ,
       AMS_MATMUL_BF16 = 3  };
int ams_student_set_option(ams_student* s, int32_t option, int32_t value);

int ams_student_profile(ams_student* s, int32_t enable);
int ams_student_profile_read(ams_student* s, char* buf, size_t cap, size_t* needed);

int ams_student_get_adam_step(const ams_student* s, int64_t* t);
int ams_student_set_adam_step(ams_student* s, int64_t t);

int ams_pack_masked_fp16(const float* params_dev, const uint8_t* mask_dev, int64_t n, uint16_t* out_half_dev,
                         int64_t* n_out_dev, int64_t* scratch_dev, size_t scratch_elems, void* stream);
size_t ams_pack_masked_fp16_scratch(int64_t n);

typedef struct ams_delta_var {
    int32_t region;
    int32_t reserved;
    int64_t offset;
    int64_t count;
    int64_t mask_offset;
} ams_delta_var;

#define AMS_DELTA_MAX_VARS 1024

enum {
    AMS_DELTA_OK = 0,
    AMS_DELTA_BAD_SIZE = 1,
    AMS_DELTA_BAD_PADDING = 2,
    AMS_DELTA_BAD_SCALE = 3,
    AMS_DELTA_Q8_NONFINITE = 4
};

int ams_student_apply_delta(ams_student* s, const uint8_t* payload_dev, int64_t payload_bytes, const ams_delta_var* vars_host,
                            int32_t n_vars, int64_t* n_applied_dev, int32_t* status_dev, int64_t* scratch_dev, size_t scratch_elems,
                            void* stream);
size_t ams_student_apply_delta_scratch(const ams_delta_var* vars_host, int32_t n_vars);

typedef struct ams_select_result {
    float a;
    float b;
    int64_t nan_count;
} ams_select_result;
int ams_select_changed(const float* after_dev, const float* before_dev, int64_t n, int64_t k, ams_select_result* result_dev,
                       int64_t* scratch_dev, size_t scratch_elems, void* stream);
size_t ams_select_changed_scratch(int64_t n);

int ams_select_apply(float* params_dev, const float* before_dev, int64_t n, float cut, uint8_t* mask_dev, int64_t* n_kept_dev, void* stream);

int ams_student_encode_delta(ams_student* s, const uint8_t* mask_dev, const ams_delta_var* vars_host, int32_t n_vars, uint8_t* payload_dev,
                             int64_t payload_cap, int64_t* payload_bytes_dev, int64_t* scratch_dev, size_t scratch_elems, void* stream);
size_t ams_student_encode_delta_scratch(const ams_delta_var* vars_host, int32_t n_vars);

int ams_student_encode_delta_q8(ams_student* s, const uint8_t* mask_dev, const ams_delta_var* vars_host, int32_t n_vars,
                                float* base_params_dev, float* base_stats_dev, int32_t advance_base, uint8_t* payload_dev,
                                int64_t payload_cap, int64_t* payload_bytes_dev, int32_t* status_dev, int64_t* scratch_dev,
                                size_t scratch_elems, void* stream);
size_t ams_student_encode_delta_q8_scratch(const ams_delta_var* vars_host, int32_t n_vars);

int ams_student_apply_delta_q8(ams_student* s, const uint8_t* payload_dev, int64_t payload_bytes, const ams_delta_var* vars_host,
                               int32_t n_vars, int64_t* n_applied_dev, int32_t* status_dev, int64_t* scratch_dev, size_t scratch_elems,
                               void* stream);
size_t ams_student_apply_delta_q8_scratch(const ams_delta_var* vars_host, int32_t n_vars);

typedef struct ams_replay_sample {
    int32_t slot;
    int32_t th, tw;
    int32_t top, left;
    int32_t flip;
} ams_replay_sample;

int ams_replay_gather(const uint8_t* frame_slots_dev, int64_t frame_slot_stride, const uint8_t* label_slots_dev, int64_t label_slot_stride,
                      int32_t capacity, int32_t src_h, int32_t src_w, const ams_replay_sample* samples_dev, const ams_replay_sample* samples_host,
                      int32_t batch, int32_t H, int32_t W, uint8_t* frames_out_dev, uint8_t* labels_out_dev, void* stream);

int ams_replay_gather_f32(const float* slots_dev, int64_t slot_stride, int32_t capacity, int32_t th, int32_t tw, int32_t channels,
                          const ams_replay_sample* samples_dev, const ams_replay_sample* samples_host, int32_t batch, float* out_dev, void* stream);

int ams_replay_gather_logits(const float* slots_dev, int64_t slot_stride, int32_t capacity, int32_t src_h, int32_t src_w, int32_t channels,
                             const ams_replay_sample* samples_dev, const ams_replay_sample* samples_host, int32_t batch, int32_t H, int32_t W,
                             float* out_dev, void* stream);

int ams_replay_gather_logits_lowres(const float* slots_dev, int64_t slot_stride, int32_t capacity, int32_t lh, int32_t lw, int32_t channels,
                                    int32_t src_h, int32_t src_w, const ams_replay_sample* samples_dev, const ams_replay_sample* samples_host,
                                    int32_t batch, int32_t H, int32_t W, float* out_dev, void* stream);

int ams_replay_pack_logits(const float* logits_dev, int32_t th, int32_t tw, int32_t num_classes, const int32_t* class_idx_host, int32_t K,
                           int32_t layout, float* slot_dev, void* stream);

int ams_teacher_labels_from_logits(const float* logits_dev, int64_t slot_stride, int32_t n, int32_t lh, int32_t lw, int32_t num_classes, int32_t Hs,
                                   int32_t Ws, uint8_t* labels_out_dev, int64_t out_stride, void* stream);

int ams_cross_confusion_pairs(const ams_student* s, const uint8_t* label_slots_dev, int64_t label_slot_stride, int32_t capacity, int64_t n_pixels,
                              const int32_t* pairs_dev, const int32_t* pairs_host, int32_t n_pairs, int64_t* conf_mats_dev, void* stream);

#define AMS_RENDER_TABLE_BYTES 1120

typedef struct ams_render_out {
    uint8_t* colour_student;
    uint8_t* overlay_student;
    uint8_t* colour_teacher;
    uint8_t* overlay_teacher;
    uint8_t* ignore_mask;
    uint8_t* cross_mask;
} ams_render_out;

size_t ams_render_table_bytes(void);

int ams_render_views(const uint8_t* frames_dev, const void* student_dev, int32_t student_dtype, const uint8_t* teacher_dev, int32_t batch, int32_t H,
                     int32_t W, int32_t K, const uint8_t* tables_dev, const ams_render_out* out, void* stream);


int ams_k_stem_conv(const void* frames, int32_t frames_dtype, int32_t B, int32_t H, int32_t W, const float* w ,
                    int32_t cout, const float* scale, const float* shift, int32_t act, float pixel_scale,
                    float* y , void* stream);

int ams_k_depthwise3x3(const float* x, int32_t B, int32_t H, int32_t W, int32_t C, const float* w ,
                       int32_t stride, int32_t rate, const float* scale, const float* shift, int32_t act,
                       float* y, void* stream);

int ams_k_pointwise(const float* x, int64_t M, int32_t K, const float* w, int32_t N, int32_t trans_w,
                    const float* img_bias, int64_t rows_per_img, const float* scale, const float* shift,
                    int32_t act, const float* res, float* y, void* stream);

int ams_k_pointwise_split(const float* x, int64_t M, int32_t K, const float* w, int32_t N, const float* scale,
                          const float* shift, int32_t act, const float* res, float* y, uint16_t* panels,
                          size_t panel_elems, void* stream);

int ams_k_pointwise_split3(const float* x, int64_t M, int32_t K, const float* w, int32_t N, const float* scale,
                           const float* shift, int32_t act, const float* res, float* y, uint16_t* panels,
                           size_t panel_elems, void* stream);

int ams_k_expand_dw(const float* x, int32_t B, int32_t H, int32_t W, int32_t Cin, const float* w_exp, const float* scale_e,
                    const float* shift_e, int32_t Cexp, const float* w_dw, int32_t stride, int32_t rate, const float* scale_d,
                    const float* shift_d, float* y, void* stream);

int ams_k_block_fused(const float* x, int32_t B, int32_t H, int32_t W, int32_t Cin, const float* w_exp, const float* scale_e, const float* shift_e,
                      int32_t Cexp, const float* w_dw, int32_t stride, const float* scale_d, const float* shift_d, const float* w_proj, int32_t Cout,
                      const float* scale_p, const float* shift_p, int32_t residual, float* y, uint16_t* panels, size_t panel_elems, void* stream);

int ams_k_expand_dw_stream(const float* x, int32_t B, int32_t H, int32_t W, int32_t Cin, const float* w_exp, const float* scale_e,
                           const float* shift_e, int32_t Cexp, const float* w_dw, int32_t rate, const float* scale_d,
                           const float* shift_d, float* y, uint16_t* panels, size_t panel_elems, int32_t parts, int32_t presplit,
                           void* stream);

int ams_k_pack_h2i(const float* x, int64_t M, int32_t C, float* out, void* stream);
int ams_k_block_fused_f16(const float* x, int32_t B, int32_t H, int32_t W, int32_t Cin, const float* w_exp, const float* scale_e,
                          const float* shift_e, int32_t Cexp, const float* w_dw, int32_t stride, const float* scale_d, const float* shift_d,
                          const float* w_proj, int32_t Cout, const float* scale_p, const float* shift_p, int32_t residual, float* y,
                          uint16_t* panels, size_t panel_elems, void* stream);
int ams_k_pointwise_split_f16(const float* x, int64_t M, int32_t K, const float* w, int32_t N, const float* scale, const float* shift,
                              int32_t act, const float* res, float* y, uint16_t* panels, size_t panel_elems, float* x_h2i, uint16_t* y_parts,
                              void* stream);
int ams_k_expand_dw_stream_f16(const float* x, int32_t B, int32_t H, int32_t W, int32_t Cin, const float* w_exp, const float* scale_e,
                               const float* shift_e, int32_t Cexp, const float* w_dw, int32_t rate, const float* scale_d,
                               const float* shift_d, float* y, uint16_t* panels, size_t panel_elems, int32_t presplit, int32_t y_h2i,
                               void* stream);

int ams_k_dw_project(const float* e, int32_t B, int32_t H, int32_t W, int32_t C, const float* w_dw, int32_t rate,
                     const float* scale_d, const float* shift_d, const float* w_proj, int32_t N, const float* scale_p,
                     const float* shift_p, const float* res, float* y, uint16_t* panels, size_t panel_elems, void* stream);

typedef struct ams_first_block_plan {
    int32_t out_h, out_w, pad_top, pad_left;
    int32_t tiles_y, tiles_x;
    int32_t ity0, itx0, niy, nix;
    int32_t interior_tiles, interior_grid;
    int32_t border_tiles, border_grid;
    int32_t border_walks;
} ams_first_block_plan;
size_t ams_k_first_block_scratch(int32_t form);
int ams_k_first_block(const void* frames, int32_t frames_dtype, int32_t B, int32_t H, int32_t W, float pixel_scale, const float* w_stem,
                      const float* scale_s, const float* shift_s, const float* w_dw, const float* scale_d, const float* shift_d, const float* w_proj,
                      const float* scale_p, const float* shift_p, float* y, int32_t form, uint16_t* panels, size_t panel_elems,
                      ams_first_block_plan* plan_out, void* stream);
int ams_k_first_block_tiles(const void* frames, int32_t frames_dtype, int32_t B, int32_t H, int32_t W, float pixel_scale, const float* w_stem,
                            const float* scale_s, const float* shift_s, const float* w_dw, const float* scale_d, const float* shift_d,
                            const float* w_proj, const float* scale_p, const float* shift_p, float* y, void* stream);
int ams_k_first_block_plan(int32_t frames_dtype, int32_t B, int32_t H, int32_t W, int32_t form, const int32_t* occupancy, ams_first_block_plan* plan_out);

enum { AMS_RESIZE_NEAREST = 0, AMS_RESIZE_LINEAR = 1 };
int ams_ingest_resize_u8(const uint8_t* src, int32_t Hs, int32_t Ws, int32_t C, int32_t mode, int32_t swap_rb, uint8_t* dst,
                         int32_t H, int32_t W, void* stream);

int ams_k_global_mean(const float* x, int32_t B, int64_t HW, int32_t C, float* y, float* scratch, size_t scratch_floats,
                      void* stream);
size_t ams_k_global_mean_scratch(int32_t B, int32_t C);

int ams_k_upsample_argmax(const float* logits , int32_t B, int32_t h, int32_t w, int32_t NC,
                          const int32_t* class_idx_host, int32_t K, int32_t H, int32_t W, const uint8_t* teacher,
                          int32_t* labels_out, int64_t* conf_mat, double* loss, void* stream);

#define AMS_CONFIDENCE_BINS 32
int ams_k_upsample_confidence(const float* logits , int32_t B, int32_t h, int32_t w, int32_t NC,
                              const int32_t* class_idx_host, int32_t K, int32_t H, int32_t W, const uint8_t* teacher,
                              uint8_t* conf_u8, float* conf_f32, int64_t* stats, void* stream);
size_t ams_confidence_stats_len(void);

int ams_k_upsample_soft_metric(const float* logits , int32_t B, int32_t h, int32_t w, int32_t NC,
                               const int32_t* class_idx_host, int32_t K, int32_t H, int32_t W, const uint8_t* teacher,
                               const float* teacher_logits , int32_t th, int32_t tw, int64_t* stats, float* p_f32,
                               float* ce_f32, void* stream);
int ams_k_upsample_soft_metric_layout(const float* logits , int32_t B, int32_t h, int32_t w, int32_t ld, int32_t NC,
                                      const int32_t* class_idx_host, int32_t K, int32_t H, int32_t W, const uint8_t* teacher,
                                      const float* teacher_logits, int32_t th, int32_t tw, int32_t layout, int64_t* stats, float* p_f32,
                                      float* ce_f32, void* stream);
size_t ams_soft_metric_stats_len(int32_t K);

int ams_k_ce_grad(const float* logits, int32_t B, int32_t h, int32_t w, int32_t NC, const int32_t* class_idx_host,
                  int32_t K, int32_t H, int32_t W, const uint8_t* teacher, const double* loss_and_count_dev,
                  float* dlogits, void* stream);

int ams_k_ce_loss_grad(const float* logits, int32_t B, int32_t h, int32_t w, int32_t NC, const int32_t* class_idx_host,
                       int32_t K, int32_t H, int32_t W, const uint8_t* teacher, double* loss_dev, float* dlogits,
                       float* scratch, size_t scratch_floats, void* stream);
size_t ams_k_ce_loss_grad_scratch(int32_t B, int32_t h, int32_t w, int32_t K);
int ams_k_ce_loss_grad_soft(const float* logits, int32_t B, int32_t h, int32_t w, int32_t NC, const int32_t* class_idx_host,
                            int32_t K, int32_t H, int32_t W, const uint8_t* teacher, const float* teacher_logits, int32_t th, int32_t tw,
                            double* loss_dev, float* dlogits, float* scratch, size_t scratch_floats, void* stream);
int ams_k_ce_loss_grad_soft_layout(const float* logits, int32_t B, int32_t h, int32_t w, int32_t ld, int32_t NC, const int32_t* class_idx_host,
                                   int32_t K, int32_t H, int32_t W, const uint8_t* teacher, const float* teacher_logits, int32_t th, int32_t tw,
                                   int32_t layout, double* loss_dev, float* dlogits, float* scratch, size_t scratch_floats, void* stream);
int ams_k_ce_loss_grad_kd(const float* logits, int32_t B, int32_t h, int32_t w, int32_t ld, int32_t NC, const int32_t* class_idx_host,
                          int32_t K, int32_t H, int32_t W, const uint8_t* teacher, const float* teacher_logits, int32_t th, int32_t tw,
                          int32_t layout, double* loss_dev, float* dlogits, float* scratch, size_t scratch_floats, void* stream,
                          float temperature, float alpha);
int ams_k_ce_loss_grad_weighted(const float* logits, int32_t B, int32_t h, int32_t w, int32_t ld, int32_t NC, const int32_t* class_idx_host,
                                int32_t K, int32_t H, int32_t W, const uint8_t* teacher, const float* teacher_logits, int32_t th, int32_t tw,
                                int32_t layout, double* loss_dev, float* dlogits, float* scratch, size_t scratch_floats, void* stream,
                                float temperature, float alpha, const float* class_weights_host, float conf_gamma);
int ams_k_ce_loss_grad_mined(const float* logits, int32_t B, int32_t h, int32_t w, int32_t ld, int32_t NC, const int32_t* class_idx_host,
                             int32_t K, int32_t H, int32_t W, const uint8_t* teacher, const float* teacher_logits, int32_t th, int32_t tw,
                             int32_t layout, double* loss_dev, float* dlogits, float* scratch, size_t scratch_floats, void* stream,
                             float temperature, float alpha, const float* class_weights_host, float conf_gamma, float top_k,
                             uint8_t* labels_out_dev, float* key_out_dev, ams_mining_result* result_dev, void* mining_scratch_dev,
                             size_t mining_scratch_bytes);

int ams_k_pointwise_wgrad(const float* x, const float* dy, int64_t M, int32_t K, int32_t N, float* dw,
                          float* scratch, size_t scratch_floats, void* stream);
size_t ams_k_pointwise_wgrad_scratch(int64_t M, int32_t K, int32_t N);
int ams_k_pointwise_wgrad_split(const float* x, const float* dy, int64_t M, int32_t K, int32_t N, float* dw,
                                float* scratch, size_t scratch_floats, void* stream);

int ams_k_depthwise3x3_dgrad(const float* dy, int32_t B, int32_t H, int32_t W, int32_t C, const float* w,
                             int32_t stride, int32_t rate, float* dx, void* stream);
int ams_k_depthwise3x3_wgrad(const float* x, const float* dy, int32_t B, int32_t H, int32_t W, int32_t C,
                             int32_t stride, int32_t rate, float* dw, float* scratch, size_t scratch_floats,
                             void* stream);

int ams_k_pointwise_red(const float* x, int64_t M, int32_t K, const float* w, int32_t N, int32_t trans_w, int32_t split, int32_t mode,
                        const float* center, const float* z, const float* scale, const float* shift, const float* mean, const float* rstd,
                        int32_t act, const float* res, float* y, float* part, size_t part_floats, int32_t* rows_out, uint16_t* panels,
                        size_t panel_elems, void* stream);

int ams_k_pointwise_xform(const float* x, int64_t M, int32_t K, const float* w, int32_t N, int32_t trans_w, int32_t split, int32_t x_mode,
                          int32_t x_act, const float* v0, const float* v1, const float* v2, const float* x2, float* y, float* x_tmp,
                          uint16_t* panels, size_t panel_elems, void* stream);
int ams_k_pointwise_wgrad_xform(const float* x, const float* dy, int64_t M, int32_t K, int32_t N, int32_t split, int32_t x_mode, int32_t x_act,
                                const float* v0, const float* v1, int32_t dy_mode, const float* d0, const float* d1, const float* d2,
                                const float* dy2, float* dw, float* scratch, size_t scratch_floats, void* stream);

size_t ams_k_depthwise3x3_fwd_bn_scratch(int32_t B, int32_t H, int32_t W, int32_t C, int32_t rate);
int ams_k_depthwise3x3_fwd_bn(const float* ze, int32_t B, int32_t H, int32_t W, int32_t C, const float* w, int32_t rate,
                              const float* scale, const float* shift, int32_t act, const float* center, float* zd, float* scratch,
                              size_t scratch_floats, int32_t* rows_out, void* stream);
size_t ams_k_depthwise3x3_dgrad_bn_scratch(int32_t B, int32_t H, int32_t W, int32_t C);
int ams_k_depthwise3x3_dgrad_bn(const float* dz, int32_t B, int32_t H, int32_t W, int32_t C, const float* w, int32_t rate,
                                const float* z_prev, const float* scale, const float* shift, int32_t act, const float* mean,
                                const float* rstd, float* out, float* scratch, size_t scratch_floats, int32_t* rows_out, void* stream);
size_t ams_k_depthwise3x3_dgrad_bn_apply_scratch(int32_t B, int32_t H, int32_t W, int32_t C, int32_t rate);
size_t ams_k_depthwise3x3_fwd_bn_tiles_scratch(int32_t B, int32_t H, int32_t W, int32_t C, int32_t rate);
int ams_k_depthwise3x3_fwd_bn_tiles(const float* ze, int32_t B, int32_t H, int32_t W, int32_t C, const float* w, int32_t rate, const float* scale,
                                    const float* shift, int32_t act, const float* center, float* zd, float* scratch, size_t scratch_floats,
                                    int32_t* rows_out, void* stream);
int ams_k_depthwise3x3_dgrad_bn_apply(const float* dy, const float* zd, const float* cA, const float* cB, const float* cC, int32_t B, int32_t H, int32_t W,
                                      int32_t C, const float* w, int32_t rate, const float* z_prev, const float* scale, const float* shift, int32_t act,
                                      const float* mean, const float* rstd, float* out, float* scratch, size_t scratch_floats, int32_t* rows_out,
                                      void* stream);

size_t ams_k_xx_gram_scratch(int64_t M, int32_t Cin);
int ams_k_xx_gram(const float* x, int64_t M, int32_t Cin, double* scratch, size_t scratch_doubles, double* xx64, float* xx32, void* stream);
int ams_k_expand_stats(const double* xx64, int32_t Cin, const float* w_exp, int32_t Cexp, double n, const float* center, const float* gamma,
                       const float* beta, float eps, float one_minus_decay, float* moving_mean, float* moving_var, float* scale, float* shift,
                       float* save_mean, float* save_rstd, double* sums, void* stream);

size_t ams_k_xdw_train_scratch(int32_t B, int32_t H, int32_t W, int32_t Cin, int32_t Cexp);
int ams_k_xdw_fwd_stats(const float* x, int32_t B, int32_t H, int32_t W, int32_t Cin, const float* w_exp, int32_t Cexp, const float* center,
                        float* scratch, size_t scratch_floats, int32_t* rows_out, int64_t* stride_out, void* stream);
int ams_k_xdw_bwd_reduce(const float* x, int32_t B, int32_t H, int32_t W, int32_t Cin, const float* w_exp, int32_t Cexp, const float* sc_e,
                         const float* sh_e, const float* mean_e, const float* rstd_e, int32_t act_e, const float* w_dw, int32_t stride,
                         const float* dz_d, float* scratch, size_t scratch_floats, int32_t* rows_out, int64_t* stride_out, void* stream);
int ams_k_xdw_bwd_dx(const float* x, int32_t B, int32_t H, int32_t W, int32_t Cin, const float* w_exp, int32_t Cexp, const float* sc_e,
                     const float* sh_e, int32_t act_e, const float* w_dw, int32_t stride, const float* dz_d, const float* cA, const float* cB,
                     const float* cC, const float* res, float* dx, void* stream);
size_t ams_k_xdw_stem_scratch(int32_t B, int32_t fH, int32_t fW);
int ams_k_xdw_bwd_reduce_stem(const void* frames, int32_t frames_dtype, int32_t B, int32_t fH, int32_t fW, float pixel_scale, const float* w_stem,
                              const float* sc_e, const float* sh_e, const float* mean_e, const float* rstd_e, int32_t act_e, const float* w_dw,
                              const float* dz_d, float* scratch, size_t scratch_floats, int32_t* rows_out, int64_t* stride_out, void* stream);
int ams_k_xdw_dwe(const float* G1, const float* xx_g0, int32_t Cin, int32_t Cexp, const float* w_exp, const float* cA, const float* cB,
                  const float* cC, float* dw_exp, void* stream);

int ams_k_adam(float* params, const float* grads, float* m, float* v, const uint8_t* mask, int64_t n, float lr_t,
               float beta1, float beta2, float eps, void* stream);

int ams_debug_launch_table_needs_attr(int32_t device, uint64_t kernel_key, size_t lds);
int ams_debug_reload_knobs(void);
int ams_debug_phase_cycles(int32_t which, uint64_t* out, int32_t n);

#ifdef __cplusplus
}
#endif
#endif
```

Baseline: 13110.

## Skip idle and halo-only steps in fused expand+depthwise streaming kernels

Adds a shared step classifier that, for each segment item, works out which pipeline steps actually touch interior pixels, which only need zero halo writes, and which are idle. The expand and depthwise loops in the stream and wreg kernels now run only to the per-item step count, and skip the MFMA expand work, global loads and depthwise compute on steps outside the active rectangle. This targets wasted work on edge segments and padding, at the cost of extra per-step branching and index bookkeeping. It also exposes a host-side step-count query for inspection.

```diff
diff --git a/ams_amd/csrc/api.hip b/ams_amd/csrc/api.hip
--- a/ams_amd/csrc/api.hip
+++ b/ams_amd/csrc/api.hip
@@ -965,6 +965,24 @@
                                float* y, uint16_t* panels, size_t panel_elems, int32_t presplit, int32_t y_h2i, void* stream) {
     return expand_dw_stream_entry("expand_dw_stream_f16", true, x, B, H, W, Cin, w_exp, scale_e, shift_e, Cexp, w_dw, rate, scale_d, shift_d, y, panels,
                                   panel_elems, 2, presplit, y_h2i, stream);
+}
+
+int ams_k_expand_dw_steps(int32_t B, int32_t H, int32_t W, int32_t Cin, int32_t Cexp, int32_t rate, int32_t f16, int32_t presplit, int32_t* out, size_t n) {
+    const bool f32 = !f16 && Cin <= 32;
+    const bool wreg = !f32 && presplit == 2;
+    BlockCall c;
+    c.B = B; c.H = H; c.W = W; c.Cin = Cin; c.Cexp = Cexp; c.rate = rate;
+    if (f32 && rate < 0) { c.stride = -rate; c.rate = 1; }
+    AMS_REQUIRE(B > 0 && H > 0 && W > 0, "expand_dw_steps: no pixels: B=%d, %d x %d", B, H, W);
+    AMS_REQUIRE(expand_dw_stream_supported(Cin, Cexp, c.stride, c.rate) && (!f16 || Cin >= 64), "expand_dw_steps: unsupported shape Cin=%d Cexp=%d rate=%d",
+                Cin, Cexp, rate);
+    AMS_REQUIRE(out && n >= 10, "expand_dw_steps: out needs at least 10 elements");
+    const int np = f32 ? 0 : (f16 ? 2 : 3);
+    XdwGeom g;
+    const bool fits = wreg ? expand_dw_wreg_geom(B, H, W, Cin, Cexp, c.rate, np, &g) : expand_dw_stream_geom(B, H, W, Cin, Cexp, c.rate, np, &g);
+    AMS_REQUIRE(fits, "expand_dw_steps: no segment geometry fits LDS (W=%d rate=%d)", W, rate);
+    expand_dw_steps(g, H, W, c.rate, out, n);
+    return AMS_OK;
 }
 
 int ams_k_global_mean(const float* x, int32_t B, int64_t HW, int32_t C, float* y, float* scratch, size_t scratch_floats,
diff --git a/ams_amd/csrc/k_xdw_stream.hip b/ams_amd/csrc/k_xdw_stream.hip
--- a/ams_amd/csrc/k_xdw_stream.hip
+++ b/ams_amd/csrc/k_xdw_stream.hip
@@ -1,6 +1,7 @@
 #include "pw_common.hpp"
 #include "split_bf16.hpp"
 #include "block_call.hpp"
+#include "xdw_steps.hpp"
 
 namespace ams {
 
@@ -126,8 +127,10 @@
             const int i0 = segy * a.SH, j0 = segx * a.SW;
             const bool live = i0 < Hs && j0 < Ws;
             const int64_t frame0 = (int64_t)b * a.H * a.W * a.Cin + (F32 ? 0 : 8 * q);
+            const XdwItemSteps steps = xdw_item_steps(Wp, STEP, a.SH, Hs, Ws, i0, j0);
+            XdwWalk ew = xdw_e_start();
             int e_row, e_col;
-            { const int e0 = 16 * wave + l15; e_row = e0 / Wp; e_col = e0 - e_row * Wp; }
+            { const int e0 = steps.inside.t0 * STEP + 16 * wave + l15; e_row = e0 / Wp; e_col = e0 - e_row * Wp; }
             float4 raw[(PRE || F32) ? 1 : KS][2];
             u32x4 rawp[PRE ? KS : 1][NP];
             float4 rawf[F32 ? KS : 1];
@@ -151,21 +154,47 @@
                     raw[s][1] = ld4(a.x + off + 32 * s + 4);
                 }
             };
-            {
+            if (steps.T_item > 0) {
                 const int64_t p = next_pixel();
 #pragma unroll
                 for (int s = 0; s < KS; ++s) load_stage(p, s);
             }
-            for (int t = 0; t < a.T; ++t) {
+            auto end_step = [&]() {
+                sbase += STEP;
+                if (sbase == R) sbase = 0;
+                lap(0);
+                __syncthreads();
+                lap(1);
+                ++nstep;
+            };
+            auto other_step = [&](int t) {
+                if (xdw_e_class(t, ew, steps) == XDW_E_ZERO) {
+                    const float4 z = make_float4(0.f, 0.f, 0.f, 0.f);
+                    float* dst = ring + sbase * PITCH + ring_lane;
+                    const bool mirror = sbase == 0 && 16 * wave + l15 < MIRROR;
+#pragma unroll
+                    for (int tt = 0; tt < NT; ++tt) {
+                        st4(dst + 16 * tt, z);
+                        if (mirror) st4(dst + R * PITCH + 16 * tt, z);
+                    }
+                }
+                xdw_advance(ew, steps);
+                end_step();
+            };
+            int t = 0;
+            for (; t < steps.inside.t0 && t < steps.T_item; ++t) other_step(t);
+            for (; t <= steps.inside.t1 && t < steps.T_item; ++t) {
+                xdw_advance(ew, steps);
+                {
                 const bool inside = in_next;
-                f32x4 acc[NT], accx[H16 ? NT : 1];
-#pragma unroll
-                for (int tt = 0; tt < NT; ++tt) acc[tt] = (f32x4){0.f, 0.f, 0.f, 0.f};
-#pragma unroll
-                for (int tt = 0; tt < (H16 ? NT : 1); ++tt) accx[tt] = (f32x4){0.f, 0.f, 0.f, 0.f};
                 e_row += qS; e_col += rS;
                 if (e_col >= Wp) { e_col -= Wp; ++e_row; }
                 const int64_t pn = next_pixel();
+                f32x4 acc[NT], accx[H16 ? NT : 1];
+#pragma unroll
+                for (int tt = 0; tt < NT; ++tt) acc[tt] = (f32x4){0.f, 0.f, 0.f, 0.f};
+#pragma unroll
+                for (int tt = 0; tt < (H16 ? NT : 1); ++tt) accx[tt] = (f32x4){0.f, 0.f, 0.f, 0.f};
                 if constexpr (F32) {
 #pragma unroll
                     for (int s = 0; s < KS; ++s) {
@@ -244,13 +273,10 @@
                         if (mirror) st4(dst + R * PITCH + 16 * tt, v);
                     }
                 }
-                sbase += STEP;
-                if (sbase == R) sbase = 0;
-                lap(0);
-                __syncthreads();
-                lap(1);
-                ++nstep;
+                }
+                end_step();
             }
+            for (; t < steps.T_item; ++t) other_step(t);
             __syncthreads();
         }
         flush(0);
@@ -284,7 +310,12 @@
             int d_row, d_col;
             { const int c0 = Wp - 1 + pt * PX; d_row = c0 / Wp; d_col = c0 - d_row * Wp; d_row -= 2; }
             __syncthreads();
-            for (int t = 0; t < a.T; ++t) {
+            const XdwItemSteps steps = xdw_item_steps(Wp, STEP, a.SH, Hs, Ws, i0, j0);
+            XdwWalk dw = xdw_d_start(Wp);
+            for (int t = 0; t < steps.T_item; ++t) {
+                const bool d_act = xdw_d_active(t, dw, steps);
+                xdw_advance(dw, steps);
+                if (d_act) {
                 if constexpr (S == 2) {
 #pragma unroll
                     for (int h = 0; h < PX; h += 2) {
@@ -372,6 +403,7 @@
                         }
                     }
                 }
+                }
                 d_row += qS; d_col += rS;
                 if (d_col >= Wp) { d_col -= Wp; ++d_row; }
                 cb += STEP;
@@ -450,6 +482,48 @@
     return xds_plan_try(B, H, W, Cin, Cexp, rate, np, 2, 4, 4, nsy_force, 0, groups_force, p);
 }
 
+bool expand_dw_stream_geom(int B, int H, int W, int Cin, int Cexp, int rate, int np, XdwGeom* g) {
+    XdsPlan p;
+    if (!xds_plan(B, H, W, Cin, Cexp, rate, np, &p)) return false;
+    const int step = 16 * p.nwe;
+    g->step = step; g->SH = p.SH; g->SW = p.SW; g->Wp = p.SW + 2; g->T = ((p.SH + 2) * g->Wp + step - 1) / step; g->ring = p.ring;
+    g->nsy = p.nsy; g->nsx = p.nsx; g->cgroups = (Cexp + 16 * p.nt - 1) / (16 * p.nt);
+    g->items = B * rate * rate * p.nsy * p.nsx; g->groups = p.groups;
+    g->nt = p.nt; g->nwe = p.nwe; g->nwd = p.nwd; g->nrg = 1; g->lds = p.lds;
+    return true;
+}
+
+void expand_dw_steps(const XdwGeom& g, int H, int W, int rate, int32_t* out, size_t n) {
+    const size_t per_item = 10, per_step = per_item + 5 * (size_t)g.items;
+    const bool items_out = n >= per_step, steps_out = n >= per_step + (size_t)g.T * g.items;
+    int64_t sum[5] = {0, 0, 0, 0, 0};
+    for (int item = 0; item < g.items; ++item) {
+        int u1 = item;
+        const int segx = u1 % g.nsx; u1 /= g.nsx;
+        const int segy = u1 % g.nsy; u1 /= g.nsy;
+        const int sub = u1 % (rate * rate);
+        const int sy = sub / rate, sx = sub - sy * rate;
+        const int Hs = (H - sy + rate - 1) / rate, Ws = (W - sx + rate - 1) / rate;
+        const XdwItemSteps s = xdw_item_steps(g.Wp, g.step, g.SH, Hs, Ws, segy * g.SH, segx * g.SW);
+        XdwWalk e = xdw_e_start(), d = xdw_d_start(g.Wp);
+        int cnt[5] = {s.T_item, 0, 0, 0, 0};
+        for (int t = 0; t < g.T; ++t) {
+            const int cls = xdw_e_class(t, e, s);
+            const bool act = xdw_d_active(t, d, s);
+            xdw_advance(e, s);
+            xdw_advance(d, s);
+            if (t < s.T_item) { cnt[1] += cls == XDW_E_COMPUTE; cnt[2] += cls == XDW_E_ZERO; cnt[3] += act; cnt[4] += cls == XDW_E_COMPUTE && act; }
+            if (steps_out) out[per_step + (size_t)item * g.T + t] = cls + 4 * act + 8 * (t < s.T_item);
+        }
+        for (int k = 0; k < 5; ++k) {
+            sum[k] += cnt[k];
+            if (items_out) out[per_item + 5 * (size_t)item + k] = cnt[k];
+        }
+    }
+    out[0] = g.step; out[1] = g.Wp; out[2] = g.SH; out[3] = g.T; out[4] = g.items;
+    for (int k = 0; k < 5; ++k) out[5 + k] = (int32_t)sum[k];
+}
+
 bool expand_dw_stream_supported(int Cin, int Cexp, int stride, int rate) {
     if (rate != 1 && rate != 2) return false;
     if (stride == 2) { if (rate != 1 || Cin > 32) return false; }
@@ -510,8 +584,10 @@
     const bool h16 = !f32 && c.expand.np == AMS_NP_F16;
     const int np = f32 ? 0 : h16 ? 2 : c.expand.np;
     AMS_REQUIRE((int64_t)H * W * Cexp * 4 < 0x7fffffffLL, "expand_dw_stream: a frame of the output exceeds 2 GiB");
-    XdsPlan p;
-    AMS_REQUIRE(xds_plan(B, H, W, Cin, Cexp, rate, np, &p), "expand_dw_stream: no segment geometry fits LDS (W=%d rate=%d)", W, rate);
+    XdwGeom g;
+    AMS_REQUIRE(expand_dw_stream_geom(B, H, W, Cin, Cexp, rate, np, &g), "expand_dw_stream: no segment geometry fits LDS (W=%d rate=%d)", W, rate);
+    XdsPlan p{};
+    p.nt = g.nt; p.nwe = g.nwe; p.nwd = g.nwd; p.lds = g.lds;
     XdsArgs a;
     memset(&a, 0, sizeof(a));
     a.x = c.x; a.xs = f32 ? nullptr : c.x_parts; a.xs_plane = c.x_plane; a.wf = c.expand.w; a.B = B; a.H = H; a.W = W; a.Cin = Cin; a.wp = c.expand.panels; a.plane = c.expand.plane;
@@ -524,10 +600,9 @@
         same_pad(W, 3, 2, 1, &a.Wo, &pl);
         a.cy0 = 1 - pt; a.cx0 = 1 - pl;
     }
-    const int step = 16 * p.nwe;
-    a.SH = p.SH; a.SW = p.SW; a.Wp = p.SW + 2; a.T = ((p.SH + 2) * a.Wp + step - 1) / step; a.ring = p.ring;
-    a.nsy = p.nsy; a.nsx = p.nsx; a.chunks = (Cexp + 16 * p.nt - 1) / (16 * p.nt);
-    a.items = B * rate * rate * p.nsy * p.nsx; a.groups = p.groups;
+    a.SH = g.SH; a.SW = g.SW; a.Wp = g.Wp; a.T = g.T; a.ring = g.ring;
+    a.nsy = g.nsy; a.nsx = g.nsx; a.chunks = g.cgroups;
+    a.items = g.items; a.groups = g.groups;
     a.y_fmt = c.y_fmt;
     a.timed = knobs().xwr_timed;
     if (h16) {
diff --git a/ams_amd/csrc/k_xdw_wreg.hip b/ams_amd/csrc/k_xdw_wreg.hip
--- a/ams_amd/csrc/k_xdw_wreg.hip
+++ b/ams_amd/csrc/k_xdw_wreg.hip
@@ -1,6 +1,7 @@
 #include "pw_common.hpp"
 #include "split_bf16.hpp"
 #include "block_call.hpp"
+#include "xdw_steps.hpp"
 
 namespace ams {
 
@@ -146,17 +147,27 @@
 #pragma unroll
                 for (int k = 0; k < LPT; ++k) sA[buf * AUNITS + pdst[k]] = piece[k];
             };
-            load_pieces(loader_pixel());
-            store_pieces(par);
+            const XdwItemSteps steps = xdw_item_steps(Wp, STEP, a.SH, Hs, Ws, i0, j0);
+            XdwWalk ew = xdw_e_start();
+            int cls_next = xdw_e_class(0, ew, steps);
+            if (cls_next == XDW_E_COMPUTE) {
+                load_pieces(loader_pixel());
+                store_pieces(par);
+            }
             __syncthreads();
-            for (int t = 0; t < a.T; ++t) {
+            for (int t = 0; t < steps.T_item; ++t) {
+                const int cls = cls_next;
 #pragma unroll
                 for (int rg = 0; rg < NRG; ++rg) {
                     in_cur[rg] = inside_of(rg);
                     e_row[rg] += qS; e_col[rg] += rS;
                     if (e_col[rg] >= Wp) { e_col[rg] -= Wp; ++e_row[rg]; }
                 }
-                if constexpr (!(ABL & 1)) load_pieces(loader_pixel());
+                xdw_advance(ew, steps);
+                cls_next = xdw_e_class(t + 1, ew, steps);
+                const bool load_next = cls_next == XDW_E_COMPUTE && !(ABL & 1);
+                if (load_next) load_pieces(loader_pixel());
+                if (cls == XDW_E_COMPUTE) {
                 f32x4 acc[NRG][2], accx[H16 ? NRG : 1][2];
                 auto zero_acc = [&]() {
 #pragma unroll
@@ -238,7 +249,20 @@
                         }
                     }
                 }
-                store_pieces(par ^ 1);
+                } else if (cls == XDW_E_ZERO && active && !(ABL & 16)) {
+                    const float4 z = make_float4(0.f, 0.f, 0.f, 0.f);
+#pragma unroll
+                    for (int rg = 0; rg < NRG; ++rg) {
+                        float* dst = ring + (sbase + 16 * rg) * PITCH + ring_lane;
+                        const bool mirror = sbase == 0 && rg == 0 && l15 < MIRROR;
+#pragma unroll
+                        for (int tt = 0; tt < 2; ++tt) {
+                            st4(dst + 16 * tt, z);
+                            if (mirror) st4(dst + R * PITCH + 16 * tt, z);
+                        }
+                    }
+                }
+                if (cls_next == XDW_E_COMPUTE) store_pieces(par ^ 1);
                 par ^= 1;
                 sbase += STEP;
                 if (sbase == R) sbase = 0;
@@ -326,7 +350,16 @@
                     }
                 }
             };
-            for (int t = 0; t < a.T; ++t) {
+            const XdwItemSteps steps = xdw_item_steps(Wp, STEP, a.SH, Hs, Ws, i0, j0);
+            XdwWalk dw = xdw_d_start(Wp);
+            for (int t = 0; t < steps.T_item; ++t) {
+                const bool d_act = xdw_d_active(t, dw, steps);
+                xdw_advance(dw, steps);
+                const int row0 = d_row, col0 = d_col, off0c = d_off;
+                d_row += qS; d_col += rS; d_off += stepdelta;
+                if (d_col >= Wp) { d_col -= Wp; ++d_row; d_off += wrapdelta; }
+                const int cb_next = cb + STEP >= R ? cb + STEP - R : cb + STEP;
+                if (d_act) {
                 load_row(0);
                 load_row(1);
                 load_row(2);
@@ -349,11 +382,6 @@
                                 AMS_DW_FMA4(acc4[hh][u], vv, w4);
                             }
                 }
-                const int row0 = d_row, col0 = d_col, off0c = d_off;
-                d_row += qS; d_col += rS; d_off += stepdelta;
-                if (d_col >= Wp) { d_col -= Wp; ++d_row; d_off += wrapdelta; }
-                cb += STEP;
-                if (cb >= R) cb -= R;
                 if constexpr (TIMED) {
 #pragma unroll
                     for (int hh = 0; hh < NH; ++hh)
@@ -362,6 +390,8 @@
                     lap(3);
                 }
                 epilogue(acc4, row0, col0, off0c);
+                }
+                cb = cb_next;
                 lap(0);
                 __syncthreads();
                 lap(1);
@@ -424,12 +454,7 @@
     return launch_xwr_k<KS, NP, 4, 4, 1, H16>(a, lds, st);
 }
 
-int launch_expand_dw_wreg(const BlockCall& c, hipStream_t st) {
-    RUN_RC(block_call_check("expand_dw_wreg", BK_WREG, c));
-    const int B = c.B, H = c.H, W = c.W, Cin = c.Cin, Cexp = c.Cexp, rate = c.rate;
-    const bool h16 = c.expand.np == AMS_NP_F16;
-    const int np = h16 ? 2 : c.expand.np;
-    AMS_REQUIRE((int64_t)H * W * Cexp * 4 < 0x7fffffffLL, "expand_dw_wreg: a frame of the output exceeds 2 GiB");
+bool expand_dw_wreg_geom(int B, int H, int W, int Cin, int Cexp, int rate, int np, XdwGeom* g) {
     int nwe = 4, nsy_force = 0, nsx_force = 0, groups_force = 0, nrg = 2;
     if (knobs().xwr_set) { const int* f = knobs().xwr; nwe = f[0]; nsy_force = f[1]; nsx_force = f[2]; groups_force = f[3]; nrg = f[4]; }
     if (nwe != 4 && nwe != 8) nwe = 4;
@@ -444,25 +469,43 @@
         ring = (2 * (SW + 2) + 2 + 2 * step + step - 1) / step * step;
         if (xwr_lds(Cin, np, nwe, nrg, ring) <= budget || SW <= 1) break;
     }
-    AMS_REQUIRE(xwr_lds(Cin, np, nwe, nrg, ring) <= budget, "expand_dw_wreg: no segment geometry fits LDS (W=%d rate=%d)", W, rate);
+    if (xwr_lds(Cin, np, nwe, nrg, ring) > budget) return false;
     nsx = (Ws + SW - 1) / SW;
     const int cgroups = (Cexp + 32 * nwe - 1) / (32 * nwe);
     int nsy = 1;
     if (nsy_force > 0) nsy = nsy_force;
     else
         while ((int64_t)B * rate * rate * cgroups * nsx * nsy < 512 && (Hs + nsy - 1) / nsy > 8) ++nsy;
+    g->nt = 2; g->nwe = nwe; g->nwd = 4; g->nrg = nrg; g->step = step;
+    g->SH = (Hs + nsy - 1) / nsy; g->SW = SW; g->Wp = SW + 2; g->T = ((g->SH + 2) * g->Wp + step - 1) / step; g->ring = ring;
+    g->nsy = nsy; g->nsx = nsx; g->cgroups = cgroups;
+    g->items = B * rate * rate * nsy * nsx;
+    int64_t groups = groups_force > 0 ? groups_force : (512 + cgroups - 1) / cgroups;
+    if (groups > g->items) groups = g->items;
+    g->groups = (int)groups;
+    g->lds = xwr_lds(Cin, np, nwe, nrg, ring);
+    return true;
+}
+
+int launch_expand_dw_wreg(const BlockCall& c, hipStream_t st) {
+    RUN_RC(block_call_check("expand_dw_wreg", BK_WREG, c));
+    const int B = c.B, H = c.H, W = c.W, Cin = c.Cin, Cexp = c.Cexp, rate = c.rate;
+    const bool h16 = c.expand.np == AMS_NP_F16;
+    const int np = h16 ? 2 : c.expand.np;
+    AMS_REQUIRE((int64_t)H * W * Cexp * 4 < 0x7fffffffLL, "expand_dw_wreg: a frame of the output exceeds 2 GiB");
+    XdwGeom g;
+    AMS_REQUIRE(expand_dw_wreg_geom(B, H, W, Cin, Cexp, rate, np, &g), "expand_dw_wreg: no segment geometry fits LDS (W=%d rate=%d)", W, rate);
+    const int nwe = g.nwe, nrg = g.nrg;
     XwrArgs a;
     memset(&a, 0, sizeof(a));
     a.xs = c.x_parts; a.xs_plane = c.x_plane; a.B = B; a.H = H; a.W = W; a.Cin = Cin; a.wp = c.expand.panels; a.plane = c.expand.plane; a.sc_e = c.expand.scale;
     a.sh_e = c.expand.shift; a.act_e = c.expand.act; a.Cexp = Cexp; a.w_dw = c.dw.w; a.sc_d = c.dw.scale; a.sh_d = c.dw.shift; a.act_d = c.dw.act; a.y = c.y; a.rate = rate;
-    a.SH = (Hs + nsy - 1) / nsy; a.SW = SW; a.Wp = SW + 2; a.T = ((a.SH + 2) * a.Wp + step - 1) / step; a.ring = ring;
-    a.nsy = nsy; a.nsx = nsx; a.cgroups = cgroups;
-    a.items = B * rate * rate * nsy * nsx;
+    a.SH = g.SH; a.SW = g.SW; a.Wp = g.Wp; a.T = g.T; a.ring = g.ring;
+    a.nsy = g.nsy; a.nsx = g.nsx; a.cgroups = g.cgroups;
+    a.items = g.items;
     a.y_fmt = c.y_fmt;
-    int64_t groups = groups_force > 0 ? groups_force : (512 + cgroups - 1) / cgroups;
-    if (groups > a.items) groups = a.items;
-    a.groups = (int)groups;
-    const size_t lds = xwr_lds(Cin, np, nwe, nrg, ring);
+    a.groups = g.groups;
+    const size_t lds = g.lds;
     if (h16) {
         switch (Cin / 32) {
             case 2: return launch_xwr_w<2, 2, true>(a, nwe, nrg, lds, st);
diff --git a/ams_amd/csrc/kernels.hpp b/ams_amd/csrc/kernels.hpp
--- a/ams_amd/csrc/kernels.hpp
+++ b/ams_amd/csrc/kernels.hpp
@@ -206,6 +206,10 @@
 int launch_expand_dw_stream(const BlockCall& c, hipStream_t st);
 
 int launch_expand_dw_wreg(const BlockCall& c, hipStream_t st);
+struct XdwGeom { int step, SH, SW, Wp, T, ring, nsy, nsx, cgroups, items, groups, nt, nwe, nwd, nrg; size_t lds; };
+bool expand_dw_stream_geom(int B, int H, int W, int Cin, int Cexp, int rate, int np, XdwGeom* g);
+bool expand_dw_wreg_geom(int B, int H, int W, int Cin, int Cexp, int rate, int np, XdwGeom* g);
+void expand_dw_steps(const XdwGeom& g, int H, int W, int rate, int32_t* out, size_t n);
 
 
 size_t image_colsum_scratch(int B, int C);
diff --git a/ams_amd/csrc/xdw_steps.hpp b/ams_amd/csrc/xdw_steps.hpp
--- /dev/null
+++ b/ams_amd/csrc/xdw_steps.hpp
@@ -0,0 +1,64 @@
+#pragma once
+
+#if defined(__HIPCC__) || defined(__CUDACC__)
+#define AMS_XDW_HD __host__ __device__ inline
+#else
+#define AMS_XDW_HD inline
+#endif
+
+namespace ams {
+
+enum XdwEClass { XDW_E_IDLE = 0, XDW_E_ZERO = 1, XDW_E_COMPUTE = 2 };
+
+struct XdwRect { int r0, r1, c0, c1, t0, t1; bool gaps; };
+
+struct XdwItemSteps {
+    int Wp, STEP, qS, rS;
+    int T_item;
+    XdwRect inside, read, stored;
+};
+
+AMS_XDW_HD XdwItemSteps xdw_item_steps(int Wp, int STEP, int SH, int Hs, int Ws, int i0, int j0) {
+    constexpr int EMPTY = -(1 << 20);
+    const int SW = Wp - 2;
+    const bool live = i0 < Hs && j0 < Ws;
+    const int rows = SH < Hs - i0 ? SH : Hs - i0, cols = SW < Ws - j0 ? SW : Ws - j0;
+    XdwItemSteps s;
+    s.Wp = Wp; s.STEP = STEP; s.qS = STEP / Wp; s.rS = STEP - s.qS * Wp;
+    s.T_item = live ? (rows * Wp + cols + Wp + 1) / STEP + 1 : 0;
+    const auto rect = [&](int r0, int r1, int c0, int c1, int lag) {
+        XdwRect r{r0, live ? r1 : EMPTY, c0, c1, 1, 0, false};
+        if (live) { r.t0 = (r0 * Wp + c0 + lag) / STEP; r.t1 = (r1 * Wp + c1 + lag) / STEP; r.gaps = Wp - (c1 - c0 + 1) >= STEP; }
+        return r;
+    };
+    s.inside = rect(i0 == 0 ? 1 : 0, SH + 1 < Hs - i0 ? SH + 1 : Hs - i0, j0 == 0 ? 1 : 0, SW + 1 < Ws - j0 ? SW + 1 : Ws - j0, 0);
+    s.read = rect(0, rows + 1, 0, cols + 1, 0);
+    s.stored = rect(1, rows, 1, cols, Wp + 1);
+    return s;
+}
+
+struct XdwWalk { int row, col; };
+AMS_XDW_HD XdwWalk xdw_e_start() { return XdwWalk{0, 0}; }
+AMS_XDW_HD XdwWalk xdw_d_start(int Wp) { return XdwWalk{-2, Wp - 1}; }
+AMS_XDW_HD void xdw_advance(XdwWalk& w, const XdwItemSteps& s) {
+    w.row += s.qS; w.col += s.rS;
+    if (w.col >= s.Wp) { w.col -= s.Wp; ++w.row; }
+}
+
+AMS_XDW_HD bool xdw_meets(int t, const XdwWalk& w, const XdwRect& r, const XdwItemSteps& s) {
+    if (!r.gaps) return (t >= r.t0) & (t <= r.t1);
+    int dist;
+    if (w.row > r.r1) return false;
+    if (w.row < r.r0) dist = (r.r0 - w.row) * s.Wp + r.c0 - w.col;
+    else if (w.col <= r.c1) dist = w.col < r.c0 ? r.c0 - w.col : 0;
+    else if (w.row < r.r1) dist = s.Wp - w.col + r.c0;
+    else return false;
+    return dist < s.STEP;
+}
+
+AMS_XDW_HD int xdw_e_class(int t, const XdwWalk& e, const XdwItemSteps& s) {
+    return ((t >= s.inside.t0) & (t <= s.inside.t1)) ? XDW_E_COMPUTE : (xdw_meets(t, e, s.read, s) ? XDW_E_ZERO : XDW_E_IDLE);
+}
+AMS_XDW_HD bool xdw_d_active(int t, const XdwWalk& d, const XdwItemSteps& s) { return xdw_meets(t, d, s.stored, s); }
+
+}
diff --git a/ams_amd/hip.py b/ams_amd/hip.py
--- a/ams_amd/hip.py
+++ b/ams_amd/hip.py
@@ -171,6 +171,7 @@
                                     C.POINTER(FirstBlockPlan), _vp]),
     "ams_k_first_block_tiles": (C.c_int, [_vp, _i32, _i32, _i32, _i32, _f32, _vp, _vp, _vp, _vp, _vp, _vp, _vp, _vp, _vp, _vp, _vp]),
     "ams_k_first_block_plan": (C.c_int, [_i32, _i32, _i32, _i32, _i32, C.POINTER(_i32), C.POINTER(FirstBlockPlan)]),
+    "ams_k_expand_dw_steps": (C.c_int, [_i32, _i32, _i32, _i32, _i32, _i32, _i32, _i32, C.POINTER(_i32), _sz]),
     "ams_k_expand_dw": (C.c_int, [_vp, _i32, _i32, _i32, _i32, _vp, _vp, _vp, _i32, _vp, _i32, _i32, _vp, _vp, _vp, _vp]),
     "ams_k_expand_dw_stream": (C.c_int, [_vp, _i32, _i32, _i32, _i32, _vp, _vp, _vp, _i32, _vp, _i32, _vp, _vp, _vp, _vp, _sz, _i32, _i32, _vp]),
     "ams_k_global_mean": (C.c_int, [_vp, _i32, _i64, _i32, _vp, _vp, _sz, _vp]),
diff --git a/include/ams_hip.h b/include/ams_hip.h
--- a/include/ams_hip.h
+++ b/include/ams_hip.h
@@ -365,6 +365,8 @@
                             const float* scale_s, const float* shift_s, const float* w_dw, const float* scale_d, const float* shift_d,
                             const float* w_proj, const float* scale_p, const float* shift_p, float* y, void* stream);
 int ams_k_first_block_plan(int32_t frames_dtype, int32_t B, int32_t H, int32_t W, int32_t form, const int32_t* occupancy, ams_first_block_plan* plan_out);
+int ams_k_expand_dw_steps(int32_t B, int32_t H, int32_t W, int32_t Cin, int32_t Cexp, int32_t rate, int32_t f16, int32_t presplit, int32_t* out,
+                          size_t n);
 
 enum { AMS_RESIZE_NEAREST = 0, AMS_RESIZE_LINEAR = 1 };
 int ams_ingest_resize_u8(const uint8_t* src, int32_t Hs, int32_t Ws, int32_t C, int32_t mode, int32_t swap_rb, uint8_t* dst,
```

After: 13320 (median of 6 runs). 1.02x the previous value.
